# Lymphatus/caesium-clt

Measured on AMD Instinct MI355X. Metric: megapixels/sec JPEG q=80 1920x1080 batch, higher is better.
Workload: dtype int32

## Files before the change

caesium-clt_amd/binding.py:

```python
import ctypes as C
import os

_HERE = os.path.dirname(os.path.abspath(__file__))
NPHASES = 8
NKERNELS = 36
PHASE_NAMES = ["decode", "pixel", "masks_flags_runs", "stats_tables", "sizes_scan", "pack", "stuff_assemble", "reserved"]


class CCSParameters(C.Structure):
    _fields_ = [("keep_metadata", C.c_bool), ("jpeg_quality", C.c_uint32), ("jpeg_chroma_subsampling", C.c_uint32),
                ("jpeg_progressive", C.c_bool), ("jpeg_optimize", C.c_bool), ("jpeg_preserve_icc", C.c_bool),
                ("png_quality", C.c_uint32), ("png_optimization_level", C.c_uint32), ("png_force_zopfli", C.c_bool),
                ("png_optimize", C.c_bool), ("gif_quality", C.c_uint32), ("webp_quality", C.c_uint32), ("webp_lossless", C.c_bool),
                ("tiff_compression", C.c_uint32), ("tiff_deflate_level", C.c_uint32), ("width", C.c_uint32), ("height", C.c_uint32)]


class CCSResult(C.Structure):
    _fields_ = [("success", C.c_bool), ("code", C.c_uint32), ("error_message", C.c_char_p)]


class CByteArray(C.Structure):
    _fields_ = [("data", C.POINTER(C.c_uint8)), ("length", C.c_size_t)]


class Timing(C.Structure):
    _fields_ = [("total_ms", C.c_float), ("phase_ms", C.c_float * NPHASES), ("kernel_ms", C.c_float * NKERNELS), ("in_bytes", C.c_uint64), ("out_bytes", C.c_uint64),
                ("pixels", C.c_uint64), ("coef_bytes", C.c_uint64), ("n_images", C.c_uint32), ("n_failed", C.c_uint32), ("n_seq_decoded", C.c_uint32), ("n_par_fallback", C.c_uint32), ("n_par_short", C.c_uint32), ("n_prog_decoded", C.c_uint32), ("n_refine_chains", C.c_uint32), ("n_search_extra", C.c_uint32), ("n_fused_lists", C.c_uint32), ("n_list_refine", C.c_uint32), ("n_ac_in_lists", C.c_uint32)]


class PngTiming(C.Structure):
    _fields_ = [("total_ms", C.c_float), ("kernel_ms", C.c_float * 16), ("in_bytes", C.c_uint64), ("out_bytes", C.c_uint64), ("pixels", C.c_uint64),
                ("raw_bytes", C.c_uint64), ("n_images", C.c_uint32), ("n_failed", C.c_uint32), ("n_trials", C.c_uint32)]


class CaesiumError(RuntimeError):
    def __init__(self, code, message):
        super().__init__(f"[{code}] {message}")
        self.code = code


def library_path():
    return os.path.join(_HERE, "libcaesium_hip.so")


EXPORTS = ["cs_default_parameters", "cs_compress_in_memory", "cs_compress_to_size_in_memory", "cs_convert_in_memory",
           "cs_batch_compress", "cs_batch_extent", "cs_free_bytes", "cs_free_result", "csh_device_count", "csh_last_error", "csh_kernel_name", "csh_kernel_name_webp", "csh_release_cached_memory", "csh_warmup", "csh_batch_create",
           "csh_batch_run", "csh_batch_fetch", "csh_batch_destroy", "csh_batch_retain_dct", "csh_batch_set_quality", "csh_batch_rerun_encode", "cs_batch_compress_to_size", "csh_batch_geometry", "csh_batch_read_coefs",
           "csp_kernel_name", "csp_batch_create", "csp_batch_create_webp", "csp_batch_create_pixels", "csh_batch_create_pixels", "csh_batch_pixels", "csh_batch_create_from_pixels", "csp_png_to_jpeg", "csp_png_to_lossless_webp", "csp_batch_run", "csp_batch_fetch", "csp_batch_destroy", "csp_batch_geometry", "csp_batch_read_rows", "csp_batch_read_stream",
           "csp_batch_trials", "csp_batch_read_scores", "csp_batch_chunk_bits", "csh_batch_create_webp", "cs_batch_convert",
           "cswd_batch_create", "cswd_batch_run", "cswd_batch_pixels", "cswd_batch_read_pixels", "cswd_batch_alpha", "cswd_batch_read_rgba", "cswd_batch_destroy", "cswd_rgba_join", "cswd_rgba_destroy", "csh_batch_create_webp_from_pixels", "csh_batch_create_from_pixels_rgb", "csl_encode_pixels", "csl_attach_alpha"]


def _declare(L):
    P = C.POINTER
    L.cs_default_parameters.argtypes = [P(CCSParameters)]
    L.cs_default_parameters.restype = None
    L.cs_compress_in_memory.argtypes = [C.c_char_p, C.c_size_t, P(CCSParameters), P(CByteArray)]
    L.cs_compress_in_memory.restype = CCSResult
    L.cs_compress_to_size_in_memory.argtypes = [C.c_char_p, C.c_size_t, P(CCSParameters), C.c_size_t, C.c_bool, P(CByteArray)]
    L.cs_compress_to_size_in_memory.restype = CCSResult
    L.cs_convert_in_memory.argtypes = [C.c_char_p, C.c_size_t, P(CCSParameters), C.c_uint32, P(CByteArray)]
    L.cs_convert_in_memory.restype = CCSResult
    L.cs_batch_compress.argtypes = [P(CByteArray), C.c_size_t, P(CCSParameters), C.c_int, P(CByteArray), P(CCSResult)]
    L.cs_batch_extent.argtypes = [P(CByteArray), C.c_size_t]
    L.cs_batch_extent.restype = C.c_size_t
    L.cs_free_bytes.argtypes = [P(CByteArray)]
    L.cs_free_bytes.restype = None
    L.cs_free_result.argtypes = [P(CCSResult)]
    L.cs_free_result.restype = None
    L.csh_last_error.restype = C.c_char_p
    L.csh_kernel_name.argtypes = [C.c_int]
    L.csh_kernel_name.restype = C.c_char_p
    L.csh_kernel_name_webp.argtypes = [C.c_int]
    L.csh_kernel_name_webp.restype = C.c_char_p
    L.csh_batch_create.argtypes = [P(CByteArray), C.c_size_t, P(CCSParameters), C.c_int, P(C.c_void_p)]
    L.csh_batch_run.argtypes = [C.c_void_p, P(Timing)]
    L.csh_batch_fetch.argtypes = [C.c_void_p, P(CByteArray), P(CCSResult)]
    L.csh_batch_retain_dct.argtypes = [C.c_void_p, C.c_int]
    L.csh_batch_set_quality.argtypes = [C.c_void_p, P(C.c_uint32)]
    L.csh_batch_rerun_encode.argtypes = [C.c_void_p, P(Timing)]
    L.cs_batch_compress_to_size.argtypes = [P(CByteArray), C.c_size_t, P(CCSParameters), C.c_size_t, C.c_bool, C.c_int, P(CByteArray), P(CCSResult)]
    L.csh_batch_destroy.argtypes = [C.c_void_p]
    L.csh_batch_destroy.restype = None
    L.csh_batch_geometry.argtypes = [C.c_void_p, C.c_size_t, C.c_int, C.c_int, P(C.c_int), P(C.c_int), P(C.c_int), P(C.c_int)]
    L.csh_batch_read_coefs.argtypes = [C.c_void_p, C.c_size_t, C.c_int, C.c_int, C.c_void_p]
    L.csh_batch_create_webp.argtypes = [P(CByteArray), C.c_size_t, P(CCSParameters), C.c_int, P(C.c_void_p)]
    L.cs_batch_convert.argtypes = [P(CByteArray), C.c_size_t, P(CCSParameters), C.c_uint32, C.c_int, P(CByteArray), P(CCSResult)]
    L.csp_kernel_name.argtypes = [C.c_int]
    L.csp_kernel_name.restype = C.c_char_p
    L.csp_batch_create.argtypes = [P(CByteArray), C.c_size_t, P(CCSParameters), C.c_int, P(C.c_void_p)]
    L.csp_batch_run.argtypes = [C.c_void_p, P(PngTiming)]
    L.csp_batch_fetch.argtypes = [C.c_void_p, P(CByteArray), P(CCSResult)]
    L.csp_batch_destroy.argtypes = [C.c_void_p]
    L.csp_batch_destroy.restype = None
    L.csp_batch_geometry.argtypes = [C.c_void_p, C.c_size_t, P(C.c_uint32), P(C.c_uint32), P(C.c_uint32)]
    L.csp_batch_read_rows.argtypes = [C.c_void_p, C.c_size_t, C.c_void_p]
    L.csp_batch_read_stream.argtypes = [C.c_void_p, C.c_size_t, C.c_int, C.c_void_p]
    L.csp_batch_read_scores.argtypes = [C.c_void_p, C.c_size_t, C.c_void_p, P(C.c_int)]
    L.csp_batch_chunk_bits.argtypes = [C.c_void_p, C.c_size_t, C.c_int, P(C.c_uint64), C.c_size_t, P(C.c_size_t)]
    L.csp_batch_trials.argtypes = [C.c_void_p, C.c_size_t, P(C.c_int), P(C.c_uint64), P(C.c_int), P(C.c_int)]
    L.cswd_batch_create.argtypes = [P(CByteArray), C.c_size_t, C.c_int, P(C.c_void_p)]
    L.cswd_batch_run.argtypes = [C.c_void_p]
    L.cswd_batch_pixels.argtypes = [C.c_void_p, C.c_size_t, P(C.c_void_p), P(C.c_uint32), P(C.c_uint32), P(C.c_uint32), P(C.c_char_p)]
    L.cswd_batch_read_pixels.argtypes = [C.c_void_p, C.c_size_t, C.c_void_p]
    L.cswd_batch_alpha.argtypes = [C.c_void_p, C.c_size_t, P(C.c_void_p), P(C.c_void_p)]
    L.cswd_batch_read_rgba.argtypes = [C.c_void_p, C.c_size_t, C.c_void_p]
    L.cswd_batch_destroy.argtypes = [C.c_void_p]
    L.cswd_batch_destroy.restype = None
    L.cswd_rgba_join.argtypes = [C.c_void_p, C.c_void_p, C.c_uint32, C.c_uint32, C.c_int, C.POINTER(C.c_void_p), C.POINTER(C.c_void_p)]
    L.cswd_rgba_join.restype = C.c_int
# ... 344 lines not shown
```

caesium-clt_amd/csrc/batch.hpp:

```cpp
#pragma once
#include <array>
#include <chrono>
#include <map>
#include <string>
#include <vector>

#include "../../include/caesium_hip.h"
#include "devmem.hpp"
#include "jpeg_host.hpp"
#include "kernels.h"
#include "webp_kernels.h"

namespace csh {

struct Item {
    int code = 0;
    std::string msg;
    JpegInfo in;
    JpegInfo out;
    int image = -1;
    size_t file_size = 0;
    std::vector<uint8_t> meta_out;
};

struct DecodePlan {
    PinnedBytes bits_pool;
    std::vector<DecScan> dscans;
    std::vector<DevHuffSet> hsets;
    std::vector<ParHuffSet> phsets;
    std::vector<char> phset_fits;
    std::vector<ParHuffSet4> phsets4;
    std::vector<std::array<int8_t, 8>> slot4;
    bool use4 = true;
    std::vector<ParScan> pscans;
    std::vector<uint32_t> need_seq_init;
    std::vector<ProgChain> chains;
    std::vector<int> chain_scans;
    std::vector<RefineUnit> refine_units;
    uint32_t refine_hist = 0, refine_pos = 0, refine_max_blocks = 0;
    uint32_t total_sub = 0, max_sub = 0, max_par_blocks = 0, dc_total = 0;

    DevBuf<uint8_t> d_bits, d_clean;
    DevBuf<ParScan> d_pscans;
    DevBuf<uint64_t> d_pstate, d_relax_list[2], d_unstuff_off, d_blk_off, d_dc_off;
    DevBuf<uint32_t> d_unstuff_cnt, d_nblk, d_need_seq, d_need_seq_init, d_relax_cnt, d_scan_pending, d_cut_block, d_claim;
    DevBuf<uint16_t> d_hyp;
    DevBuf<int32_t> d_dcdiff;
    DevBuf<DecScan> d_dscans;
    DevBuf<ProgChain> d_chains;
    DevBuf<int> d_chain_scans;
    DevBuf<uint64_t> d_refine_hist;
    DevBuf<uint32_t> d_refine_pos, d_refine_prog;
    DevBuf<RefineUnit> d_refine_units;
    DevBuf<DevHuffSet> d_hsets;
    DevBuf<ParHuffSet> d_phsets;
    DevBuf<ParHuffSet4> d_phsets4;
};

struct PixelPlan {
    std::vector<PlaneWork> pwork;
    std::vector<ResizeWork> rwork;
    std::vector<ResizeTap> rtaps;
    std::vector<float> rweights;
    uint64_t rgb_bytes = 0, tmp_floats = 0, max_tmp = 0, max_dst = 0;
    uint32_t max_row_in = 0, max_out_w = 0, max_nh = 0;
    uint32_t max_src_px = 0;
    uint64_t plane_bytes = 0, oplane_bytes = 0;
    uint32_t max_quads = 0;
    bool any_layout = false, any_layout_rgb = false;

    DevBuf<uint8_t> d_planes, d_oplanes, d_rgb;
    DevBuf<PlaneWork> d_pwork;
    DevBuf<ResizeWork> d_rwork;
    DevBuf<ResizeTap> d_rtaps;
    DevBuf<float> d_rweights, d_rtmp;
    DevBuf<int16_t> d_dct_raw;
};

struct Stage {
    uint32_t work0 = 0, nwork = 0, slot0 = 0, nslots = 0, ech0 = 0, nech = 0, table0 = 0, ntables = 0, plan0 = 0, nplans = 0, nzc0 = 0, nnzc = 0, ls0 = 0, nls = 0, ts0 = 0, nts = 0, rs0 = 0, nrs = 0;
    bool nz_build[2] = {true, true}, nz_filter[2] = {true, true};
};
struct SearchImg {
    int cand_work[64]; int ncand;
    int Al_luma = 0, Al_chroma = 0;
    uint64_t best_luma = 0, best_chroma = 0;
    int split_luma = 0, split_chroma = 0;
    bool luma_on = false, chroma_on = false;
};

struct EncodePlan {
    std::vector<EncScan> script;
    std::vector<ScanWork> swork;
    uint32_t nslots = 0, nlist_slots = 0, ntok_slots = 0;
    uint32_t nref_slots = 0;
    uint32_t last_run_refine = 0;
    uint64_t total_corr = 0;
    uint64_t total_units = 0, total_words = 0;
    uint32_t max_units = 0;
    int ntables = 0;
    std::vector<TokPlan> plans;
    std::vector<int> plan_comp, plan_image;
    std::vector<EChunk> echunks;
    uint64_t tok_cap = 0;
    uint32_t tok_scale = 1;
    std::vector<TokRegion> regions;
    std::vector<uint32_t> region_est;
    uint32_t hist_rows = 0;
    std::vector<NzList> nzlists;
    std::vector<NzSet> nzsets;
    std::vector<int> nzset_of;
    std::vector<uint32_t> nzset_built;
    std::vector<int> nzset_comp, nzset_image;
    std::vector<NzChunk> nzchunks;
    std::vector<NzChunk> nzchunks_fused;
    uint32_t n_fused = 0;
    uint32_t last_run_fused = 0;
    uint32_t n_ac_lists = 0;
    uint32_t last_run_ac_lists = 0;
    std::vector<uint8_t> nzset_ac_lists;
    std::vector<uint32_t> nz_est, nz_worst;
    uint32_t nz_nrec = 0;
    uint64_t nz_cap = 0;
    bool search = false;
    enum { ST_1 = 0, ST_1B = 1, ST_2 = 2, ST_2B = 3, ST_2C = 4, ST_N = 5 };
    Stage stage[ST_N];
    void stage_begin(Stage &sg) {
        sg.work0 = uint32_t(swork.size()); sg.slot0 = nslots; sg.ech0 = uint32_t(echunks.size()); sg.table0 = uint32_t(ntables); sg.plan0 = uint32_t(plans.size());
        sg.nzc0 = uint32_t(nzchunks.size()); sg.ls0 = nlist_slots; sg.ts0 = ntok_slots; sg.rs0 = nref_slots;
    }
    void stage_end(Stage &sg) {
        sg.nwork = uint32_t(swork.size()) - sg.work0; sg.nslots = nslots - sg.slot0; sg.nech = uint32_t(echunks.size()) - sg.ech0;
        sg.ntables = uint32_t(ntables) - sg.table0; sg.nplans = uint32_t(plans.size()) - sg.plan0;
        sg.nnzc = uint32_t(nzchunks.size()) - sg.nzc0; sg.nls = nlist_slots - sg.ls0; sg.nts = ntok_slots - sg.ts0; sg.nrs = nref_slots - sg.rs0;
    }
    std::vector<SearchImg> simg;
    std::vector<uint8_t> work_active;
    uint32_t n_gated_runs = 0;
    std::vector<uint32_t> img_list, img_nlist, h_cost;
    std::map<std::array<int, 5>, int> cand_script;
    std::vector<uint8_t> hdr_pool;
    std::vector<uint32_t> hdr_off;

    DevBuf<uint8_t> d_hdr, d_tail, d_scan_tmp, d_work_active;
    DevBuf<EncScan> d_script;
    DevBuf<ScanWork> d_swork;
    DevBuf<uint32_t> d_slot_work;
    DevBuf<EChunk> d_echunks;
    DevBuf<SlotRec> d_slots;
    DevBuf<TokPlan> d_plans;
    DevBuf<uint64_t> d_corr, d_symbits, d_eobbits, d_tok_off, d_chunk_off, d_scan_raw_off;
    DevBuf<uint32_t> d_tok_cursor;
    DevBuf<TokRegion> d_regions;
    DevBuf<uint16_t> d_eobrun, d_slot_hist;
    DevBuf<uint32_t> d_img_list, d_img_nlist, d_scan_cost, d_slot_raw, d_slot_eobh, d_long_runs, d_long_cnt, d_tokens, d_chunk_ntok, d_chunk_bits, d_raw, d_scan_pad, d_chunk_ff, d_hdr_off;
    DevBuf<DevEncTable> d_tables;
    DevBuf<NzList> d_nzlists;
    DevBuf<NzSet> d_nzsets;
    DevBuf<NzChunk> d_nzchunks, d_nzchunks_fused;
    DevBuf<uint32_t> d_nz_pool, d_nz_cursor, d_nz_chunk_off, d_nz_chunk_cnt, d_list_slots, d_tok_slots, d_ref_slots;
};

struct TrellisPlan {
    bool trellis = false, dering = false;
    Stage tstage;
    std::vector<TrellisWork> twork;
    std::vector<TrellisRun> truns;
    uint32_t t_units = 0, t_max_rows = 0;
    std::vector<uint32_t> trows;
    bool t_sort = false;
    bool nz_once = false;

    DevBuf<TrellisWork> d_twork;
    DevBuf<TrellisRun> d_truns;
    DevBuf<uint32_t> d_tqueue, d_trows, d_tperm, d_tspill;
    DevBuf<uint8_t> d_tblk_cnt;
    DevBuf<uint16_t> d_tblk_off;
    DevBuf<uint64_t> d_tlambda, d_tdcbt;
};

struct WebpTail {
    uint32_t webp_mb_bytes = 768;
    std::vector<csw::WebpImg> wimgs;
    uint64_t wwork_bytes = 0, wlevels = 0;
    uint32_t wmax_luma = 0, wmax_mbh = 0;

    DevBuf<csw::WebpImg> d_wimgs;
    DevBuf<uint8_t> d_wwork, d_wscratch, d_wprobs, d_wupdate;
    DevBuf<uint32_t> d_wpart, d_wstats;
    DevBuf<int16_t> d_wlevels;
};

struct Outputs {
    uint64_t raw_bytes_cap = 0, out_cap = 0;
    DevBuf<uint8_t> d_out;
    DevBuf<uint64_t> d_img_off;
    DevBuf<uint32_t> d_img_size, d_img_size_pad, d_status, d_overflow;
    std::vector<uint32_t> h_img_size;
    std::vector<uint64_t> h_img_off;
    std::vector<uint32_t> h_status;
    bool ran = false;
};

}

struct csh_batch {
    int device = 0;
    hipStream_t stream = 0;
    bool have_stream = false;
    CCSParameters params;
    std::vector<csh::Item> items;
    int nimg = 0;
    bool lossless = false;
    bool rgb_out = false;
    bool webp = false;
    int test_pool_shift = -1;
    bool progressive = true;
    bool retain_dct = false;
    bool have_dct = false;
    int q_base = 0;

    std::vector<csh::ImgDesc> imgs;
    std::vector<csh::DevQuant> quants;
    uint32_t ntiles = 0, ntiles_in = 0, ntiles_out = 0, max_tiles = 0, max_dummy = 0;
    csh::DevBuf<csh::ImgDesc> d_imgs;
    csh::DevBuf<csh::DevQuant> d_quants;
    csh::DevBuf<int16_t> d_coef;

    csh::DecodePlan dec;
    csh::PixelPlan pix;
    csh::EncodePlan enc;
    csh::TrellisPlan tr;
    csh::WebpTail wp;
    csh::Outputs out;

    ~csh_batch() { if (have_stream) { (void)hipStreamSynchronize(stream); (void)hipStreamDestroy(stream); } }
};

namespace csh {

enum KernelSlot {
    KS_MEMSET_COEF, KS_UNSTUFF, KS_DEC_SPEC, KS_DEC_RELAX0, KS_DEC_RELAX, KS_DEC_WRITE, KS_DC_SCATTER, KS_REFINE_CHAINS, KS_DECODE_PROG_SEQ,
    KS_IDCT_PLANE, KS_RESIZE, KS_XFORM_DIRECT, KS_RESAMPLE_FDCT, KS_FIX_DUMMY, KS_MEMSET_ENC, KS_TRELLIS_STATS, KS_TRELLIS_AC, KS_TRELLIS_DC,
    KS_NZLIST, KS_TOKENS, KS_LIST_STATS, KS_AC_RUNS, KS_GEN_TABLES, KS_CHUNK_SIZES, KS_SCAN_CHUNK_BITS, KS_SCAN_LAYOUT, KS_PACK, KS_LIST_PACK,
    KS_FF_COUNT, KS_SCAN_SEARCH, KS_LAYOUT, KS_SCAN_IMAGES, KS_EMIT, KS_SPARE0, KS_SPARE1, KS_SPARE2, KS_COUNT,
    KS_WEBP_YUV = KS_XFORM_DIRECT, KS_WEBP_ENCODE = KS_RESAMPLE_FDCT, KS_WEBP_ASSEMBLE = KS_FIX_DUMMY
};
struct KernelSlotRow { KernelSlot slot; const char *name; int phase; };
constexpr KernelSlotRow kKernelSlots[] = {
    {KS_MEMSET_COEF, "memset_coef", 0},        {KS_UNSTUFF, "unstuff", 0},                 {KS_DEC_SPEC, "k_dec_spec", 0},
    {KS_DEC_RELAX0, "k_dec_relax0", 0},        {KS_DEC_RELAX, "k_dec_relax1_4", 0},        {KS_DEC_WRITE, "k_dec_write", 0},
    {KS_DC_SCATTER, "k_dc_scatter", 0},        {KS_REFINE_CHAINS, "k_refine_chains", 0},   {KS_DECODE_PROG_SEQ, "k_decode_prog+seq", 0},
    {KS_IDCT_PLANE, "k_idct_plane", 1},        {KS_RESIZE, "resize", 1},                   {KS_XFORM_DIRECT, "k_xform_direct", 1},
    {KS_RESAMPLE_FDCT, "k_resample+k_plane_fdct", 1}, {KS_FIX_DUMMY, "k_fix_dummy", 1},    {KS_MEMSET_ENC, "memset_enc", 2},
    {KS_TRELLIS_STATS, "trellis_stats", 1},    {KS_TRELLIS_AC, "k_trellis_ac", 1},         {KS_TRELLIS_DC, "k_trellis_dc", 1},
    {KS_NZLIST, "k_nzlist", 2},                {KS_TOKENS, "k_tokens", 2},                 {KS_LIST_STATS, "k_list_stats", 2},
    {KS_AC_RUNS, "k_ac_runs", 2},              {KS_GEN_TABLES, "k_gen_tables", 3},         {KS_CHUNK_SIZES, "k_chunk_sizes", 4},
    {KS_SCAN_CHUNK_BITS, "scan_chunk_bits", 4}, {KS_SCAN_LAYOUT, "scan_layout", 4},        {KS_PACK, "k_pack", 5},
    {KS_LIST_PACK, "k_list_pack", 5},          {KS_FF_COUNT, "k_ff_count", 6},             {KS_SCAN_SEARCH, "scan_search_stage2", 7},
    {KS_LAYOUT, "k_layout", 6},                {KS_SCAN_IMAGES, "scan_images", 6},         {KS_EMIT, "k_emit", 6},
    {KS_SPARE0, "", 7},                        {KS_SPARE1, "", 7},                         {KS_SPARE2, "", 7}};
constexpr bool kernel_slots_in_order() {
    for (int i = 0; i < int(sizeof kKernelSlots / sizeof kKernelSlots[0]); i++) if (kKernelSlots[i].slot != i) return false;
    return true;
}
static_assert(sizeof kKernelSlots / sizeof kKernelSlots[0] == CSH_NKERNELS && int(KS_COUNT) == int(CSH_NKERNELS), "one row per csh_timing.kernel_ms slot");
static_assert(kernel_slots_in_order(), "row i of kKernelSlots describes slot i");

struct PlanSwitches {
    std::string profile;
    bool nz_once = true;
    bool tr_sort = true;
    int prog_par = -1;
    bool fused_420 = true;
    bool nz_fused = true;
    bool ref_list = true;
    bool ac_tiles = false;
    static PlanSwitches read();
};

struct Laps {
    const bool trace;
    std::chrono::steady_clock::time_point at = std::chrono::steady_clock::now();
    std::string text;
    Laps();
    void lap(const char *what);
};

struct BatchPlanner {
    csh_batch *const b;
    const CByteArray *const inputs;
    const size_t count;
    const CCSParameters *const p;
    const csp_pixels *const px;
    const PlanSwitches sw;
    const bool progressive;
    uint16_t qout_nat[64];
    int script_base3 = 0, script_base1 = 0;
    std::vector<std::pair<std::vector<uint8_t>, int>> hset_keys;
    std::map<std::vector<uint16_t>, int> quant_index;
    uint64_t plane_off = 64, oplane_off = 0;

    BatchPlanner(csh_batch *b, const CByteArray *inputs, size_t count, const CCSParameters *p, const csp_pixels *px);
    void begin();
    void parse();
    int reserve_pinned();
    int plan_image(size_t n);
    int plan_search_stages();
    int plan_trellis();
    void finish_descriptors();
    int upload(Laps &laps);

private:
    void image_geometry(Item &it, ImgDesc &im);
    int decode_scans(Item &it, ImgDesc &im, const uint8_t *d);
    int huff_set(const JScan &js);
    void place_blocks(ParScan &ps, const JpegInfo &in, const JScan &js, uint32_t units, bool dc_rows, bool subseqs);
    int sequential_split(const Item &it, const ImgDesc &im, const uint8_t *d, int img_index, bool &par_ok);
    bool progressive_plan(const Item &it, const ImgDesc &im, int img_index);
    void plane_work(ImgDesc &im, const JpegInfo &in, const JpegInfo &o, int img_index, bool resized);
    void resize_work(const JpegInfo &in, const JpegInfo &o, int img_index);
    void output_scans(Item &it, ImgDesc &im, int img_index, size_t in_len);
    void frame_header(Item &it);
    template <class Fill> int enc_scan(const std::array<int, 5> &key, Fill fill);
    int cand_index(int comp, int Ss, int Se, int Ah, int Al);
    int dc_scan_index(int ncomp);
    int seq1_index(int comp);
    uint32_t nz_list(int img_index, int comp, int Al, const ImgDesc &im, size_t in_len);
    void add_works(Item &it, ImgDesc &im, int img_index, const std::vector<int> &list, size_t in_len, const JpegInfo &o, bool stats_only = false);
    template <class Make> void add_stage(int sid, Make make);
    template <class Add> void splits(const ImgDesc &im, Add &add, int i0, int i1, bool whole);
};

void layout_token_pool(csh_batch *b);

int run_once(csh_batch *b, csh_timing *t, bool requant_only);

int search_costs(csh_batch *b, AsmCtx &a, int stage);
uint32_t search_gate(csh_batch *b, int stage, int (*want)(const SearchImg &));
int search_decide(csh_batch *b, int stage);
int search_lists(csh_batch *b);

}
```

caesium-clt_amd/csrc/batch_plan.cpp:

```cpp
#include <algorithm>
#include <atomic>
#include <cmath>
#include <thread>

#include "batch.hpp"
#include "resize_host.h"

namespace csh {

static void build_dev_huff(const HuffSpec &h, DevHuff &d) {
    memset(&d, 0, sizeof d);
    for (int l = 0; l < 18; l++) d.maxcode[l] = -1;
    if (!h.present) return;
    int code = 0, p = 0;
    for (int l = 1; l <= 16; l++) {
        if (h.bits[l]) {
            d.valptr[l] = p - code;
            for (int i = 0; i < h.bits[l]; i++, p++, code++)
                if (l <= 9) {
                    int base = code << (9 - l);
                    for (int k = 0; k < (1 << (9 - l)); k++) d.look[(base + k) & 511] = uint16_t((l << 8) | h.vals[p]);
                }
            d.maxcode[l] = code - 1;
        }
// ... 115 lines not shown
    else if (hx == 2 && vx == 1 && cw > 2) u.cls = CSH_UP_H2V1;
    else if (hx == 1 && vx == 2) u.cls = CSH_UP_H1V2;
    else if (hx == 2 && vx == 2 && cw > 2) u.cls = CSH_UP_H2V2;
    else u.cls = CSH_UP_REP;
    return u;
}
static int dn_kind(int hx, int vx) { return hx == 1 ? CSH_DN_FULL : (hx == 4 ? CSH_DN_H4V1 : (vx == 2 ? CSH_DN_H2V2 : CSH_DN_H2V1)); }

static int plan_item(Item &it, const CCSParameters &p, bool lossless) {
    const JpegInfo &in = it.in;
    if (in.ncomp != 1 && in.ncomp != 3) { it.msg = "unsupported component count (CMYK/YCCK not on the device path yet)"; return CS_ERR_JPEG_FEATURE; }
    if (in.ncomp == 3) {
        bool rgb_ids = in.comp[0].id == 'R' && in.comp[1].id == 'G' && in.comp[2].id == 'B';
        if (in.adobe_transform == 0 || rgb_ids) { it.msg = "RGB-colourspace JPEG not on the device path yet"; return CS_ERR_JPEG_FEATURE; }
    }
    if (uint64_t(in.width) * uint64_t(in.height) > (1ull << 28)) { it.msg = "image dimensions too large for the device path"; return CS_ERR_JPEG_FEATURE; }
    it.out = JpegInfo();
    JpegInfo &o = it.out;
    o.width = in.width; o.height = in.height; o.ncomp = in.ncomp;
    if (p.width || p.height) {
        if (lossless) { it.msg = "resize + lossless transcode not on the device path"; return CS_ERR_UNSUPPORTED; }
        csh_compute_dimensions(in.width, in.height, int(p.width), int(p.height), o.width, o.height);
        if (o.width > 65500 || o.height > 65500 || uint64_t(o.width) * uint64_t(o.height) > (1ull << 28)) { it.msg = "resize target too large for JPEG"; return CS_ERR_JPEG_FEATURE; }
    }
    if (lossless) {
        for (int c = 0; c < in.ncomp; c++) o.comp[c] = in.comp[c];
        jpeg_geometry(o);
        return 0;
    }
    int ss = int(p.jpeg_chroma_subsampling);
    if (ss == 0) ss = 420;
    for (int c = 0; c < in.ncomp; c++) { o.comp[c].id = c + 1; o.comp[c].h = o.comp[c].v = 1; o.comp[c].tq = c ? 1 : 0; }
    if (in.ncomp == 3) {
        int blocks = 0;
        for (int c = 0; c < 3; c++) {
            const JComp &k = in.comp[c];
            blocks += k.h * k.v;
            if (in.hmax % k.h || in.vmax % k.v) { it.msg = "fractional chroma sampling ratio (component factors do not divide the largest ones)"; return CS_ERR_JPEG_FEATURE; }
            if (in.hmax / k.h > 4 || in.vmax / k.v > 4) { it.msg = "chroma sampling ratio above 4"; return CS_ERR_JPEG_FEATURE; }
        }
        if (blocks > 10) { it.msg = "more than 10 blocks per MCU"; return CS_ERR_JPEG_FEATURE; }
        if (ss == 420) { o.comp[0].h = 2; o.comp[0].v = 2; }
        else if (ss == 422) { o.comp[0].h = 2; o.comp[0].v = 1; }
        else if (ss == 411) { o.comp[0].h = 4; o.comp[0].v = 1; }
        else if (ss != 444) { it.msg = "unknown output chroma subsampling"; return CS_ERR_JPEG_FEATURE; }
    }
    jpeg_geometry(o);
    return 0;
}

void layout_token_pool(csh_batch *b) {
    b->enc.regions.resize(b->enc.region_est.size());
    if (b->test_pool_shift < 0) b->test_pool_shift = getenv("CSH_TEST_POOL_SHIFT") ? std::min(16, std::max(0, atoi(getenv("CSH_TEST_POOL_SHIFT")))) : 0;
    const int shift = b->test_pool_shift;
    uint64_t at = 0;
    for (size_t i = 0; i < b->enc.regions.size(); i++) {
        const uint64_t cap = std::min<uint64_t>(std::max<uint64_t>((uint64_t(b->enc.region_est[i]) * b->enc.tok_scale) >> shift, 64), 0xFFFFFFF0ull);
        b->enc.regions[i].base = at; b->enc.regions[i].cap = uint32_t(cap); b->enc.regions[i].pad = 0;
        at += (cap + 3) & ~uint64_t(3);
    }
    b->enc.tok_cap = at + 64;
    at = 0;
    for (size_t i = 0; i < b->enc.nzlists.size(); i++) {
        const uint64_t cap = std::min<uint64_t>(std::max<uint64_t>((uint64_t(b->enc.nz_est[i]) * b->enc.tok_scale) >> shift, 64), b->enc.nz_worst[i]);
        b->enc.nzlists[i].base = at; b->enc.nzlists[i].cap = uint32_t(cap);
        at += (cap + 3) & ~uint64_t(3);
    }
    b->enc.nz_cap = at + 64;
}

PlanSwitches PlanSwitches::read() {
    auto is = [](const char *name, const char *v) { const char *e = getenv(name); return e && !strcmp(e, v); };
    PlanSwitches s;
    const char *penv = getenv("CSH_PROFILE");
    s.profile = penv && *penv ? penv : "mozjpeg";
    s.nz_once = !is("CSH_NZ_ONCE", "0");
    s.tr_sort = !is("CSH_TR_SORT", "0");
    s.nz_fused = !is("CSH_NZ_FUSED", "0");
    s.ac_tiles = is("CSH_AC_TILES", "1");
    s.ref_list = is("CSH_REF_LIST", "1") || (s.ref_list && !is("CSH_REF_LIST", "0"));
    const char *pp = getenv("CSH_PROG_PAR");
    s.prog_par = pp && !strcmp(pp, "0") ? 0 : (pp && !strcmp(pp, "1") ? 1 : -1);
    s.fused_420 = !getenv("CSH_NO_FUSED_420");
    return s;
}

Laps::Laps() : trace(getenv("CSH_TRACE") != nullptr) {}
void Laps::lap(const char *what) {
    if (!trace) return;
    const auto now = std::chrono::steady_clock::now();
    char buf[64];
    snprintf(buf, sizeof buf, " %s %.1f", what, std::chrono::duration<double, std::milli>(now - at).count());
    text += buf; at = now;
}

BatchPlanner::BatchPlanner(csh_batch *b_, const CByteArray *inputs_, size_t count_, const CCSParameters *p_, const csp_pixels *px_)
    : b(b_), inputs(inputs_), count(count_), p(p_), px(px_), sw(PlanSwitches::read()), progressive(p_->jpeg_progressive) {}

void BatchPlanner::begin() {
    b->items.resize(count);
    quality_table(int(p->jpeg_quality), qout_nat);
    DevQuant qo; make_quant(qout_nat, qo);
    b->quants.push_back(qo);
    b->q_base = int(b->quants.size()) - 1;
    for (int q = 1; q <= 100; q++) { uint16_t tq[64]; quality_table(q, tq); DevQuant dq; make_quant(tq, dq); b->quants.push_back(dq); }
    b->progressive = progressive;

    add_script(b->enc.script, 3, true);
    add_script(b->enc.script, 1, true);
    add_script(b->enc.script, 3, false);
    add_script(b->enc.script, 1, false);
    script_base3 = progressive ? 0 : 16; script_base1 = progressive ? 10 : 17;
    const bool webp = b->webp, rgb_out = b->rgb_out;
    const std::string &profile = sw.profile;
    b->enc.search = progressive && !webp && !rgb_out && profile != "plain";
    const bool lossy_jpeg = !b->lossless && !webp && !rgb_out;
    b->tr.trellis = lossy_jpeg && (profile == "mozjpeg" || profile == "mozjpeg-trellis");
    b->tr.dering = lossy_jpeg && (profile == "mozjpeg" || profile == "mozjpeg-dering");
    b->tr.nz_once = b->tr.trellis && progressive && sw.nz_once && sw.tr_sort;
}

template <class Fill>
int BatchPlanner::enc_scan(const std::array<int, 5> &key, Fill fill) {
    auto f = b->enc.cand_script.find(key);
    if (f != b->enc.cand_script.end()) return f->second;
    EncScan e;
    memset(&e, 0, sizeof e);
    fill(e);
    b->enc.script.push_back(e);
    return b->enc.cand_script[key] = int(b->enc.script.size()) - 1;
}
int BatchPlanner::cand_index(int comp, int Ss, int Se, int Ah, int Al) {
    return enc_scan({comp, Ss, Se, Ah, Al}, [&](EncScan &e) {
        const int id = comp ? 1 : 0;
        e.ncomp = 1; e.comp[0] = comp; e.Ss = Ss; e.Se = Se; e.Ah = Ah; e.Al = Al;
        e.ntables = 1; e.dht_id[0] = 0x10 | id; e.sos_tdta[0] = id;
    });
}
int BatchPlanner::dc_scan_index(int ncomp) {
    return enc_scan({-ncomp, 0, 0, 0, 0}, [&](EncScan &e) {
        e.ncomp = ncomp;
        for (int k = 0; k < ncomp; k++) {
            e.comp[k] = k;
            const int id = k ? 1 : 0;
            int idx = -1;
            for (int t = 0; t < e.ntables; t++) if (e.dht_id[t] == id) idx = t;
            if (idx < 0) { idx = e.ntables; e.dht_id[e.ntables++] = id; }
            e.dc_tbl[k] = idx; e.sos_tdta[k] = id << 4;
        }
    });
}
int BatchPlanner::seq1_index(int comp) {
    return enc_scan({comp, 0, 63, -1, -1}, [&](EncScan &e) {
        const int id = comp ? 1 : 0;
        e.ncomp = 1; e.comp[0] = comp; e.Ss = 0; e.Se = 63; e.sequential = 1;
        e.ntables = 2; e.dht_id[0] = id; e.dht_id[1] = 0x10 | id; e.dc_tbl[0] = 0; e.ac_tbl[0] = 1; e.sos_tdta[0] = (id << 4) | id;
    });
}

static uint64_t blocks_of(const ImgDesc &im) {
    uint64_t n = 0;
    for (int k = 0; k < im.ncomp; k++) n += uint64_t(im.out[k].real_bw) * im.out[k].real_bh;
    return n;
}

uint32_t BatchPlanner::nz_list(int img_index, int comp, int Al, const ImgDesc &im, size_t in_len) {
    if (b->enc.nzset_of.size() < size_t(img_index + 1) * CSH_MAX_COMPS) b->enc.nzset_of.resize(size_t(img_index + 1) * CSH_MAX_COMPS, -1);
    int &si = b->enc.nzset_of[size_t(img_index) * CSH_MAX_COMPS + size_t(comp)];
    const uint32_t nu = uint32_t(im.out[comp].real_bw * im.out[comp].real_bh);
    if (si < 0) {
        NzSet S;
        memset(&S, 0, sizeof S);
        for (int L = 0; L < CSH_NZ_LEVELS; L++) S.list[L] = 0xFFFFFFFFu;
        S.cnt_base = 0xFFFFFFFFu;
        S.nunits = nu; S.real_bw = im.out[comp].real_bw; S.bw = im.out[comp].bw; S.tile_base = im.out[comp].tile_base;
        si = int(b->enc.nzsets.size());
        b->enc.nzsets.push_back(S); b->enc.nzset_built.push_back(0u); b->enc.nzset_comp.push_back(comp); b->enc.nzset_image.push_back(img_index);
    }
    const uint64_t blocks_all = blocks_of(im);
    static const uint32_t kShare[CSH_NZ_LEVELS] = {20, 16, 12, 9};
    for (int L : {0, Al}) {
        if (b->enc.nzsets[size_t(si)].list[L] != 0xFFFFFFFFu) continue;
        const uint32_t nch = (nu + 255) / 256;
        NzList R;
        memset(&R, 0, sizeof R);
        R.chunk0 = b->enc.nz_nrec; b->enc.nz_nrec += nch;
        b->enc.nzsets[size_t(si)].list[L] = uint32_t(b->enc.nzlists.size());
        b->enc.nzlists.push_back(R);
        const uint64_t est = uint64_t(in_len) * kShare[L] / 8 * nu / std::max<uint64_t>(1, blocks_all) + nu + 4ull * nch + 256;
        const uint64_t worst = uint64_t(nu) * 64 + 4ull * nch;
        b->enc.nz_est.push_back(uint32_t(std::min<uint64_t>(est, worst)));
        b->enc.nz_worst.push_back(uint32_t(std::min<uint64_t>(worst, 0xFFFFFFF0ull)));
    }
    return b->enc.nzsets[size_t(si)].list[Al];
}

void BatchPlanner::add_works(Item &it, ImgDesc &im, int img_index, const std::vector<int> &list, size_t in_len, const JpegInfo &o, bool stats_only) {
    const int w_first = int(b->enc.swork.size());
    uint32_t nz_need[CSH_MAX_COMPS] = {0, 0, 0}, nz_gate[CSH_MAX_COMPS] = {0, 0, 0};
    for (int sidx : list) {
        const EncScan &e = b->enc.script[sidx];
        ScanWork w;
        memset(&w, 0, sizeof w);
        w.image = img_index; w.scan = sidx;
        w.out_off = 0xFFFFFFFFu;
        const bool from_list = e.Ss > 0 && !e.sequential && e.Ah == 0;
        const bool ref_list = sw.ref_list && e.Ss > 0 && !e.sequential && e.Ah != 0;
        w.list = 0xFFFFFFFFu; w.rs_base = 0xFFFFFFFFu;
        if (from_list || ref_list) {
            if (e.Al >= CSH_NZ_LEVELS) { it.code = CS_ERR_JPEG_FEATURE; it.msg = "internal: output scan script outside what the list coder carries"; }
            else {
                w.list = nz_list(img_index, e.comp[0], e.Al, im, in_len);
                if (!nz_need[e.comp[0]]) nz_gate[e.comp[0]] = uint32_t(b->enc.swork.size());
                nz_need[e.comp[0]] |= 1u << e.Al;
            }
        }
        if (e.Ss == 0 && e.ncomp > 1) w.nunits = uint32_t(im.omcus_x * im.omcus_y);
        else w.nunits = uint32_t(im.out[e.comp[0]].real_bw * im.out[e.comp[0]].real_bh);
        w.unit_base = uint32_t(b->enc.total_units);
        b->enc.total_units += w.nunits;
        w.corr_base = 0xFFFFFFFFu;
        if (e.Ss > 0 && !e.sequential && e.Ah) { w.corr_base = uint32_t(b->enc.total_corr); b->enc.total_corr += w.nunits; }
        w.word_base = uint32_t(b->enc.total_words);
        if (e.Ss) b->enc.total_words += (w.nunits + 63) / 64;
        w.table_base = uint32_t(b->enc.ntables);
        b->enc.ntables += e.ntables;
        b->enc.max_units = std::max(b->enc.max_units, w.nunits);
        {
            const uint32_t nch = (w.nunits + 255) / 256;
            w.first_chunk = b->enc.nslots; b->enc.nslots += nch;
            w.hist_row0 = b->enc.hist_rows; b->enc.hist_rows += nch * uint32_t(e.ntables);
            uint32_t &cursor = (from_list && w.list != 0xFFFFFFFFu) ? b->enc.nlist_slots : b->enc.ntok_slots;
            w.ls_base = cursor; cursor += nch;
            if (ref_list && w.list != 0xFFFFFFFFu) { w.rs_base = b->enc.nref_slots; b->enc.nref_slots += nch; }
        }
        if (e.Ss == 0 || e.sequential) {
            uint32_t blocks = 0;
            for (int k = 0; k < e.ncomp; k++) blocks += e.ncomp > 1 ? uint32_t(o.comp[e.comp[k]].h * o.comp[e.comp[k]].v) : 1u;
            const uint32_t per_unit = e.sequential ? blocks * 20u : (e.Ah ? (blocks + 14u) / 15u : blocks);
            for (uint32_t j = 0; j < (w.nunits + 255) / 256; j++) b->enc.echunks.push_back(EChunk{uint32_t(b->enc.swork.size()), 0, 1, j, 0, uint32_t(b->enc.region_est.size())});
            b->enc.region_est.push_back(stats_only ? 64u : w.nunits * per_unit + 64);
        }
        b->enc.swork.push_back(w);
    }
    for (int c = 0; c < im.ncomp; c++) {
        if (!nz_need[c]) continue;
        const int si = b->enc.nzset_of[size_t(img_index) * CSH_MAX_COMPS + size_t(c)];
        uint32_t levels = stats_only ? (nz_need[c] | 1u) : ((nz_need[c] | 1u) & ~b->enc.nzset_built[size_t(si)]);
        b->enc.nzset_built[size_t(si)] |= levels;
        if (!stats_only && b->tr.nz_once && (levels & 1u)) levels = (levels & ~1u) | CSH_NZ_COMPACT0;
        const uint32_t nu = b->enc.nzsets[size_t(si)].nunits;
        for (uint32_t j = 0; levels && j < (nu + 255) / 256; j++) b->enc.nzchunks.push_back(NzChunk{uint32_t(si), j, levels, nz_gate[c]});
    }
    for (int c = 0; c < im.ncomp; c++) {
        int nac = 0;
        for (int sidx : list) { const EncScan &e = b->enc.script[sidx]; if (e.Ss > 0 && !e.sequential && e.Ah && e.comp[0] == c) { nac++; if (e.Al > 3 && !sw.ref_list) nac = 99; } }
        const bool too_many = !sw.ref_list && nac > CSH_TK_MAXSLOT;
        if (too_many) { it.code = CS_ERR_JPEG_FEATURE; it.msg = "internal: output scan script outside what the token kernel carries"; }
        const uint32_t nu = uint32_t(im.out[c].real_bw * im.out[c].real_bh);
        if (!nac || too_many) continue;
        const uint64_t blocks_all = blocks_of(im);
        const uint64_t scripts = b->enc.search ? uint64_t(nac + 1) / 2 : 1;
        const uint64_t est = uint64_t(in_len) * 3 * scripts * nu / std::max<uint64_t>(1, blocks_all) + uint64_t(nu) * nac + 1024;
        if (sw.ref_list) {
            for (size_t k = 0; k < list.size(); k++) {
                const EncScan &e = b->enc.script[list[k]];
                if (e.Ss > 0 && !e.sequential && e.Ah && e.comp[0] == c && b->enc.swork[size_t(w_first) + k].rs_base != 0xFFFFFFFFu) b->enc.swork[size_t(w_first) + k].region = uint32_t(b->enc.region_est.size());
            }
            b->enc.region_est.push_back(stats_only ? 64u : uint32_t(std::min<uint64_t>(est, 0x3FFFFFFFu)));
            continue;
        }
        TokPlan P;
        memset(&P, 0, sizeof P);
        P.nunits = nu; P.real_bw = im.out[c].real_bw; P.bw = im.out[c].bw; P.tile_base = im.out[c].tile_base;
        P.work0 = 0xFFFFFFFFu;
        for (size_t k = 0; k < list.size(); k++) {
            const EncScan &e = b->enc.script[list[k]];
            if (!(e.Ss > 0 && !e.sequential && e.Ah && e.comp[0] == c)) continue;
            const ScanWork &w = b->enc.swork[size_t(w_first) + k];
            if (P.work0 == 0xFFFFFFFFu) P.work0 = uint32_t(w_first) + uint32_t(k);
            AcSlot &a = P.s[P.nslot++];
            a.unit_base = w.unit_base; a.word_base = w.word_base; a.first_chunk = w.first_chunk; a.table_base = w.table_base; a.nunits_work = w.nunits; a.corr_base = w.corr_base;
            a.Ss = uint8_t(e.Ss); a.Se = uint8_t(e.Se); a.Ah = uint8_t(e.Ah); a.Al = uint8_t(e.Al);
        }
        for (uint32_t j = 0; j < (nu + 255) / 256; j++) b->enc.echunks.push_back(EChunk{uint32_t(img_index), uint16_t(c), 0, j, uint32_t(b->enc.plans.size()), uint32_t(b->enc.region_est.size())});
        b->enc.region_est.push_back(stats_only ? 64u : uint32_t(std::min<uint64_t>(est, 0x3FFFFFFFu)));
        b->enc.plan_comp.push_back(c); b->enc.plan_image.push_back(img_index);
        b->enc.plans.push_back(P);
    }
}

void BatchPlanner::parse() {
    std::atomic<size_t> next{0};
    auto worker = [&]() {
        for (size_t n; (n = next++) < count;) {
            Item &it = b->items[n];
            it.file_size = inputs[n].length;
            int type = sniff_type(inputs[n].data, inputs[n].length);
            if (type == CS_TYPE_UNKN) { it.code = CS_ERR_UNKNOWN_TYPE; it.msg = "unknown file type"; }
            else if (type != CS_TYPE_JPEG) { it.code = CS_ERR_UNSUPPORTED; it.msg = "this input format has no device path in this build (built: JPEG, PNG)"; }
            else it.code = parse_jpeg(inputs[n].data, inputs[n].length, it.in, it.msg);
        }
    };
    size_t nthreads = std::min<size_t>(std::min<size_t>(16, std::max(1u, std::thread::hardware_concurrency())), (count + 15) / 16);
    std::vector<std::thread> pool;
    for (size_t t = 1; t < nthreads; t++) pool.emplace_back(worker);
    worker();
    for (auto &t : pool) t.join();
}

int BatchPlanner::reserve_pinned() {
    size_t total = 0;
    for (size_t n = 0; n < count; n++) total += inputs[n].length;
    if (total + total / 16 + (64u << 10) >= 0xF0000000ull) { csh_set_error("csh_batch_create: more than 3.75 GiB of input in one device batch (cs_batch_extent sizes groups)"); return CS_ERR_POOL_OVERFLOW; }
    if (!b->dec.bits_pool.reserve(total + total / 16 + (64u << 10))) { csh_set_error("out of pinned host memory"); return CS_ERR_NO_DEVICE; }
    return 0;
}
// ... 533 lines not shown
        std::vector<uint8_t> fused(b->enc.nzsets.size(), 0);
        const bool lists_only = progressive && !sw.ac_tiles && sw.ref_list && sw.nz_once && sw.tr_sort && (!b->tr.trellis || (b->tr.t_sort && b->tr.nz_once));
        std::vector<uint8_t> planned(b->enc.nzsets.size(), 0);
        for (size_t i = 0; i < b->enc.plans.size(); i++) {
            const size_t at = size_t(b->enc.plan_image[i]) * CSH_MAX_COMPS + size_t(b->enc.plan_comp[i]);
            if (at < b->enc.nzset_of.size() && b->enc.nzset_of[at] >= 0) planned[size_t(b->enc.nzset_of[at])] = 1;
        }
        b->enc.nzset_ac_lists.assign(b->enc.nzsets.size(), 0);
        for (PlaneWork &w : b->pix.pwork) {
            w.ac_lists = 0u;
            const size_t at = size_t(w.image) * CSH_MAX_COMPS + size_t(w.comp);
            const int si = allowed && at < b->enc.nzset_of.size() ? b->enc.nzset_of[at] : -1;
            if (si < 0) continue;
            const NzSet &S = b->enc.nzsets[size_t(si)];
            if (S.real_bw != S.bw || S.list[0] == 0xFFFFFFFFu) continue;
            w.nzset = uint32_t(si); fused[size_t(si)] = 1; b->enc.n_fused++;
            if (lists_only && !planned[size_t(si)]) { w.ac_lists = 1u; b->enc.nzset_ac_lists[size_t(si)] = 1; b->enc.n_ac_lists++; }
        }
        for (TrellisWork &tw : b->tr.twork) tw.ac_lists = (tw.nzset != 0xFFFFFFFFu && b->enc.nzset_ac_lists[tw.nzset]) ? 1u : 0u;
        for (NzChunk &ch : b->enc.nzchunks_fused) if (fused[ch.set]) ch.levels &= ~1u;
        auto flags = [&](Stage &sg) {
            for (int f = 0; f < 2; f++) {
                const std::vector<NzChunk> &v = f ? b->enc.nzchunks_fused : b->enc.nzchunks;
                sg.nz_build[f] = sg.nz_filter[f] = false;
                for (uint32_t i = sg.nzc0; i < sg.nzc0 + sg.nnzc; i++) { sg.nz_build[f] |= (v[i].levels & 1u) != 0u; sg.nz_filter[f] |= (v[i].levels & ~1u) != 0u; }
            }
        };
        for (Stage &sg : b->enc.stage) flags(sg);
        flags(b->tr.tstage);
    }
    for (ParScan &ps : b->dec.pscans)
        for (int m = 0; m < ps.nb_mcu && m < 10; m++) {
            int dcs = ps.dct[m] & 3, acs = 4 + (ps.act[m] & 3);
            if (b->dec.use4) { dcs = std::max<int>(0, b->dec.slot4[ps.huff_set][dcs]); acs = std::max<int>(0, b->dec.slot4[ps.huff_set][acs]); }
            ps.sel |= uint64_t(dcs | (acs << 3)) << (6 * m);
        }
    {
        std::vector<int> last(b->dec.chains.size(), -1);
        for (int s = 0;; s++) {
            bool any = false;
            for (size_t c = 0; c < b->dec.chains.size(); c++)
                if (b->dec.chains[c].refine && b->dec.chains[c].count > s) {
                    RefineUnit u; u.chain = int(c); u.s = s; u.prev = last[c];
                    last[c] = int(b->dec.refine_units.size());
                    b->dec.refine_units.push_back(u);
                    any = true;
                }
            if (!any) break;
        }
    }
    b->ntiles = b->ntiles_in + b->ntiles_out;
    b->pix.plane_bytes = plane_off;
    b->pix.oplane_bytes = oplane_off;
    b->out.out_cap = b->out.raw_bytes_cap;
    layout_token_pool(b);
}

int BatchPlanner::upload(Laps &laps) {
    hipStream_t st = b->stream;
    if (!b->nimg) return 0;
    b->dec.bits_pool.flush_copies();
    laps.lap("copy_in");
    if (b->dec.d_bits.alloc(b->dec.bits_pool.size()) || (b->dec.bits_pool.size() && hipMemcpyAsync(b->dec.d_bits.p, b->dec.bits_pool.p, b->dec.bits_pool.size(), hipMemcpyHostToDevice, st) != hipSuccess) ||
        b->d_imgs.upload(b->imgs, st) || b->dec.d_dscans.upload(b->dec.dscans, st) || b->dec.d_chains.upload(b->dec.chains, st) || b->dec.d_chain_scans.upload(b->dec.chain_scans, st) ||
        b->dec.d_hsets.upload(b->dec.hsets, st) || b->dec.d_phsets.upload(b->dec.phsets, st) || (b->dec.use4 && b->dec.d_phsets4.upload(b->dec.phsets4, st)) || b->d_quants.upload(b->quants, st) || b->pix.d_pwork.upload(b->pix.pwork, st) ||
        b->enc.d_script.upload(b->enc.script, st) || b->enc.d_swork.upload(b->enc.swork, st) || b->enc.d_slot_work.alloc(size_t(b->enc.nslots) + 1) || b->enc.d_slots.alloc(size_t(b->enc.nslots) + 1) || b->enc.d_plans.upload(b->enc.plans, st) || b->enc.d_echunks.upload(b->enc.echunks, st) || b->enc.d_hdr.upload(b->enc.hdr_pool, st) ||
        b->enc.d_hdr_off.upload(b->enc.hdr_off, st) || b->dec.d_pscans.upload(b->dec.pscans, st) || b->pix.d_rwork.upload(b->pix.rwork, st) || b->pix.d_rtaps.upload(b->pix.rtaps, st) ||
        b->pix.d_rweights.upload(b->pix.rweights, st) || b->pix.d_rgb.alloc(b->pix.rgb_bytes + 64) || b->pix.d_rtmp.alloc((resize_is_fused(b->pix.max_row_in) ? 0 : b->pix.tmp_floats) + 16) || b->dec.d_need_seq_init.upload(b->dec.need_seq_init, st))
        return CS_ERR_NO_DEVICE;
    size_t nchunks = b->dec.bits_pool.size() / 64 + 1, nst = size_t(b->dec.total_sub) + b->dec.pscans.size() + 1;
    if (b->dec.d_clean.alloc(b->dec.bits_pool.size() + 64) || b->dec.d_unstuff_cnt.alloc(nchunks + 1) || b->dec.d_unstuff_off.alloc(nchunks + 2) ||
        b->dec.d_pstate.alloc(nst) || b->dec.d_relax_list[0].alloc(nst) || b->dec.d_relax_list[1].alloc(nst) || b->dec.d_relax_cnt.alloc(512) || b->dec.d_scan_pending.alloc(b->dec.pscans.size() + 1) || b->dec.d_cut_block.alloc(b->dec.pscans.size() + 1) || b->dec.d_claim.alloc(size_t(b->dec.total_sub) + 1) || b->dec.d_hyp.alloc((size_t(b->dec.total_sub) + 1) * 10) ||
        b->dec.d_nblk.alloc(size_t(b->dec.total_sub) + 1) || b->dec.d_blk_off.alloc(size_t(b->dec.total_sub) + 2) || b->dec.d_need_seq.alloc(b->nimg + 1) ||
        b->dec.d_dcdiff.alloc(size_t(b->dec.dc_total) + 1) || b->dec.d_dc_off.alloc(size_t(b->dec.dc_total) + 2) ||
        b->dec.d_refine_hist.alloc(size_t(b->dec.refine_hist) + 1) || b->dec.d_refine_pos.alloc(size_t(b->dec.refine_pos) + 1) || b->dec.d_refine_units.upload(b->dec.refine_units, st) ||
        b->dec.d_refine_prog.alloc(b->dec.refine_units.size() + 1))
        return CS_ERR_NO_DEVICE;
    if (b->d_coef.alloc(size_t(b->ntiles) * CSH_TILE_I16) || b->pix.d_planes.alloc(b->pix.plane_bytes + 64) || b->pix.d_oplanes.alloc(b->pix.oplane_bytes + 64) ||
        b->enc.d_symbits.alloc(b->enc.total_words + 1) || b->enc.d_eobbits.alloc(b->enc.total_words + 1) ||
        b->enc.d_long_runs.alloc(2 * (b->enc.total_units / 512 + b->enc.swork.size() + 16)) || b->enc.d_long_cnt.alloc(4) || b->enc.d_tail.alloc(b->enc.total_units + 1) || b->enc.d_eobrun.alloc(b->enc.total_units + 1) || b->enc.d_corr.alloc(b->enc.total_corr + 1) ||
        b->enc.d_tok_off.alloc(4 * size_t(b->enc.nslots) + 4) || b->enc.d_chunk_ntok.alloc(4 * size_t(b->enc.nslots) + 4) || b->enc.d_slot_hist.alloc(size_t(b->enc.hist_rows) * 256 + 256) ||
        b->enc.d_slot_raw.alloc(size_t(b->enc.nslots) + 1) || b->enc.d_img_list.upload(b->enc.img_list, st) || b->enc.d_img_nlist.upload(b->enc.img_nlist, st) || b->enc.d_scan_cost.alloc(b->enc.swork.size() + 1) || b->enc.d_slot_eobh.alloc(16 * size_t(b->enc.nslots) + 16) || b->enc.d_chunk_bits.alloc(size_t(b->enc.nslots) + 1) || b->enc.d_chunk_off.alloc(size_t(b->enc.nslots) + 2) || b->enc.d_tok_cursor.alloc(b->enc.region_est.size() + 1) || b->enc.d_regions.upload(b->enc.regions, st) ||
        b->enc.d_tables.alloc(b->enc.ntables) || b->enc.d_scan_pad.alloc(b->enc.swork.size() + 1) ||
        b->enc.d_nzlists.upload(b->enc.nzlists, st) || b->enc.d_nzsets.upload(b->enc.nzsets, st) || b->enc.d_nzchunks.upload(b->enc.nzchunks, st) || (b->enc.n_fused && b->enc.d_nzchunks_fused.upload(b->enc.nzchunks_fused, st)) || b->enc.d_list_slots.alloc(size_t(b->enc.nlist_slots) + 1) || b->enc.d_tok_slots.alloc(size_t(b->enc.ntok_slots) + 1) || b->enc.d_ref_slots.alloc(size_t(b->enc.nref_slots) + 1) ||
        b->enc.d_nz_cursor.alloc(b->enc.nzlists.size() + 1) || b->enc.d_nz_chunk_off.alloc(size_t(b->enc.nz_nrec) + 1) || b->enc.d_nz_chunk_cnt.alloc(size_t(b->enc.nz_nrec) + 1) ||
        b->enc.d_scan_raw_off.alloc(b->enc.swork.size() + 2) || b->out.d_img_size.alloc(b->nimg + 1) || b->out.d_img_size_pad.alloc(b->nimg + 1) ||
        b->out.d_img_off.alloc(b->nimg + 2) || b->out.d_status.alloc(b->nimg) || b->out.d_overflow.alloc(4))
        return CS_ERR_NO_DEVICE;
    if (hipMemsetAsync(b->enc.d_slots.p, 0, (size_t(b->enc.nslots) + 1) * sizeof(SlotRec), st) != hipSuccess ||
        hipMemsetAsync(b->enc.d_slot_work.p, 0, (size_t(b->enc.nslots) + 1) * sizeof(uint32_t), st) != hipSuccess) { csh_set_error("hipMemsetAsync failed"); return CS_ERR_NO_DEVICE; }
    launch_make_slots(st, b->enc.d_swork.p, uint32_t(b->enc.swork.size()), b->enc.d_script.p, b->enc.d_nzlists.p, b->enc.d_slots.p, b->enc.d_slot_work.p, b->enc.d_list_slots.p, b->enc.d_tok_slots.p, b->enc.d_ref_slots.p);
    if (b->tr.trellis && (b->tr.d_trows.upload(b->tr.trows, st) || (b->tr.t_sort && (b->tr.d_tperm.alloc(size_t(b->tr.t_units) + 1) || b->tr.d_tblk_cnt.alloc(size_t(b->tr.t_units) + 1) || (b->tr.nz_once && b->tr.d_tblk_off.alloc(size_t(b->tr.t_units) + 1)))))) return CS_ERR_NO_DEVICE;
    if (b->tr.trellis && (b->tr.d_twork.upload(b->tr.twork, st) || b->tr.d_truns.upload(b->tr.truns, st) || b->tr.d_tqueue.alloc(1) || b->tr.d_tlambda.alloc(size_t(b->tr.t_units) + 1) || b->tr.d_tdcbt.alloc(size_t(b->tr.t_units) + 1) ||
                       b->tr.d_tspill.alloc(trellis_spill_words(trellis_ac_slots())) || b->pix.d_dct_raw.alloc(size_t(b->ntiles_out) * CSH_TILE_I16)))
        return CS_ERR_NO_DEVICE;
    for (size_t n = 0; px && n < count; n++) {
        const Item &it = b->items[n];
        if (it.image < 0) continue;
        const ResizeWork &rw = b->pix.rwork[size_t(it.image)];
        if (rw.image != it.image) { csh_set_error("internal: resize work out of order"); return CS_ERR_NO_DEVICE; }
        if (hipMemcpyAsync(b->pix.d_rgb.p + rw.rgb_src_off, px[n].device_pixels, size_t(px[n].width) * px[n].height * px[n].channels, hipMemcpyDeviceToDevice, st) != hipSuccess) { csh_set_error("pixel copy failed"); return CS_ERR_NO_DEVICE; }
    }
    laps.lap("alloc+enqueue");
    if (hipStreamSynchronize(st) != hipSuccess) { csh_set_error("upload failed"); return CS_ERR_NO_DEVICE; }
    laps.lap("upload_wait");
    return 0;
}

}
```

caesium-clt_amd/csrc/batch_run.cpp:

```cpp
#include <algorithm>

#include "batch.hpp"

namespace csh {
namespace {

class KernelMarks {
    hipEvent_t ev[CSH_NKERNELS + 1];
    int created = 0, next = 0;
    const hipStream_t st;

public:
    explicit KernelMarks(hipStream_t s) : st(s) {}
    KernelMarks(const KernelMarks &) = delete;
    KernelMarks &operator=(const KernelMarks &) = delete;
    ~KernelMarks() { for (int i = 0; i < created; i++) (void)hipEventDestroy(ev[i]); }
    int start() {
        for (; created <= CSH_NKERNELS; created++) CSH_CHECK(hipEventCreate(&ev[created]));
        CSH_CHECK(hipEventRecord(ev[0], st));
        return 0;
    }
    int claim(KernelSlot slot, hipEvent_t *e) {
        if (int(slot) != next || next >= CSH_NKERNELS) {
            csh_set_error("internal: timing mark '%s' out of order (slot %d is next)", slot < KS_COUNT ? kKernelSlots[slot].name : "?", next);
// ... 149 lines not shown
                      b->pix.max_src_px, b->pix.max_tmp, b->pix.max_dst, b->pix.max_row_in, b->pix.max_out_w, b->pix.max_nh, !(b->webp || b->rgb_out), b->pix.any_layout_rgb);
        MARK(KS_RESIZE);
        return 0;
    }
    int pixels() {
        const int nw = b->lossless ? 0 : int(b->pix.pwork.size());
        int16_t *rawp = ((b->retain_dct || b->tr.trellis) && !b->lossless) ? b->pix.d_dct_raw.p : nullptr;
        NzFuse nzf;
        memset(&nzf, 0, sizeof nzf);
        fused = nw && b->enc.n_fused;
        if (fused) {
            if (b->enc.d_nz_cursor.zero(st) || b->enc.d_nz_chunk_cnt.zero(st)) return -1;
            nzf.nzsets = b->enc.d_nzsets.p; nzf.nzlists = b->enc.d_nzlists.p; nzf.nz_pool = b->enc.d_nz_pool.p; nzf.nz_cursor = b->enc.d_nz_cursor.p;
            nzf.nz_chunk_off = b->enc.d_nz_chunk_off.p; nzf.nz_chunk_cnt = b->enc.d_nz_chunk_cnt.p; nzf.overflow = b->out.d_overflow.p;
            nzf.blk_cnt = (b->tr.trellis && b->tr.t_sort) ? b->tr.d_tblk_cnt.p : nullptr;
            nzf.blk_off = (nzf.blk_cnt && b->tr.nz_once) ? b->tr.d_tblk_off.p : nullptr;
        }
        if (nw && getenv("CSH_DEBUG") && (uint32_t(atoi(getenv("CSH_DEBUG"))) & 32768u))
            CSH_CHECK(hipMemsetAsync(b->d_coef.p + size_t(b->ntiles_in) * CSH_TILE_I16, 0x5A, size_t(b->ntiles - b->ntiles_in) * CSH_TILE_I16 * sizeof(int16_t), st));
        launch_xform_direct(st, b->d_imgs.p, b->pix.d_pwork.p, nw, b->max_tiles, b->d_quants.p, b->d_coef.p, b->d_coef.p, rawp, b->ntiles_in, b->tr.dering, nzf);
        MARK(KS_XFORM_DIRECT);
        launch_resample_plane(st, b->d_imgs.p, b->pix.d_pwork.p, nw, b->pix.max_quads, b->pix.d_planes.p, b->pix.d_oplanes.p);
        if (b->pix.any_layout) launch_resample_any(st, b->d_imgs.p, b->pix.d_pwork.p, nw, b->pix.max_quads, b->pix.d_planes.p, b->pix.d_oplanes.p);
        launch_plane_fdct(st, b->d_imgs.p, b->pix.d_pwork.p, nw, b->max_tiles, b->d_quants.p, b->pix.d_oplanes.p, b->d_coef.p, rawp, b->ntiles_in, b->tr.dering, nzf);
        launch_resample_fdct_420(st, b->d_imgs.p, b->pix.d_pwork.p, nw, b->max_tiles, b->d_quants.p, b->pix.d_planes.p, b->d_coef.p, rawp, b->ntiles_in, b->tr.dering, nzf);
        MARK(KS_RESAMPLE_FDCT);
        if (!b->lossless) launch_fix_dummy(st, b->d_imgs.p, nimg, b->max_dummy, b->d_coef.p);
        MARK(KS_FIX_DUMMY);
        return 0;
    }

    void fill_enc_ctx() {
        memset(&c, 0, sizeof c);
        c.imgs = b->d_imgs.p; c.script = b->enc.d_script.p; c.work = b->enc.d_swork.p; c.nwork = int(b->enc.swork.size());
        c.echunks = b->enc.d_echunks.p; c.plans = b->enc.d_plans.p; c.nechunks = uint32_t(b->enc.echunks.size()); c.slot_work = b->enc.d_slot_work.p; c.slots = b->enc.d_slots.p; c.nslots = b->enc.nslots;
        c.coef = b->d_coef.p; c.sym_bits = b->enc.d_symbits.p; c.eob_bits = b->enc.d_eobbits.p; c.tail = b->enc.d_tail.p;
        c.eobrun = b->enc.d_eobrun.p; c.long_runs = b->enc.d_long_runs.p; c.long_cnt = b->enc.d_long_cnt.p; c.corr = b->enc.d_corr.p;
        c.tokens = b->enc.d_tokens.p; c.regions = b->enc.d_regions.p; c.tok_cursor = b->enc.d_tok_cursor.p; c.tok_off = b->enc.d_tok_off.p; c.chunk_ntok = b->enc.d_chunk_ntok.p; c.slot_hist = b->enc.d_slot_hist.p; c.slot_raw = b->enc.d_slot_raw.p; c.slot_eobh = b->enc.d_slot_eobh.p;
        c.chunk_bits = b->enc.d_chunk_bits.p; c.chunk_off = b->enc.d_chunk_off.p; c.tables = b->enc.d_tables.p;
        c.raw = b->enc.d_raw.p; c.raw_words = raw_chunks * 16; c.status = b->out.d_status.p; c.overflow = b->out.d_overflow.p;
        c.nzlists = b->enc.d_nzlists.p; c.nzsets = b->enc.d_nzsets.p; c.nz_pool = b->enc.d_nz_pool.p; c.nz_cursor = b->enc.d_nz_cursor.p; c.nz_chunk_off = b->enc.d_nz_chunk_off.p; c.nz_chunk_cnt = b->enc.d_nz_chunk_cnt.p;
        c.debug = getenv("CSH_DEBUG") ? uint32_t(atoi(getenv("CSH_DEBUG"))) : 0u;
    }
    void fill_asm_ctx() {
        memset(&a, 0, sizeof a);
        a.imgs = b->d_imgs.p; a.script = b->enc.d_script.p; a.work = b->enc.d_swork.p; a.nimg = nimg;
        a.nwork = b->tr.trellis ? int(b->tr.tstage.work0) : c.nwork;
        a.tables = b->enc.d_tables.p; a.chunk_off = b->enc.d_chunk_off.p; a.scan_pad_bytes = b->enc.d_scan_pad.p; a.scan_raw_off = b->enc.d_scan_raw_off.p;
        a.raw = b->enc.d_raw.p; a.raw_chunks = raw_chunks; a.chunk_ff = b->enc.d_chunk_ff.p;
        a.hdr_pool = b->enc.d_hdr.p; a.hdr_off = b->enc.d_hdr_off.p; a.img_size = b->out.d_img_size.p; a.img_size_pad = b->out.d_img_size_pad.p;
        a.img_off = b->out.d_img_off.p; a.out = b->out.d_out.p; a.out_cap = b->out.out_cap; a.status = b->out.d_status.p; a.overflow = b->out.d_overflow.p;
        a.img_list = b->enc.d_img_list.p; a.img_nlist = b->enc.d_img_nlist.p; a.scan_cost = b->enc.d_scan_cost.p;
    }
    void fill_trellis_ctx(TrellisCtx &tc) {
        memset(&tc, 0, sizeof tc);
        tc.imgs = b->d_imgs.p; tc.quant = b->d_quants.p; tc.work = b->tr.d_twork.p; tc.nwork = int(b->tr.twork.size()); tc.runs = b->tr.d_truns.p; tc.nruns = uint32_t(b->tr.truns.size());
        tc.tables = b->enc.d_tables.p; tc.raw = b->pix.d_dct_raw.p; tc.raw_tile0 = b->ntiles_in; tc.coef = b->d_coef.p; tc.dcrec = b->tr.d_tlambda.p; tc.dcbt = b->tr.d_tdcbt.p;
        tc.spill = b->tr.d_tspill.p; tc.nslots = uint32_t(b->tr.d_tspill.n / trellis_spill_words(1)); tc.max_rows = b->tr.t_max_rows;
        tc.queue = b->tr.d_tqueue.p;
        tc.rows = b->tr.d_trows.p; tc.nrows = uint32_t(b->tr.trows.size());
        if (b->tr.t_sort) { tc.blk_cnt = b->tr.d_tblk_cnt.p; tc.perm = b->tr.d_tperm.p; }
        if (b->tr.t_sort && b->tr.nz_once) {
            tc.nz_pool = b->enc.d_nz_pool.p; tc.nzlists = b->enc.d_nzlists.p; tc.nzsets = b->enc.d_nzsets.p; tc.nz_chunk_off = b->enc.d_nz_chunk_off.p; tc.nz_chunk_cnt = b->enc.d_nz_chunk_cnt.p;
            tc.blk_off = b->tr.d_tblk_off.p;
        }
        tc.ac_lists = fused ? 1u : 0u;
        tc.debug = getenv("CSH_TR_DEBUG") ? uint32_t(atoi(getenv("CSH_TR_DEBUG"))) : 0u;
    }

    int encode_begin() {
        fill_enc_ctx();
        launch_reset_works(st, b->enc.d_swork.p, c.nwork);
        if (!fused && (b->enc.d_nz_cursor.zero(st) || b->enc.d_nz_chunk_cnt.zero(st))) return -1;
        if (b->enc.d_symbits.zero(st) || b->enc.d_eobbits.zero(st) || (!eobrun_cleared && b->enc.d_eobrun.zero(st)) || b->enc.d_tables.zero(st) || b->enc.d_tok_cursor.zero(st) || b->enc.d_slot_eobh.zero(st) || b->enc.d_scan_pad.zero(st)) return -1;
#ifdef CSH_EMUL
        if (b->enc.d_raw.zero(st)) return -1;
#else
        if ((c.debug & 8192u) && b->enc.d_raw.zero(st)) return -1;
#endif
        MARK(KS_MEMSET_ENC);
        return 0;
    }

    void set_stage(const Stage &sg) {
        c.echunks = b->enc.d_echunks.p + sg.ech0; c.nechunks = sg.nech; c.slot0 = sg.slot0; c.nslots = sg.nslots;
        c.nzchunks = (fused ? b->enc.d_nzchunks_fused.p : b->enc.d_nzchunks.p) + sg.nzc0; c.nnzchunks = sg.nnzc;
        c.nz_build = sg.nz_build[fused ? 1 : 0]; c.nz_filter = sg.nz_filter[fused ? 1 : 0];
        c.list_slots = b->enc.d_list_slots.p + sg.ls0; c.nlist_slots = sg.nls; c.tok_slots = b->enc.d_tok_slots.p + sg.ts0; c.ntok_slots = sg.nts;
        c.ref_slots = b->enc.d_ref_slots.p + sg.rs0; c.nref_slots = sg.nrs;
    }

    int trellis() {
        const Stage &tg = b->tr.tstage;
        set_stage(tg);
        c.stats_only = 1;
        if (b->enc.d_long_cnt.zero(st)) return -1;
        c.nz_blk_cnt = b->tr.t_sort ? b->tr.d_tblk_cnt.p : nullptr;
        c.nz_blk_off = (b->tr.t_sort && b->tr.nz_once) ? b->tr.d_tblk_off.p : nullptr;
        launch_nzlist(st, c);
        c.nz_blk_cnt = nullptr; c.nz_blk_off = nullptr;
        if (b->tr.t_sort) {
            TrellisCtx ts;
            memset(&ts, 0, sizeof ts);
            ts.work = b->tr.d_twork.p; ts.nwork = int(b->tr.twork.size()); ts.blk_cnt = b->tr.d_tblk_cnt.p; ts.perm = b->tr.d_tperm.p;
            launch_trellis_sort(st, ts);
        }
        launch_tokens(st, c);
        launch_list_stats(st, c);
        launch_ac_runs(st, c);
        launch_gen_tables(st, b->enc.d_tables.p + tg.table0, int(tg.ntables));
        c.stats_only = 0;
        if (b->enc.d_nz_cursor.zero(st)) return -1;
        MARK(KS_TRELLIS_STATS);
        TrellisCtx tc;
        fill_trellis_ctx(tc);
        if (b->tr.d_tqueue.zero(st)) return -1;
        launch_trellis_ac(st, tc);
        MARK(KS_TRELLIS_AC);
        launch_trellis_dc(st, tc);
        launch_fix_dummy(st, b->d_imgs.p, nimg, b->max_dummy, b->d_coef.p);
        MARK(KS_TRELLIS_DC);
        return 0;
    }

    int stage(const Stage &sg, bool mark, bool gate) {
#define SMARK(slot) do { if (mark) MARK(slot); } while (0)
        set_stage(sg);
        c.work_active = gate ? b->enc.d_work_active.p : nullptr;
        a.work0 = int(sg.work0); a.nwork_run = int(sg.nwork);
        if (b->enc.d_long_cnt.zero(st)) return -1;
        launch_nzlist(st, c);
        SMARK(KS_NZLIST);
        launch_list_refine(st, c);
        for (uint32_t wi = sg.work0; sg.nrs && wi < sg.work0 + sg.nwork; wi++)
            if (b->enc.swork[wi].rs_base != 0xFFFFFFFFu && (!gate || b->enc.work_active[wi])) b->enc.last_run_refine++;
        launch_tokens(st, c);
        SMARK(KS_TOKENS);
        launch_list_stats(st, c);
        SMARK(KS_LIST_STATS);
        launch_ac_runs(st, c);
        SMARK(KS_AC_RUNS);
        launch_gen_tables(st, b->enc.d_tables.p + sg.table0, int(sg.ntables));
        SMARK(KS_GEN_TABLES);
        launch_chunk_sizes(st, c);
        SMARK(KS_CHUNK_SIZES);
        launch_exclusive_scan(st, b->enc.d_chunk_bits.p + sg.slot0, b->enc.d_chunk_off.p + sg.slot0, sg.nslots, b->enc.d_scan_tmp.p, b->enc.d_scan_tmp.n);
        SMARK(KS_SCAN_CHUNK_BITS);
        launch_scan_sizes(st, a);
        launch_exclusive_scan(st, b->enc.d_scan_pad.p, b->enc.d_scan_raw_off.p, uint64_t(a.nwork), b->enc.d_scan_tmp.p, b->enc.d_scan_tmp.n);
        launch_scan_place(st, a);
        launch_zero_edges(st, c);
        SMARK(KS_SCAN_LAYOUT);
        launch_pack(st, c);
        SMARK(KS_PACK);
        launch_list_pack(st, c);
        SMARK(KS_LIST_PACK);
        launch_ff_count(st, a);
        SMARK(KS_FF_COUNT);
#undef SMARK
        return 0;
    }

    int gated_stage(int sid, int (*want)(const SearchImg &)) {
        if (!search_gate(b, sid, want)) return 0;
        b->enc.n_gated_runs++;
        if (b->enc.d_work_active.upload(b->enc.work_active, st)) return -1;
        if (stage(b->enc.stage[sid], false, true) || search_costs(b, a, sid)) return -1;
        return search_decide(b, sid);
    }
    int search() {
        b->enc.n_gated_runs = 0;
        if (search_costs(b, a, EncodePlan::ST_1) || search_decide(b, EncodePlan::ST_1)) return -1;
        if (gated_stage(EncodePlan::ST_1B, [](const SearchImg &si) { return si.luma_on ? 1 : 0; })) return -1;
        if (stage(b->enc.stage[EncodePlan::ST_2], false, false)) return -1;
        if (search_costs(b, a, EncodePlan::ST_2) || search_decide(b, EncodePlan::ST_2)) return -1;
        for (int sid : {int(EncodePlan::ST_2B), int(EncodePlan::ST_2C)})
            if (gated_stage(sid, [](const SearchImg &si) { return (si.luma_on ? 1 : 0) | (si.chroma_on ? 2 : 0); })) return -1;
        if (search_lists(b)) return -1;
        return 0;
    }

    int emit() {
        MARK(KS_SCAN_SEARCH);
        launch_layout(st, a);
        MARK(KS_LAYOUT);
        launch_exclusive_scan(st, b->out.d_img_size_pad.p, b->out.d_img_off.p, uint64_t(nimg), b->enc.d_scan_tmp.p, b->enc.d_scan_tmp.n);
        MARK(KS_SCAN_IMAGES);
        launch_emit(st, a);
        MARK(KS_EMIT);
        return 0;
    }

    int finish(bool phases) {
        CSH_CHECK(hipStreamSynchronize(st));
        CSH_CHECK(hipGetLastError());
        if (t && marks.read(t, phases)) return -1;
        if (t && !phases) t->n_images = uint32_t(nimg);
        return 0;
    }

    int webp() {
        const int nwimg = int(b->wp.wimgs.size());
        uint64_t out_bytes = 0;
        std::vector<uint64_t> off(size_t(b->nimg) + 1, 0);
        for (auto &wi : b->wp.wimgs) {
            const uint64_t cap = 4096 + uint64_t(wi.mbw) * wi.mbh * (b->wp.webp_mb_bytes + 2);
            wi.out_cap = uint32_t(std::min<uint64_t>(cap, 0xFFFFFF00u)); wi.out_off = out_bytes;
            off[wi.image] = out_bytes;
            out_bytes += (wi.out_cap + 63) & ~uint64_t(63);
            const int q = int(b->params.webp_quality);
            wi.quality = q < 0 ? 0 : q > 100 ? 100 : q;
        }
        off[b->nimg] = out_bytes;
        if (b->out.d_out.n < out_bytes + 64 && b->out.d_out.alloc(out_bytes + 64)) return -1;
        if ((b->wp.d_wscratch.n < out_bytes + 64 && b->wp.d_wscratch.alloc(out_bytes + 64)) || (b->wp.d_wpart.n < size_t(b->nimg) * 9 + 9 && b->wp.d_wpart.alloc(size_t(b->nimg) * 9 + 9)) ||
            (b->wp.d_wstats.n < size_t(b->nimg) * 2112 + 8 && (b->wp.d_wstats.alloc(size_t(b->nimg) * 2112 + 8) || b->wp.d_wprobs.alloc(size_t(b->nimg) * 1056 + 8) || b->wp.d_wupdate.alloc(size_t(b->nimg) * 1056 + 8))))
            return -1;
        if (b->wp.d_wstats.zero(st)) return -1;
        if (b->wp.d_wimgs.upload(b->wp.wimgs, st) || (b->wp.d_wwork.n < b->wp.wwork_bytes + 64 && b->wp.d_wwork.alloc(b->wp.wwork_bytes + 64)) ||
            (b->wp.d_wlevels.n < b->wp.wlevels + 64 && b->wp.d_wlevels.alloc(b->wp.wlevels + 64)))
            return -1;
        CSH_CHECK(hipMemcpyAsync(b->out.d_img_off.p, off.data(), off.size() * sizeof(uint64_t), hipMemcpyHostToDevice, st));
        if (b->out.d_img_size.zero(st)) return -1;
        csw::launch_webp_yuv(st, b->wp.d_wimgs.p, nwimg, b->wp.wmax_luma, b->pix.d_rgb.p, b->wp.d_wwork.p);
        MARK(KS_WEBP_YUV);
        hipEvent_t mid;
        if (marks.claim(KS_WEBP_ENCODE, &mid)) return -1;
        if (csw::launch_webp_encode(st, b->wp.wimgs.data(), nwimg, b->wp.d_wimgs.p, b->wp.d_wwork.p, b->wp.d_wlevels.p, b->wp.d_wscratch.p, b->wp.d_wpart.p, b->out.d_out.p, b->out.d_img_size.p, b->out.d_status.p, mid)) return -1;
        MARK(KS_WEBP_ASSEMBLE);
        return finish(false);
    }
};

}

int run_once(csh_batch *b, csh_timing *t, bool requant_only) {
    Run r(b, t);
    b->enc.last_run_fused = 0; b->enc.last_run_refine = 0; b->enc.last_run_ac_lists = 0;
    if (r.pools() || r.marks.start()) return -1;
    const bool from_pixels = requant_only && b->tr.dering;
    if (requant_only && !from_pixels) {
        if (r.requant()) return -1;
    } else {
        if (from_pixels ? r.skip_decode() : r.decode()) return -1;
        if (r.planes()) return -1;
        if (b->webp) return r.webp();
        if (b->rgb_out) return (r.marks.mark(KS_XFORM_DIRECT) || r.finish(false)) ? -1 : 0;
        if (r.pixels()) return -1;
    }
    if (r.encode_begin()) return -1;
    b->enc.last_run_fused = r.fused ? b->enc.n_fused : 0u;
    b->enc.last_run_ac_lists = r.fused ? b->enc.n_ac_lists : 0u;
    if (b->tr.trellis ? r.trellis() : r.marks.skip_to(KS_NZLIST)) return -1;
    r.fill_asm_ctx();
    if (r.stage(b->enc.stage[0], true, false)) return -1;
    if (b->enc.search && r.search()) return -1;
    return (r.emit() || r.finish(true)) ? -1 : 0;
}

}
```

caesium-clt_amd/csrc/k_aclist.hip:

```cpp
#include "kernels.h"
#include "wave.h"

namespace csh {

#define CSH_LP_WORDS 1024

__device__ __forceinline__ static uint32_t lbitlen(uint32_t v) { return 32u - uint32_t(__clz(v)); }
__device__ __forceinline__ static int lwave() { return int(threadIdx.x) / CSP_WAVE_THREADS; }

#define CSH_NZ_HALF 16
__device__ __forceinline__ static uint4 nz_load(const EncCtx &c, const NzSet &S, uint32_t u, int bx, int by, uint32_t oct) {
    uint4 q; q.x = q.y = q.z = q.w = 0u;
    if (u < S.nunits) {
        const int b = by * S.bw + bx;
        q = *reinterpret_cast<const uint4 *>(c.coef + (size_t(S.tile_base) + size_t(b >> 6)) * CSH_TILE_I16 + size_t((b & 63) * CSH_BLK_STRIDE) + size_t(oct) * CSH_OCT_STRIDE);
    }
    return q;
}
__device__ __forceinline__ static uint32_t nz_mask8(const uint4 &q, uint32_t oct) {
    uint32_t m = 0;
    m |= (q.x & 0xFFFFu) ? 1u : 0u;   m |= (q.x >> 16) ? 2u : 0u;
    m |= (q.y & 0xFFFFu) ? 4u : 0u;   m |= (q.y >> 16) ? 8u : 0u;
    m |= (q.z & 0xFFFFu) ? 16u : 0u;  m |= (q.z >> 16) ? 32u : 0u;
    m |= (q.w & 0xFFFFu) ? 64u : 0u;  m |= (q.w >> 16) ? 128u : 0u;
// ... 156 lines not shown
    for (uint32_t g0 = 0; g0 < n0; g0 += 256) {
        LV<uint32_t> e0, e1, e2, e3;
        LFOR(l) {
            const uint32_t g = g0 + 4u * uint32_t(l);
            uint4 e; e.x = e.y = e.z = e.w = 0u;
            if (g < n0) e = *reinterpret_cast<const uint4 *>(src + g);
            e0[l] = e.x; e1[l] = e.y; e2[l] = e.z; e3[l] = e.w;
        }
        for (int L = Lfirst; L < CSH_NZ_LEVELS; L++) {
            if (!okL[L]) continue;
            LV<uint32_t> k4;
            LFOR(l) k4[l] = kept(e0[l], L) + kept(e1[l], L) + kept(e2[l], L) + kept(e3[l], L);
            uint32_t tot;
            const LV<uint32_t> ex = lscan(k4, tot);
            LFOR(l) {
                const uint32_t e[4] = {e0[l], e1[l], e2[l], e3[l]};
                uint32_t o = runL[L] + ex[l];
                CSH_UNROLL
                for (int q = 0; q < 4; q++)
                    if (kept(e[q], L)) dstL[L][o++] = (e[q] & 0xFF8000FFu) | ((((e[q] >> 8) & 0x7FFFu) >> L) << 8);
            }
            runL[L] += tot;
        }
    }
    if (okL[0]) {
        const uint32_t na = (n0new + 3u) & ~3u;
        LFOR(l) {
            if (n0new + uint32_t(l) < na) dstL[0][n0new + uint32_t(l)] = 0u;
            if (l == 0) c.nz_chunk_cnt[L0.chunk0 + ch.j] = n0new;
        }
    }
}

__global__ void __launch_bounds__(256) k_nz_to_tiles(const NzSet *nzsets, const NzList *nzlists, const uint32_t *nz_pool, const uint32_t *nz_chunk_off, const uint32_t *nz_chunk_cnt, uint32_t set,
                                                      int16_t *coef) {
    const NzSet S = nzsets[set];
    const NzList L0 = nzlists[S.list[0]];
    const uint32_t j = blockIdx.x, u0 = j * 256u;
    CSH_PHASE_LOOP(2) {
        if (phase == 0) {
            const uint32_t u = u0 + threadIdx.x;
            if (u >= S.nunits) continue;
            const int by = int(u) / S.real_bw, bx = int(u) - by * S.real_bw;
            int16_t *blk = coef + coef_index(S.tile_base, by * S.bw + bx, 0);
            uint4 z; z.x = z.y = z.z = z.w = 0u;
            z.x = uint32_t(uint16_t(blk[0]));
            CSH_UNROLL
            for (int o = 0; o < 8; o++) { *reinterpret_cast<uint4 *>(blk + CSH_OCT_STRIDE * o) = z; z.x = 0u; }
            continue;
        }
        const uint32_t n = nz_chunk_cnt[L0.chunk0 + j];
        const uint32_t *src = nz_pool + L0.base + nz_chunk_off[L0.chunk0 + j];
        for (uint32_t i = threadIdx.x; i < n; i += 256u) {
            const uint32_t e = src[i], k = e & 127u, u = u0 + ((e >> 23) & 255u);
            if (k == 0u || k >= CSH_NZ_END || u >= S.nunits) continue;
            const int by = int(u) / S.real_bw, bx = int(u) - by * S.real_bw, m = int((e >> 8) & 0x7FFFu);
            coef[coef_index(S.tile_base, by * S.bw + bx, int(k))] = int16_t((e & 128u) ? -m : m);
        }
    }
}
void launch_nz_to_tiles(hipStream_t st, const NzSet *nzsets, const NzList *nzlists, const uint32_t *nz_pool, const uint32_t *nz_chunk_off, const uint32_t *nz_chunk_cnt, uint32_t set,
                        uint32_t nchunks, int16_t *coef) {
    if (nchunks) CSH_LAUNCH_PHASED(k_nz_to_tiles, 2, dim3(nchunks), dim3(256), st, nzsets, nzlists, nz_pool, nz_chunk_off, nz_chunk_cnt, set, coef);
}

struct NzEvent { uint32_t coded, term, run, size, bits, has, eob, blk; };
__device__ __forceinline__ static NzEvent nz_event(uint32_t e, uint32_t p, uint32_t Ss, uint32_t Se) {
    NzEvent v;
    const uint32_t k = e & 127u, pk = p & 127u;
    const bool same = !(p & CSH_NZ_END);
    const bool pin = same && pk >= Ss;
    v.coded = (k >= Ss && k <= Se) ? 1u : 0u;
    v.term = (k > Se && !(same && pk > Se)) ? 1u : 0u;
    v.run = k - (pin ? pk + 1u : Ss);
    const uint32_t m = (e >> 8) & 0x7FFFu;
    v.size = lbitlen(m);
    v.bits = ((e & 128u) ? ~m : m) & ((1u << v.size) - 1u);
    v.has = pin ? 1u : 0u;
    v.eob = (pin && pk == Se) ? 0u : 1u;
    v.blk = (e >> 23) & 255u;
    return v;
}
struct ListSlot { const uint32_t *lst; uint32_t n; };
__device__ __forceinline__ static ListSlot list_of_slot(const EncCtx &c, const SlotRec &r) {
    ListSlot s;
    s.n = c.nz_chunk_cnt[r.nzrec];
    s.lst = c.nz_pool + c.nzlists[r.nzlist].base + c.nz_chunk_off[r.nzrec];
    return s;
}
__device__ __forceinline__ static void list_load4(const ListSlot &s, uint32_t g, uint32_t &e0, uint32_t &e1, uint32_t &e2, uint32_t &e3) {
    uint4 q; q.x = q.y = q.z = q.w = 0u;
    if (g < s.n) q = *reinterpret_cast<const uint4 *>(s.lst + g);
    e0 = q.x; e1 = q.y; e2 = q.z; e3 = q.w;
}

__global__ void __launch_bounds__(256) k_list_stats(EncCtx c) {
    CSH_SHARED uint32_t s_hist[4][4][256];
    CSH_SHARED uint32_t s_flag[4][16];
    const int wv = lwave();
    const uint32_t idx = blockIdx.x * 4u + uint32_t(wv);
    if (idx >= c.nlist_slots) return;
    const uint32_t cs = c.list_slots[idx];
    const SlotRec r = c.slots[cs];
    if (c.work_active && !c.work_active[r.work]) return;
    const ListSlot ls = list_of_slot(c, r);
    uint32_t *hist = &s_hist[wv][0][0], *flag = s_flag[wv];
    LFOR(l) { for (int i = l; i < 1024; i += 64) hist[i] = 0u; if (l < 16) flag[l] = 0u; }
    CSP_WAVE_SYNC();
    const uint32_t Ss = r.Ss, Se = r.Se;
    uint32_t carry = CSH_NZ_END;
    LV<uint32_t> raw;
    LFOR(l) raw[l] = 0u;
    LV<uint32_t> x0, x1, x2, x3;
    LFOR(l) list_load4(ls, 4u * uint32_t(l), x0[l], x1[l], x2[l], x3[l]);
    for (uint32_t g0 = 0; g0 < ls.n; g0 += 256) {
        const LV<uint32_t> e0 = x0, e1 = x1, e2 = x2, e3 = x3;
        if (g0 + 256u < ls.n) LFOR(l) list_load4(ls, g0 + 256u + 4u * uint32_t(l), x0[l], x1[l], x2[l], x3[l]);
        const LV<uint32_t> p0 = lprev(e3, carry);
        carry = llast(e3);
        LFOR(l) {
            uint32_t *h = hist + 256 * (l & 3);
            const uint32_t e[4] = {e0[l], e1[l], e2[l], e3[l]}, p[4] = {p0[l], e0[l], e1[l], e2[l]};
            CSH_UNROLL
            for (int q = 0; q < 4; q++) {
                const NzEvent v = nz_event(e[q], p[q], Ss, Se);
                if (v.coded) {
                    atomicAdd(&h[((v.run & 15u) << 4) | v.size], 1u);
                    if (v.run >> 4) atomicAdd(&h[0xF0], v.run >> 4);
                    raw[l] += v.size;
                } else if (v.term) {
                    if (v.has) atomicOr(&flag[v.blk >> 5], 1u << (v.blk & 31u));
                    if (v.eob) atomicOr(&flag[8u + (v.blk >> 5)], 1u << (v.blk & 31u));
                }
            }
        }
    }
    CSP_WAVE_SYNC();
    const uint32_t rawbits = lsum32(raw);
    LFOR(l) {
        for (int i = l; i < 256; i += 64) {
            const uint32_t v = hist[i] + hist[256 + i] + hist[512 + i] + hist[768 + i];
            c.slot_hist[size_t(r.hist_row) * 256u + uint32_t(i)] = uint16_t(v);
            if (v) atomicAdd(&c.tables[r.table_base].freq[i], v);
        }
        if (l == 0) c.slot_raw[cs] = rawbits;
        if (l < 4 && r.j * 4u + uint32_t(l) < ((r.nunits_work + 63u) >> 6)) {
            c.sym_bits[r.word_base + r.j * 4u + uint32_t(l)] = uint64_t(flag[2 * l]) | (uint64_t(flag[2 * l + 1]) << 32);
            c.eob_bits[r.word_base + r.j * 4u + uint32_t(l)] = uint64_t(flag[8 + 2 * l]) | (uint64_t(flag[9 + 2 * l]) << 32);
        }
    }
}

__device__ __forceinline__ static void lor_bits(uint32_t *words, uint64_t pos, uint32_t v, uint32_t n) {
    v &= n >= 32 ? 0xFFFFFFFFu : ((1u << n) - 1u);
    const uint64_t t = uint64_t(v) << (64u - n - uint32_t(pos & 31u));
    const uint32_t hi = uint32_t(t >> 32), lo = uint32_t(t);
    if (hi) atomicOr(words + (pos >> 5), hi);
    if (lo) atomicOr(words + (pos >> 5) + 1, lo);
}
__global__ void __launch_bounds__(256) k_list_pack(EncCtx c) {
    CSH_SHARED uint32_t s_win[4][CSH_LP_WORDS];
    CSH_SHARED uint32_t s_lut[4][256];
    CSH_SHARED uint16_t s_eob[4][256];
    const int wv = lwave();
    const uint32_t idx = blockIdx.x * 4u + uint32_t(wv);
    if (idx >= c.nlist_slots) return;
    const uint32_t cs = c.list_slots[idx];
    const SlotRec r = c.slots[cs];
    if (c.work_active && !c.work_active[r.work]) return;
    const ScanWork &w = c.work[r.work];
    if (w.no_room) { LFOR(l) if (l == 0) c.status[w.image] = 20200; return; }
    const ListSlot ls = list_of_slot(c, r);
    const uint64_t scan0 = c.chunk_off[r.first_chunk];
    const uint64_t raw_bit0 = w.raw_off * 8 + (c.chunk_off[cs] - scan0);
    uint32_t pad = 0;
    if (r.j == r.nch - 1) { const uint64_t total = c.chunk_off[r.first_chunk + r.nch] - scan0; pad = uint32_t((8 - (total & 7)) & 7); }
    uint32_t *buf = s_win[wv], *lut = s_lut[wv];
    uint16_t *eobrun = s_eob[wv];
    LFOR(l) {
        for (int i = l; i < 256; i += 64) {
            lut[i] = c.tables[r.table_base].lut[i];
            eobrun[i] = uint32_t(i) < r.nun ? c.eobrun[r.unit0 + uint32_t(i)] : uint16_t(0);
        }
        for (int i = l; i < CSH_LP_WORDS; i += 64) buf[i] = 0u;
    }
    CSP_WAVE_SYNC();
    uint32_t *out = c.raw + (raw_bit0 >> 5);
    uint64_t pos = raw_bit0 & 31u;
    uint32_t ww = 0;
    bool first_flush = true;
    const uint32_t Ss = r.Ss, Se = r.Se;
    const uint32_t zrl = lut[0xF0], zc = zrl & 0xFFFFu, zl = zrl >> 16;
    uint32_t carry = CSH_NZ_END;
    const uint32_t n_ext = ls.n + (pad ? 1u : 0u);
    LV<uint32_t> x0, x1, x2, x3;
    LFOR(l) list_load4(ls, 4u * uint32_t(l), x0[l], x1[l], x2[l], x3[l]);
    for (uint32_t g0 = 0; g0 < n_ext; g0 += 256) {
        const LV<uint32_t> e0 = x0, e1 = x1, e2 = x2, e3 = x3;
        if (g0 + 256u < n_ext) LFOR(l) list_load4(ls, g0 + 256u + 4u * uint32_t(l), x0[l], x1[l], x2[l], x3[l]);
        const LV<uint32_t> p0 = lprev(e3, carry);
        carry = llast(e3);
        LV<uint32_t> v0, v1, v2, v3, n0, n1, n2, n3, z, len;
        LFOR(l) {
            const uint32_t e[4] = {e0[l], e1[l], e2[l], e3[l]}, p[4] = {p0[l], e0[l], e1[l], e2[l]};
            uint32_t v[4], n[4], zz = 0, ln = 0;
            CSH_UNROLL
            for (int q = 0; q < 4; q++) {
                v[q] = 0; n[q] = 0;
                const uint32_t g = g0 + 4u * uint32_t(l) + uint32_t(q);
                const NzEvent ev = nz_event(e[q], p[q], Ss, Se);
                if (g >= ls.n) { if (pad && g == ls.n) { v[q] = (1u << pad) - 1u; n[q] = pad; } }
                else if (ev.coded) {
                    const uint32_t t = lut[((ev.run & 15u) << 4) | ev.size];
                    v[q] = ((t & 0xFFFFu) << ev.size) | ev.bits; n[q] = (t >> 16) + ev.size;
                    zz |= (ev.run >> 4) << (2 * q);
                    ln += (ev.run >> 4) * zl;
                } else if (ev.term) {
                    const uint32_t run = eobrun[ev.blk];
                    if (run) {
                        const uint32_t nb = lbitlen(run) - 1u, t = lut[nb << 4];
                        v[q] = ((t & 0xFFFFu) << nb) | (run & ((1u << nb) - 1u)); n[q] = (t >> 16) + nb;
                    }
                }
                ln += n[q];
            }
            v0[l] = v[0]; v1[l] = v[1]; v2[l] = v[2]; v3[l] = v[3]; n0[l] = n[0]; n1[l] = n[1]; n2[l] = n[2]; n3[l] = n[3]; z[l] = zz; len[l] = ln;
        }
        uint32_t tot;
        const LV<uint32_t> ex = lscan(len, tot);
        LFOR(l) {
            uint64_t at = pos + ex[l] - uint64_t(ww) * 32u;
            const uint32_t v[4] = {v0[l], v1[l], v2[l], v3[l]}, n[4] = {n0[l], n1[l], n2[l], n3[l]};
            CSH_UNROLL
            for (int q = 0; q < 4; q++) {
                for (uint32_t t = (z[l] >> (2 * q)) & 3u; t; t--) { lor_bits(buf, at, zc, zl); at += zl; }
                if (n[q]) { lor_bits(buf, at, v[q], n[q]); at += n[q]; }
            }
        }
        pos += tot;
        const uint32_t done = uint32_t(pos >> 5) - ww;
        if (done > CSH_LP_WORDS - 640) {
            CSP_WAVE_SYNC();
            LFOR(l) for (uint32_t q = uint32_t(l); q < done; q += 64) {
                const uint32_t v = buf[q];
                if (first_flush && q == 0) { if (v) atomicOr(out + ww, v); } else out[ww + q] = v;
            }
            const uint32_t partial = buf[done];
            CSP_WAVE_SYNC();
            LFOR(l) for (int q = l; q < CSH_LP_WORDS; q += 64) buf[q] = (q == 0) ? partial : 0u;
            CSP_WAVE_SYNC();
            ww += done; first_flush = false;
        }
    }
    CSP_WAVE_SYNC();
    const uint32_t last = uint32_t((pos + 31) >> 5) - ww;
    LFOR(l) for (uint32_t q = uint32_t(l); q < last; q += 64) {
        const uint32_t v = buf[q];
        if ((first_flush && q == 0) || q == last - 1) { if (v) atomicOr(out + ww + q, v); } else out[ww + q] = v;
    }
}

struct RefCarry { uint32_t runH, runN, base, prevN, prevNZ; };
__device__ __forceinline__ static uint32_t ref_isN(uint32_t e, uint32_t Ss, uint32_t Se) { const uint32_t k = e & 127u; return (k >= Ss && k <= Se && ((e >> 8) & 0x7FFFu) == 1u) ? 1u : 0u; }
__device__ __forceinline__ static uint32_t ref_isH(uint32_t e, uint32_t Ss, uint32_t Se) { const uint32_t k = e & 127u; return (k >= Ss && k <= Se && ((e >> 8) & 0x7FFFu) >= 2u) ? 1u : 0u; }
__device__ __forceinline__ static uint32_t ref_same(uint32_t key, uint32_t blk) { return (key >> 6) == blk + 1u ? (key & 63u) : 0u; }
template <bool WITH_ZQ>
__device__ __forceinline__ static void ref_step(const LV<uint32_t> (&e)[4], uint32_t Ss, uint32_t Se, RefCarry &C, LV<uint32_t> (&hex)[4], LV<uint32_t> (&z)[4], LV<uint32_t> (&zp)[4],
                                                LV<uint32_t> (&zq)[4]) {
    LV<uint32_t> cnt;
    LFOR(l) {
        uint32_t s = 0;
        CSH_UNROLL
        for (int q = 0; q < 4; q++) s += ref_isH(e[q][l], Ss, Se) | (ref_isN(e[q][l], Ss, Se) << 16);
        cnt[l] = s;
    }
    uint32_t tot;
    const LV<uint32_t> ex = lscan(cnt, tot);
    LV<uint32_t> kb[4];
    LFOR(l) {
        uint32_t ph = C.runH + (ex[l] & 0xFFFFu), pn = C.runN + (ex[l] >> 16);
        CSH_UNROLL
        for (int q = 0; q < 4; q++) {
            kb[q][l] = (e[q][l] & CSH_NZ_END) ? ((ph << 14) | pn) + 1u : 0u;
            hex[q][l] = ph; z[q][l] = pn;
            ph += ref_isH(e[q][l], Ss, Se); pn += ref_isN(e[q][l], Ss, Se);
        }
    }
    C.runH += tot & 0xFFFFu; C.runN += tot >> 16;
    lscan_last4(kb, C.base);
    LFOR(l) {
        CSH_UNROLL
        for (int q = 0; q < 4; q++) {
            const uint32_t b = kb[q][l] ? kb[q][l] - 1u : 0u, blk = (e[q][l] >> 23) & 255u, nz = ref_isH(e[q][l], Ss, Se) | ref_isN(e[q][l], Ss, Se);
            const uint32_t h = hex[q][l] - (b >> 14), n = z[q][l] - (b & 0x3FFFu);
            hex[q][l] = h;
            z[q][l] = nz ? (e[q][l] & 127u) - Ss - h - n : 0u;
            const uint32_t key = ((blk + 1u) << 6) | z[q][l];
            zp[q][l] = ref_isN(e[q][l], Ss, Se) ? key : 0u;
            if (WITH_ZQ) zq[q][l] = nz ? key : 0u;
        }
    }
    lscan_last4(zp, C.prevN);
    if (WITH_ZQ) lscan_last4(zq, C.prevNZ);
    LFOR(l) {
        CSH_UNROLL
        for (int q = 0; q < 4; q++) {
            const uint32_t blk = (e[q][l] >> 23) & 255u;
            zp[q][l] = ref_same(zp[q][l], blk);
            if (WITH_ZQ) zq[q][l] = ref_same(zq[q][l], blk);
        }
    }
}
__global__ void __launch_bounds__(256) k_list_refine(EncCtx c) {
    CSH_SHARED uint32_t s_hist[4][4][256];
    CSH_SHARED uint32_t s_lastn[4][256];
    CSH_SHARED uint32_t s_nh[4][256];
    CSH_SHARED uint32_t s_corr[4][256][2];
    const int wv = lwave();
    const uint32_t idx = blockIdx.x * 4u + uint32_t(wv);
    if (idx >= c.nref_slots) return;
    const uint32_t cs = c.ref_slots[idx];
    const SlotRec r = c.slots[cs];
    if (c.work_active && !c.work_active[r.work]) return;
    const ListSlot ls = list_of_slot(c, r);
    uint32_t *hist = &s_hist[wv][0][0], *lastn = s_lastn[wv], *nh = s_nh[wv], *corr = &s_corr[wv][0][0];
    LFOR(l) {
        for (int i = l; i < 1024; i += 64) hist[i] = 0u;
        for (int i = l; i < 256; i += 64) { lastn[i] = 0u; nh[i] = 0u; corr[2 * i] = 0u; corr[2 * i + 1] = 0u; }
    }
    CSP_WAVE_SYNC();
    const uint32_t Ss = r.Ss, Se = r.Se;
    RefCarry C;
    C.runH = C.runN = C.base = C.prevN = C.prevNZ = 0u;
    LV<uint32_t> ntok;
    LFOR(l) ntok[l] = 0u;
    {
        LV<uint32_t> x[4];
        LFOR(l) list_load4(ls, 4u * uint32_t(l), x[0][l], x[1][l], x[2][l], x[3][l]);
        for (uint32_t g0 = 0; g0 < ls.n; g0 += 256) {
            LV<uint32_t> e[4], hex[4], z[4], zp[4], zq[4];
            LFOR(l) { e[0][l] = x[0][l]; e[1][l] = x[1][l]; e[2][l] = x[2][l]; e[3][l] = x[3][l]; }
            if (g0 + 256u < ls.n) LFOR(l) list_load4(ls, g0 + 256u + 4u * uint32_t(l), x[0][l], x[1][l], x[2][l], x[3][l]);
            ref_step<false>(e, Ss, Se, C, hex, z, zp, zq);
            LFOR(l) {
                uint32_t *h = hist + 256 * (l & 3);
                CSH_UNROLL
                for (int q = 0; q < 4; q++) {
                    const uint32_t v = e[q][l], blk = (v >> 23) & 255u;
                    if (ref_isH(v, Ss, Se)) {
                        atomicMax(&nh[blk], hex[q][l] + 1u);
                        if (v & 0x100u) atomicOr(&corr[2u * blk + (hex[q][l] >> 5)], 0x80000000u >> (hex[q][l] & 31u));
                    } else if (ref_isN(v, Ss, Se)) {
                        const uint32_t zr = z[q][l] - zp[q][l];
                        atomicMax(&lastn[blk], ((v & 127u) << 6) | hex[q][l]);
                        atomicAdd(&h[((zr & 15u) << 4) | 1u], 1u);
                        if (zr >> 4) atomicAdd(&h[0xF0], zr >> 4);
                        ntok[l] += 1u + (zr >> 4);
                    }
                }
            }
        }
    }
    CSP_WAVE_SYNC();
    for (uint32_t w4 = 0; w4 < 4; w4++) {
        LFOR(l) {
            const uint32_t i = 64u * w4 + uint32_t(l);
            if (i < r.nun) {
                const uint32_t ln = lastn[i];
                if (ls.n && (ln >> 6) != Se) ntok[l] += 1u;
                c.tail[r.unit0 + i] = uint8_t(nh[i] - (ln & 63u));
                c.corr[r.corr0 + i] = (uint64_t(corr[2u * i]) << 32) | corr[2u * i + 1u];
            }
        }
        const uint64_t ms = lballot([&](int j) { const uint32_t i = 64u * w4 + uint32_t(j); return i < r.nun && lastn[i] != 0u; });
        const uint64_t me = lballot([&](int j) { const uint32_t i = 64u * w4 + uint32_t(j); return i < r.nun && (lastn[i] >> 6) != Se; });
        LFOR(l) if (l == 0 && r.j * 4u + w4 < ((r.nunits_work + 63u) >> 6)) { c.sym_bits[r.word_base + r.j * 4u + w4] = ms; c.eob_bits[r.word_base + r.j * 4u + w4] = me; }
    }
    const uint32_t total = lsum32(ntok);
    LFOR(l) {
        for (int i = l; i < 256; i += 64) {
            const uint32_t v = hist[i] + hist[256 + i] + hist[512 + i] + hist[768 + i];
            c.slot_hist[size_t(r.hist_row) * 256u + uint32_t(i)] = uint16_t(v);
            if (v) atomicAdd(&c.tables[r.table_base].freq[i], v);
        }
        if (l == 0) c.slot_raw[cs] = C.runN + C.runH;
    }
    if (c.stats_only) return;
    const TokRegion rg = c.regions[r.region];
    uint32_t rel = 0;
    LFOR(l) if (l == 0) rel = atomicAdd(&c.tok_cursor[r.region], total);
    rel = uni(rel);
    const bool ok = uint64_t(rel) + total <= rg.cap;
    LFOR(l) {
        if (l < 4) { c.tok_off[cs * 4u + uint32_t(l)] = rg.base + rel; c.chunk_ntok[cs * 4u + uint32_t(l)] = (ok && l == 0) ? total : 0u; }
        if (l == 0 && !ok) c.overflow[1] = 1;
    }
    if (!ok) return;
    uint32_t *tk = c.tokens + rg.base + rel;
    C.runH = C.runN = C.base = C.prevN = C.prevNZ = 0u;
    uint32_t curc = 0, at = 0;
    for (uint32_t g0 = 0; g0 < ls.n; g0 += 256) {
        LV<uint32_t> e[4], hex[4], z[4], zp[4], zq[4], cur[4], nt;
        LFOR(l) list_load4(ls, g0 + 4u * uint32_t(l), e[0][l], e[1][l], e[2][l], e[3][l]);
        ref_step<true>(e, Ss, Se, C, hex, z, zp, zq);
        LFOR(l) {
            uint32_t s = 0;
            CSH_UNROLL
            for (int q = 0; q < 4; q++) {
                const uint32_t v = e[q][l], blk = (v >> 23) & 255u, lastk = lastn[blk] >> 6, isN = ref_isN(v, Ss, Se);
                uint32_t nz = 0, n = 0;
                if ((isN | ref_isH(v, Ss, Se)) && (v & 127u) <= lastk) { nz = ((z[q][l] - zp[q][l]) >> 4) - ((zq[q][l] - zp[q][l]) >> 4); n = nz + isN; }
                cur[q][l] = n ? ((blk + 1u) << 6) | hex[q][l] : 0u;
                if ((v & CSH_NZ_END) && lastk != Se) n = 1u;
                zq[q][l] = nz | (n << 8);
                s += n;
            }
            nt[l] = s;
        }
        lscan_last4(cur, curc);
        uint32_t tot;
        const LV<uint32_t> ex = lscan(nt, tot);
        LFOR(l) {
            uint32_t o = at + ex[l];
            CSH_UNROLL
            for (int q = 0; q < 4; q++) {
                const uint32_t v = e[q][l], blk = (v >> 23) & 255u, nz = zq[q][l] & 255u, n = zq[q][l] >> 8;
                if (!n) continue;
                const uint32_t cu = ref_same(cur[q][l], blk);
                if (v & CSH_NZ_END) {
                    if (o < total) tk[o] = TK_EOB | (blk << 3) | ((nh[blk] - cu) << 16) | (cu << 22);
                    o++;
                    continue;
                }
                uint32_t cnt = hex[q][l] - cu, from = cu;
                for (uint32_t t = 0; t < nz; t++) {
                    if (o < total) tk[o] = TK_REF | (blk << 3) | (cnt << 16) | (from << 22) | (1u << 28);
                    o++; cnt = 0u; from = hex[q][l];
                }
                if (n > nz) {
                    if (o < total) tk[o] = TK_REF | (blk << 3) | (((z[q][l] - zp[q][l]) & 15u) << 11) | ((v & 128u) ? 0u : (1u << 15)) | (cnt << 16) | (from << 22);
                    o++;
                }
            }
        }
        at += tot;
    }
#ifdef CSH_EMUL
    if (at != total) { fprintf(stderr, "k_list_refine: pass 2 made %u tokens, pass 1 counted %u\n", at, total); abort(); }
#endif
}

__global__ void k_reset_works(ScanWork *work, int nwork) {
    const int j = int(blockIdx.x * blockDim.x + threadIdx.x);
    if (j >= nwork) return;
    work[j].out_off = 0xFFFFFFFFu; work[j].raw_bytes = 0; work[j].hdr_bytes = 0; work[j].ff_bytes = 0; work[j].no_room = 0;
}

void launch_nzlist(hipStream_t st, const EncCtx &c) {
    if (!c.nnzchunks) return;
    if (c.nz_build) CSH_LAUNCH_PHASED(k_nzlist, 3, dim3(c.nnzchunks), dim3(2 * CSP_WAVE_THREADS), st, c);
    if (c.nz_filter) CSH_LAUNCH(k_nzfilter, dim3(c.nnzchunks), dim3(CSP_WAVE_THREADS), st, c);
}
void launch_list_stats(hipStream_t st, const EncCtx &c) { if (c.nlist_slots) CSH_LAUNCH(k_list_stats, dim3((c.nlist_slots + 3) / 4), dim3(4 * CSP_WAVE_THREADS), st, c); }
void launch_list_refine(hipStream_t st, const EncCtx &c) { if (c.nref_slots) CSH_LAUNCH(k_list_refine, dim3((c.nref_slots + 3) / 4), dim3(4 * CSP_WAVE_THREADS), st, c); }
void launch_list_pack(hipStream_t st, const EncCtx &c) { if (c.nlist_slots) CSH_LAUNCH(k_list_pack, dim3((c.nlist_slots + 3) / 4), dim3(4 * CSP_WAVE_THREADS), st, c); }
__global__ void __launch_bounds__(64) k_make_slots(const ScanWork *works, uint32_t nworks, const EncScan *script, const NzList *nzlists, SlotRec *slots, uint32_t *slot_work, uint32_t *list_slots,
                                                   uint32_t *tok_slots, uint32_t *ref_slots) {
    const uint32_t wi = blockIdx.x;
    if (wi >= nworks) return;
    const ScanWork &w = works[wi];
    const EncScan &e = script[w.scan];
    const uint32_t nch = (w.nunits + 255u) / 256u;
    const bool prog_ac = e.Ss > 0 && !e.sequential, has_list = w.list != 0xFFFFFFFFu;
    const bool ref_list = has_list && prog_ac && e.Ah;
    const bool listed = has_list && !ref_list;
    for (uint32_t j = threadIdx.x; j < nch; j += blockDim.x) {
        SlotRec r;
        r.work = wi; r.j = j; r.nch = nch; r.first_chunk = w.first_chunk; r.unit0 = w.unit_base + 256u * j;
        r.nun = w.nunits - 256u * j < 256u ? w.nunits - 256u * j : 256u; r.table_base = w.table_base; r.ntables = uint16_t(e.ntables);
        r.flags = uint16_t((prog_ac ? 1 : 0) | (prog_ac && e.Ah ? 2 : 0) | (listed ? 4 : 0) | (ref_list ? 8 : 0));
        r.hist_row = w.hist_row0 + j * uint32_t(e.ntables);
        r.word_base = w.word_base; r.unit_base = w.unit_base; r.nunits_work = w.nunits;
        r.Ss = uint8_t(e.Ss); r.Se = uint8_t(e.Se); r.Ah = uint8_t(e.Ah); r.Al = uint8_t(e.Al); r.corr0 = w.corr_base == 0xFFFFFFFFu ? 0u : w.corr_base + 256u * j;
        r.nzlist = has_list ? w.list : 0u; r.nzrec = has_list ? nzlists[w.list].chunk0 + j : 0u; r.region = ref_list ? w.region : 0u;
        slots[w.first_chunk + j] = r;
        slot_work[w.first_chunk + j] = wi;
        (listed ? list_slots : tok_slots)[w.ls_base + j] = w.first_chunk + j;
        if (ref_list) ref_slots[w.rs_base + j] = w.first_chunk + j;
    }
}
__global__ void __launch_bounds__(64) k_rebind_slots(const ScanWork *works, uint32_t nworks, const NzList *nzlists, SlotRec *slots) {
    const uint32_t wi = blockIdx.x;
    if (wi >= nworks) return;
    const ScanWork &w = works[wi];
    if (w.list == 0xFFFFFFFFu) return;
    const uint32_t nch = (w.nunits + 255u) / 256u, chunk0 = nzlists[w.list].chunk0;
    for (uint32_t j = threadIdx.x; j < nch; j += blockDim.x) { slots[w.first_chunk + j].nzlist = w.list; slots[w.first_chunk + j].nzrec = chunk0 + j; }
}
void launch_rebind_slots(hipStream_t st, const ScanWork *works, uint32_t nworks, const NzList *nzlists, SlotRec *slots) {
    if (nworks) CSH_LAUNCH(k_rebind_slots, dim3(nworks), dim3(64), st, works, nworks, nzlists, slots);
}
void launch_make_slots(hipStream_t st, const ScanWork *works, uint32_t nworks, const EncScan *script, const NzList *nzlists, SlotRec *slots, uint32_t *slot_work, uint32_t *list_slots,
                       uint32_t *tok_slots, uint32_t *ref_slots) {
    if (!nworks) return;
    CSH_LAUNCH(k_make_slots, dim3(nworks), dim3(64), st, works, nworks, script, nzlists, slots, slot_work, list_slots, tok_slots, ref_slots);
}

void launch_reset_works(hipStream_t st, ScanWork *work, int nwork) { if (nwork) CSH_LAUNCH(k_reset_works, dim3((nwork + 255) / 256), dim3(256), st, work, nwork); }

}
```

caesium-clt_amd/csrc/kernels.h:

```cpp
#pragma once
#include "gpu_rt.h"
#include "types.h"

namespace csh {

__host__ __device__ static inline int coef_off(int k) { return (k >> 3) * CSH_OCT_STRIDE + (k & 7); }
__host__ __device__ static inline size_t coef_index(uint32_t tile_base, int b, int k) {
    return (size_t(tile_base) + size_t(b >> 6)) * CSH_TILE_I16 + size_t((b & 63) * CSH_BLK_STRIDE) + size_t(coef_off(k));
}

#define CSH_RAW_OCT 8
__host__ __device__ static inline size_t raw_index(uint32_t tile_base, int b) { return size_t(tile_base) * CSH_TILE_I16 + size_t(b) * 64; }

__device__ __forceinline__ static int csh_plane_at(const uint8_t *p, int pitch, int cw, int ch, int y, int x) {
    y = y < 0 ? 0 : (y > ch - 1 ? ch - 1 : y);
    x = x < 0 ? 0 : (x > cw - 1 ? cw - 1 : x);
    return p[size_t(y) * pitch + x];
}
__device__ __forceinline__ static int csh_upsample_at(const uint8_t *p, int pitch, int cw, int ch, UpDesc u, int r, int xx) {
    switch (u.cls) {
    case CSH_UP_COPY: return csh_plane_at(p, pitch, cw, ch, r, xx);
    case CSH_UP_H2V1: {
        const int cx = xx >> 1, nb = (xx & 1) ? cx + 1 : cx - 1;
        return (3 * csh_plane_at(p, pitch, cw, ch, r, cx) + csh_plane_at(p, pitch, cw, ch, r, nb) + ((xx & 1) ? 2 : 1)) >> 2;
    }
    case CSH_UP_H1V2: {
        const int cy = r >> 1, fy = (r & 1) ? cy + 1 : cy - 1;
        return (3 * csh_plane_at(p, pitch, cw, ch, cy, xx) + csh_plane_at(p, pitch, cw, ch, fy, xx) + ((r & 1) ? 2 : 1)) >> 2;
    }
    case CSH_UP_H2V2: {
        const int cy = r >> 1, cx = xx >> 1, fy = (r & 1) ? cy + 1 : cy - 1, nb = (xx & 1) ? cx + 1 : cx - 1;
        const int cs = 3 * csh_plane_at(p, pitch, cw, ch, cy, cx) + csh_plane_at(p, pitch, cw, ch, fy, cx);
        const int cn = 3 * csh_plane_at(p, pitch, cw, ch, cy, nb) + csh_plane_at(p, pitch, cw, ch, fy, nb);
        return (3 * cs + cn + ((xx & 1) ? 7 : 8)) >> 4;
    }
    default: return csh_plane_at(p, pitch, cw, ch, r / int(u.vx), xx / int(u.hx));
    }
}

void launch_decode_seq(hipStream_t st, const uint8_t *bits, ImgDesc *imgs, const DecScan *scans, const DevHuffSet *huffs,
                       int16_t *coef, int nimg, const uint32_t *need_seq);

void launch_unstuff_count(hipStream_t st, const uint8_t *raw, const ParScan *ps, int nps, uint32_t nchunks, uint32_t *cnt);
void launch_unstuff_copy(hipStream_t st, const uint8_t *raw, uint8_t *clean, ParScan *ps, int nps, uint32_t nchunks, const uint64_t *off);
struct DenseArgs {
    const uint8_t *clean; const ParScan *pss; const void *huffs; int compact;
    uint64_t *state; uint32_t *nblk; uint64_t *list_out; uint32_t *cnt_out;
    uint16_t *hyp; const uint32_t *scan_pending;
    const uint64_t *blk_off; const ImgDesc *imgs; int16_t *coef; int32_t *dcdiff; uint32_t *need_seq;
    uint32_t *cut_block;
    uint8_t *zero_ptr; uint64_t zero_bytes;
    uint8_t *zero2_ptr; uint64_t zero2_bytes;
};
void launch_dec_dense(hipStream_t st, int mode , int nps, uint32_t max_sub, const DenseArgs &a);
void launch_dec_relax_list(hipStream_t st, const uint8_t *clean, const ParScan *ps, uint32_t total_sub, const void *huffs, int compact, uint64_t *state, uint32_t *nblk,
                           const uint64_t *list_in, const uint32_t *cnt_in, uint64_t *list_out, uint32_t *cnt_out, size_t nstate, uint32_t *claim, uint32_t epoch);
void launch_refine_chains(hipStream_t st, const uint8_t *clean, const ParScan *pss, const ParHuffSet *huffs, const DecScan *scans, const ProgChain *chains,
                          const int *chain_scans, int nchains, const RefineUnit *units, int nunits, uint32_t max_blocks, const ImgDesc *imgs, int16_t *coef,
                          uint32_t *need_seq, uint64_t *hist, uint32_t *posv, uint32_t *prog);
void launch_rebind_slots(hipStream_t st, const ScanWork *works, uint32_t nworks, const NzList *nzlists, SlotRec *slots);
void launch_make_slots(hipStream_t st, const ScanWork *works, uint32_t nworks, const EncScan *script, const NzList *nzlists, SlotRec *slots, uint32_t *slot_work, uint32_t *list_slots,
                       uint32_t *tok_slots, uint32_t *ref_slots);
void launch_decode_prog(hipStream_t st, const uint8_t *clean, const ParScan *pss, const ParHuffSet *huffs, const DecScan *scans, const ProgChain *chains,
                        const int *chain_scans, int nchains, const ImgDesc *imgs, int16_t *coef, uint32_t *need_seq);
void launch_dec_mark_pending(hipStream_t st, const ParScan *ps, uint32_t total_sub, const uint64_t *list_in, const uint32_t *cnt_in, uint32_t *scan_pending);
void launch_dec_chain(hipStream_t st, const ParScan *ps, int nps, uint64_t *state, uint32_t *nblk, const uint16_t *hyp, const uint32_t *scan_pending, uint32_t *need_seq);
void launch_dc_refine(hipStream_t st, const uint8_t *clean, const ParScan *ps, int nps, uint32_t max_blocks, const ImgDesc *imgs, int16_t *coef, const uint32_t *need_seq);
void launch_dc_scatter(hipStream_t st, const ParScan *ps, int nps, uint32_t max_blocks, const ImgDesc *imgs, const uint64_t *dc_off, int16_t *coef,
                       const uint32_t *need_seq, const uint32_t *cut_block);

struct NzFuse {
    const NzSet *nzsets; const NzList *nzlists;
    uint32_t *nz_pool, *nz_cursor, *nz_chunk_off, *nz_chunk_cnt;
    uint8_t *blk_cnt; uint16_t *blk_off;
    uint32_t *overflow;
};
void launch_xform_direct(hipStream_t st, const ImgDesc *imgs, const PlaneWork *work, int nwork, int max_tiles, const DevQuant *quant,
                         const int16_t *coef_in, int16_t *coef_out, int16_t *dct_raw, uint32_t raw_tile0, bool dering, const NzFuse &nzf);
void launch_requant(hipStream_t st, const ImgDesc *imgs, const PlaneWork *work, int nwork, int max_tiles, const DevQuant *quant, const int16_t *dct_raw,
                    uint32_t raw_tile0, int16_t *coef_out);
void launch_idct_plane(hipStream_t st, const ImgDesc *imgs, const PlaneWork *work, int nwork, int max_tiles, const DevQuant *quant,
                       const int16_t *coef_in, uint8_t *planes);
void launch_resample_plane(hipStream_t st, const ImgDesc *imgs, const PlaneWork *work, int nwork, uint32_t max_quads, const uint8_t *planes, uint8_t *oplanes);
void launch_plane_fdct(hipStream_t st, const ImgDesc *imgs, const PlaneWork *work, int nwork, int max_tiles, const DevQuant *quant,
                       const uint8_t *oplanes, int16_t *coef_out, int16_t *dct_raw, uint32_t raw_tile0, bool dering, const NzFuse &nzf);
void launch_resample_fdct_420(hipStream_t st, const ImgDesc *imgs, const PlaneWork *work, int nwork, int max_tiles, const DevQuant *quant,
                              const uint8_t *planes, int16_t *coef_out, int16_t *dct_raw, uint32_t raw_tile0, bool dering, const NzFuse &nzf);
void launch_resample_any(hipStream_t st, const ImgDesc *imgs, const PlaneWork *work, int nwork, uint32_t max_quads, const uint8_t *planes, uint8_t *oplanes);
void launch_fix_dummy(hipStream_t st, const ImgDesc *imgs, int nimg, int max_blocks, int16_t *coef_out);

bool resize_is_fused(uint32_t max_row_in);
void launch_resize(hipStream_t st, const ImgDesc *imgs, const ResizeWork *work, int nwork, const ResizeTap *taps, const float *weights,
                   uint8_t *planes, uint8_t *rgb, float *tmp, uint32_t max_src_px, uint64_t max_tmp, uint64_t max_dst, uint32_t max_row_in, uint32_t max_out_w, uint32_t max_nh, bool to_planes,
                   bool any_layout = false);

struct EncCtx {
    const ImgDesc *imgs;
    const EncScan *script;
    const ScanWork *work;
    int nwork;
    const EChunk *echunks;
    uint32_t nechunks;
    const TokPlan *plans;
    const uint32_t *slot_work;
    const SlotRec *slots;
    uint32_t slot0, nslots;
    const int16_t *coef;
    uint64_t *sym_bits;
    uint64_t *eob_bits;
    uint8_t *tail;
    uint16_t *eobrun;
    uint32_t *long_runs, *long_cnt;
    uint64_t *corr;
    uint32_t *tokens;
    const TokRegion *regions;
    uint32_t *tok_cursor;
    uint64_t *tok_off;
    uint32_t *chunk_ntok;
    uint16_t *slot_hist;
    uint32_t *slot_raw;
    uint32_t *slot_eobh;
    uint32_t *chunk_bits;
    const uint64_t *chunk_off;
    DevEncTable *tables;
    uint32_t *raw;
    uint64_t raw_words;
    uint32_t *status;
    uint32_t *overflow;
    uint32_t debug;
    uint32_t stats_only;
    const uint8_t *work_active;
    const NzList *nzlists;
    const NzSet *nzsets;
    const NzChunk *nzchunks;
    uint32_t nnzchunks;
    uint32_t *nz_pool;
    uint32_t *nz_cursor;
    uint32_t *nz_chunk_off;
    uint32_t *nz_chunk_cnt;
    uint8_t *nz_blk_cnt;
    uint16_t *nz_blk_off;
    const uint32_t *list_slots;
    uint32_t nlist_slots;
    const uint32_t *tok_slots;
    uint32_t ntok_slots;
    const uint32_t *ref_slots;
    uint32_t nref_slots;
    uint32_t nz_build, nz_filter;
};
enum : uint32_t { TK_SYM = 0u, TK_RAW = 1u, TK_ACF = 2u, TK_REF = 3u, TK_EOB = 4u };
void launch_tokens(hipStream_t st, const EncCtx &c);
void launch_ac_runs(hipStream_t st, const EncCtx &c);
void launch_gen_tables(hipStream_t st, DevEncTable *tables, int ntables);
void launch_chunk_sizes(hipStream_t st, const EncCtx &c);
void launch_zero_edges(hipStream_t st, const EncCtx &c);
void launch_pack(hipStream_t st, const EncCtx &c);
void launch_nzlist(hipStream_t st, const EncCtx &c);
void launch_list_stats(hipStream_t st, const EncCtx &c);
void launch_list_refine(hipStream_t st, const EncCtx &c);
void launch_list_pack(hipStream_t st, const EncCtx &c);
void launch_nz_to_tiles(hipStream_t st, const NzSet *nzsets, const NzList *nzlists, const uint32_t *nz_pool, const uint32_t *nz_chunk_off, const uint32_t *nz_chunk_cnt,
                        uint32_t set, uint32_t nchunks, int16_t *coef);
void launch_reset_works(hipStream_t st, ScanWork *work, int nwork);

#ifndef CSH_TR_WG
#define CSH_TR_WG 256
#endif
#ifndef CSH_TR_RUN
#define CSH_TR_RUN 8
#endif
struct TrellisCtx {
    const ImgDesc *imgs;
    const DevQuant *quant;
    const TrellisWork *work;
    int nwork;
    const TrellisRun *runs;
    uint32_t nruns;
    uint32_t *queue;
    uint32_t nslots;
    const DevEncTable *tables;
    const int16_t *raw;
    uint32_t raw_tile0;
    int16_t *coef;
    uint64_t *dcrec;
    uint64_t *dcbt;
    uint32_t *spill;
    uint32_t max_rows;
    const uint8_t *blk_cnt;
    uint32_t *perm;
    const uint32_t *rows;
    uint32_t nrows;
    uint32_t debug;
    uint32_t *nz_pool;
    const NzList *nzlists;
    const NzSet *nzsets;
    const uint32_t *nz_chunk_off, *nz_chunk_cnt;
    const uint16_t *blk_off;
    uint32_t ac_lists;
};
void launch_trellis_sort(hipStream_t st, const TrellisCtx &c);
void launch_trellis_ac(hipStream_t st, const TrellisCtx &c);
void launch_trellis_dc(hipStream_t st, const TrellisCtx &c);
uint32_t trellis_ac_slots();
size_t trellis_spill_words(uint32_t nslots);

void launch_exclusive_scan(hipStream_t st, const uint32_t *in, uint64_t *out, uint64_t n, void *tmp, size_t tmp_bytes);
size_t exclusive_scan_tmp_bytes(uint64_t n);

struct AsmCtx {
    const ImgDesc *imgs;
    const EncScan *script;
    ScanWork *work;
    int nwork, nimg, scans_per_image;
    int work0, nwork_run;
    const uint32_t *img_list;
    const uint32_t *img_nlist;
    uint32_t *scan_cost;
    const DevEncTable *tables;
    const uint64_t *chunk_off;
    uint32_t *scan_pad_bytes;
    uint64_t *scan_raw_off;
    const uint32_t *raw;
    uint64_t raw_chunks;
    uint32_t *chunk_ff;
    const uint8_t *hdr_pool;
    const uint32_t *hdr_off;
    uint32_t *img_size_pad;
    uint32_t *img_size;
    uint64_t *img_off;
    uint8_t *out;
    uint64_t out_cap;
    uint32_t *status;
    uint32_t *overflow;
};
void launch_scan_cost(hipStream_t st, const AsmCtx &a);
void launch_scan_sizes(hipStream_t st, const AsmCtx &a);
void launch_scan_place(hipStream_t st, const AsmCtx &a);
void launch_ff_count(hipStream_t st, const AsmCtx &a);
void launch_layout(hipStream_t st, const AsmCtx &a);
void launch_emit(hipStream_t st, const AsmCtx &a);

}
```

caesium-clt_amd/csrc/pipeline.cpp:

```cpp
#include <algorithm>
#include <atomic>
#include <cmath>
#include <cstdarg>
#include <memory>
#include <thread>

#include "batch.hpp"
#include "../../include/vp8_tables.h"
#include "resize_host.h"

static thread_local char g_err[512];
void csh_set_error(const char *fmt, ...) {
    va_list ap;
    va_start(ap, fmt);
    vsnprintf(g_err, sizeof g_err, fmt, ap);
    va_end(ap);
}
extern "C" const char *csh_last_error(void) { return g_err; }

#ifdef CSH_EMUL
thread_local dim3 threadIdx, blockIdx, blockDim, gridDim;
int csh_emul_reverse = 0;
thread_local int csh_emul_phase = 0;
extern "C" void csh_emul_set_reverse(int r) { csh_emul_reverse = r; }
// ... 142 lines not shown
    if (b->lossless) { csh_set_error("retain_dct: a coefficient transcode has no quality to re-target"); return -1; }
    b->retain_dct = on != 0;
    if (b->retain_dct && b->nimg && b->pix.d_dct_raw.n == 0 && b->pix.d_dct_raw.alloc(size_t(b->ntiles_out) * CSH_TILE_I16)) return -1;
    return 0;
}
extern "C" int csh_batch_set_quality(csh_batch *b, const uint32_t *quality) {
    if (b->lossless) { csh_set_error("set_quality on a lossless batch"); return -1; }
    b->enc.hdr_pool.clear(); b->enc.hdr_off.clear();
    for (size_t n = 0; n < b->items.size(); n++) {
        Item &it = b->items[n];
        if (it.image < 0) continue;
        ImgDesc &im = b->imgs[it.image];
        if (quality[n]) {
            int q = int(quality[n]) < 1 ? 1 : (quality[n] > 100 ? 100 : int(quality[n]));
            for (int c = 0; c < im.ncomp; c++) im.qt_out[c] = b->q_base + q;
        }
        JpegInfo hdr = it.out;
        int qidx = im.qt_out[0];
        uint16_t nat[64];
        for (int k = 0; k < 64; k++) nat[kZigZag[k]] = b->quants[qidx].q[k];
        memcpy(hdr.qt[0], nat, 128); memcpy(hdr.qt[1], nat, 128);
        std::vector<uint8_t> fh = build_frame_header(hdr, b->progressive, it.meta_out.empty() ? nullptr : &it.meta_out);
        b->enc.hdr_off.push_back(uint32_t(b->enc.hdr_pool.size()));
        b->enc.hdr_pool.insert(b->enc.hdr_pool.end(), fh.begin(), fh.end());
    }
    b->enc.hdr_off.push_back(uint32_t(b->enc.hdr_pool.size()));
    if (!b->nimg) return 0;
    if (hipSetDevice(b->device) != hipSuccess) return -1;
    if (b->d_imgs.upload(b->imgs, b->stream) || b->enc.d_hdr.upload(b->enc.hdr_pool, b->stream) || b->enc.d_hdr_off.upload(b->enc.hdr_off, b->stream)) return -1;
    CSH_CHECK(hipStreamSynchronize(b->stream));
    return 0;
}
extern "C" int csh_batch_rerun_encode(csh_batch *b, csh_timing *t) {
    if (!b->have_dct) { csh_set_error("rerun_encode needs a completed csh_batch_run after csh_batch_retain_dct(1)"); return -1; }
    return batch_run(b, t, true);
}

static int batch_run(csh_batch *b, csh_timing *t, bool requant_only) {
    if (t) memset(t, 0, sizeof *t);
    if (!b->nimg) { b->out.ran = true; return 0; }
    if (hipSetDevice(b->device) != hipSuccess) { csh_set_error("hipSetDevice failed"); return CS_ERR_NO_DEVICE; }
    for (int attempt = 0; attempt < 4; attempt++) {
        if (run_once(b, t, requant_only)) return CS_ERR_NO_DEVICE;
        uint32_t ovf[4] = {0, 0, 0, 0};
        if (csh_copy_wait(ovf, b->out.d_overflow.p, sizeof ovf, hipMemcpyDeviceToHost, b->stream) != hipSuccess) { csh_set_error("D2H failed"); return CS_ERR_NO_DEVICE; }
        b->out.h_status.resize(b->nimg);
        if (csh_copy_wait(b->out.h_status.data(), b->out.d_status.p, b->nimg * sizeof(uint32_t), hipMemcpyDeviceToHost, b->stream) != hipSuccess) return CS_ERR_NO_DEVICE;
        bool pool = ovf[0] != 0;
        if (ovf[1]) {
            pool = true; b->enc.tok_scale *= 4;
            layout_token_pool(b);
            if (b->enc.d_regions.upload(b->enc.regions, b->stream) || b->enc.d_nzlists.upload(b->enc.nzlists, b->stream) || hipStreamSynchronize(b->stream) != hipSuccess) return CS_ERR_NO_DEVICE;
        }
        for (uint32_t s : b->out.h_status) if (s == CS_ERR_POOL_OVERFLOW) pool = true;
        if (!pool) break;
        if (attempt == 3) { csh_set_error("device pools overflowed after 3 retries"); return CS_ERR_POOL_OVERFLOW; }
        b->out.raw_bytes_cap *= 4; b->out.out_cap = b->out.raw_bytes_cap;
        b->wp.webp_mb_bytes *= 4;
    }
    b->out.h_img_size.resize(b->nimg);
    b->out.h_img_off.resize(b->nimg + 1);
    if (csh_copy_wait(b->out.h_img_size.data(), b->out.d_img_size.p, b->nimg * sizeof(uint32_t), hipMemcpyDeviceToHost, b->stream) != hipSuccess ||
        csh_copy_wait(b->out.h_img_off.data(), b->out.d_img_off.p, (b->nimg + 1) * sizeof(uint64_t), hipMemcpyDeviceToHost, b->stream) != hipSuccess) {
        csh_set_error("D2H of sizes failed"); return CS_ERR_NO_DEVICE;
    }
    if (t) {
        std::vector<uint32_t> ns(b->nimg);
        if (csh_copy_wait(ns.data(), b->dec.d_need_seq.p, b->nimg * sizeof(uint32_t), hipMemcpyDeviceToHost, b->stream) != hipSuccess) return CS_ERR_NO_DEVICE;
        if (getenv("CSH_TRACE") && b->dec.d_relax_cnt.n) {
            std::vector<uint32_t> rc(b->dec.d_relax_cnt.n);
            if (csh_copy_wait(rc.data(), b->dec.d_relax_cnt.p, rc.size() * sizeof(uint32_t), hipMemcpyDeviceToHost, b->stream) == hipSuccess) {
                fprintf(stderr, "[csh] relax list sizes (of %u sub-sequences):", b->dec.total_sub);
                for (size_t i = 0; i < rc.size() && (i < 16 || rc[i]); i++) fprintf(stderr, " %u", rc[i]);
                fprintf(stderr, "\n");
            }
        }
        for (const ProgChain &pc : b->dec.chains) if (pc.refine && ns[size_t(pc.image)] == 4) t->n_refine_chains++;
        for (uint32_t v : ns) { if (v == 4) { t->n_prog_decoded++; continue; } if (v) t->n_seq_decoded++; if (v == 2 || v == 3) t->n_par_fallback++; if (v == 3) t->n_par_short++; }
        t->n_images = uint32_t(b->nimg);
        t->n_search_extra = b->enc.search ? b->enc.n_gated_runs : 0u;
        t->n_fused_lists = b->enc.last_run_fused;
        t->n_list_refine = b->enc.last_run_refine;
        t->n_ac_in_lists = b->enc.last_run_ac_lists;
        for (const Item &it : b->items) if (it.image < 0) t->n_failed++;
        for (int i = 0; i < b->nimg; i++) { t->out_bytes += b->out.h_img_size[i]; t->pixels += uint64_t(b->imgs[i].width) * b->imgs[i].height; }
        t->in_bytes = b->dec.bits_pool.size();
        uint64_t in_tiles = 0;
        for (const ImgDesc &im : b->imgs) for (int c = 0; c < im.ncomp; c++) in_tiles += im.in[c].ntiles;
        t->coef_bytes = in_tiles * CSH_TILE_I16 * 2;
    }
    b->out.ran = true;
    if (!requant_only) b->have_dct = (b->retain_dct || b->tr.trellis) && !b->lossless;
    return 0;
}

static void set_result(CCSResult *r, int code, const std::string &msg) {
    r->success = code == 0;
    r->code = uint32_t(code);
    r->error_message = nullptr;
    if (code) { char *m = (char *)malloc(msg.size() + 1); memcpy(m, msg.c_str(), msg.size() + 1); r->error_message = m; }
}

extern "C" int csh_batch_pixels(csh_batch *b, size_t image, const uint8_t **device_pixels, uint32_t *width, uint32_t *height, uint32_t *channels, const char **message) {
    *device_pixels = nullptr; *width = *height = *channels = 0;
    if (message) *message = "";
    if (!b || !b->out.ran || !b->rgb_out || image >= b->items.size()) { csh_set_error("csh_batch_pixels: not a pixel batch that has run"); if (message) *message = "not a pixel batch that has run"; return CS_ERR_NO_DEVICE; }
    const Item &it = b->items[image];
    if (it.code) { if (message) *message = it.msg.c_str(); return it.code; }
    if (b->out.h_status[it.image]) { if (message) *message = "device reported a malformed stream"; return int(b->out.h_status[it.image]); }
    if (size_t(it.image) < b->pix.rwork.size() && b->pix.rwork[size_t(it.image)].image == it.image) {
        const ResizeWork &rw = b->pix.rwork[size_t(it.image)];
        *device_pixels = b->pix.d_rgb.p + rw.rgb_dst_off; *width = uint32_t(rw.nw); *height = uint32_t(rw.nh); *channels = uint32_t(b->imgs[it.image].ncomp);
        return 0;
    }
    if (message) *message = "image has no pixel output";
    return CS_ERR_NO_DEVICE;
}

extern "C" int csh_batch_fetch(csh_batch *b, CByteArray *outputs, CCSResult *results) {
    if (!b->out.ran) { csh_set_error("csh_batch_fetch before csh_batch_run"); return -1; }
    if (b->rgb_out) { csh_set_error("csh_batch_fetch: a pixel batch has no files (csh_batch_pixels)"); return -1; }
    struct PinnedOut { uint8_t *p = nullptr; size_t cap = 0; ~PinnedOut() { if (p) pinned_cache().put(p, cap); } uint8_t *data() const { return p; } } host;
    if (b->nimg && b->out.h_img_off[b->nimg]) {
        host.p = static_cast<uint8_t *>(pinned_cache().get(b->out.h_img_off[b->nimg], host.cap));
        if (!host.p) { csh_set_error("out of pinned host memory"); return -1; }
        if (csh_copy_wait(host.p, b->out.d_out.p, b->out.h_img_off[b->nimg], hipMemcpyDeviceToHost, b->stream) != hipSuccess) { csh_set_error("D2H of output failed"); return -1; }
    }
    std::atomic<int> failed{0};
    std::atomic<size_t> next{0};
    auto worker = [&]() {
        for (size_t n; (n = next++) < b->items.size();) {
            Item &it = b->items[n];
            outputs[n].data = nullptr; outputs[n].length = 0;
            int code = it.code;
            std::string msg = it.msg;
            if (!code && it.image >= 0 && b->out.h_status[it.image]) { code = int(b->out.h_status[it.image]); msg = "device reported a malformed stream"; }
            if (!code) {
                size_t len = b->out.h_img_size[it.image];
                outputs[n].data = (uint8_t *)malloc(len ? len : 1);
                memcpy(outputs[n].data, host.data() + b->out.h_img_off[it.image], len);
                outputs[n].length = len;
            } else failed++;
            if (results) set_result(&results[n], code, msg);
        }
    };
    size_t nthreads = std::min<size_t>(std::min<size_t>(8, std::max(1u, std::thread::hardware_concurrency())), b->items.size() / 64 + 1);
    std::vector<std::thread> pool;
    for (size_t t = 1; t < nthreads; t++) pool.emplace_back(worker);
    worker();
    for (auto &t : pool) t.join();
    return failed.load();
}

extern "C" int csh_batch_geometry(csh_batch *b, size_t image, int comp, int which, int *bw, int *bh, int *real_bw, int *real_bh) {
    if (image >= b->items.size() || b->items[image].image < 0) { csh_set_error("image not on the device"); return -1; }
    const ImgDesc &im = b->imgs[b->items[image].image];
    if (comp < 0 || comp >= im.ncomp) { csh_set_error("bad component"); return -1; }
    const CompGeom &g = which ? im.out[comp] : im.in[comp];
    *bw = g.bw; *bh = g.bh; *real_bw = g.real_bw; *real_bh = g.real_bh;
    return 0;
}

extern "C" int csh_batch_read_coefs(csh_batch *b, size_t image, int comp, int which, int16_t *dst) {
    int bw, bh, rbw, rbh;
    if (csh_batch_geometry(b, image, comp, which, &bw, &bh, &rbw, &rbh)) return -1;
    const ImgDesc &im = b->imgs[b->items[image].image];
// ... 17 lines not shown
```

caesium-clt_amd/csrc/types.h:

```cpp
#pragma once
#include <cstdint>

#define CSH_TILE_BLOCKS 64
#define CSH_TILE_I16 4096
#ifndef CSH_BLOCK_MAJOR
#define CSH_BLOCK_MAJOR 0
#endif
#if CSH_BLOCK_MAJOR
#define CSH_OCT_STRIDE 8
#define CSH_BLK_STRIDE 64
#else
#define CSH_OCT_STRIDE 512
#define CSH_BLK_STRIDE 8
#endif
#define CSH_MAX_COMPS 3
#define CSH_MASK_PLANES 6
#define CSH_MASK_TILE (CSH_MASK_PLANES * 64)
#define CSH_MAX_SCANS 20
#define CSH_LIST_MAX 16

namespace csh {

struct CompGeom {
    int h, v;
// ... 59 lines not shown

#define CSH_SUBSEQ_BYTES 128
struct ParScan {
    uint32_t bits_off, bits_len;
    uint32_t clean_len;
    int huff_set, image, ncomp;
    int nb_mcu;
    int comp_of[10], by_of[10], bx_of[10], dct[10], act[10];
    uint32_t total_blocks;
    uint32_t sub_base;
    uint32_t par_index;
    uint32_t dc_base[10], dc_per_mcu[10], dc_idx[10];
    uint64_t sel;
    uint32_t first_mcu;
    int kind;
    int Ss, Se, Al;
};
enum { CSH_PS_SEQ = 0, CSH_PS_UNSTUFF = 1, CSH_PS_DC_FIRST = 2, CSH_PS_AC_FIRST = 3, CSH_PS_DC_REFINE = 4 };

struct DevQuant {
    uint16_t q[64];
    int32_t div[64];
    float rcp[64];
    float lt[64];
    uint32_t mul[64];
    uint32_t sh[64];
};

enum { CSH_UP_COPY = 0, CSH_UP_H2V2 = 1, CSH_UP_H2V1 = 2, CSH_UP_H1V2 = 3, CSH_UP_REP = 4 };
enum { CSH_DN_FULL = 0, CSH_DN_H2V2 = 1, CSH_DN_H2V1 = 2, CSH_DN_H4V1 = 3 };
struct UpDesc { uint8_t cls, hx, vx, pad; };

#define CSH_MODE_ANY 11
struct PlaneWork {
    int image, comp;
    int mode;
    UpDesc up;
    int dn;
    uint32_t nzset;
    uint32_t ac_lists;
};

#define CSH_RZ_ANY (-2)
struct ResizeWork {
    int image, in_kind;
    UpDesc up[CSH_MAX_COMPS];
    int nw, nh;
    uint64_t rgb_src_off, rgb_dst_off;
    uint64_t tmp_off;
    uint32_t vtap_base, htap_base;
};
struct ResizeTap { int left, n; uint32_t woff; };

struct EncScan {
    int ncomp, comp[CSH_MAX_COMPS];
    int Ss, Se, Ah, Al;
    int dc_tbl[CSH_MAX_COMPS];
    int ac_tbl[CSH_MAX_COMPS];
    int sequential;
    int ntables;
    int dht_id[4];
    int sos_tdta[CSH_MAX_COMPS];
};

struct ScanWork {
    int image, scan;
    uint32_t nunits;
    uint32_t unit_base;
    uint32_t first_chunk;
    uint32_t word_base;
    uint32_t table_base;
    uint32_t ff_bytes;
    uint64_t raw_off;
    uint32_t raw_bytes;
    uint32_t out_off;
    uint32_t hdr_bytes;
    uint32_t no_room;
    uint32_t list;
    uint32_t corr_base;
    uint32_t hist_row0;
    uint32_t ls_base;
    uint32_t rs_base;
    uint32_t region;
};

struct EChunk { uint32_t a; uint16_t comp, kind; uint32_t j; uint32_t plan; uint32_t region; };
struct TokRegion { uint64_t base; uint32_t cap, pad; };
#define CSH_TK_MAXSLOT 12
struct AcSlot { uint32_t unit_base, word_base, first_chunk, table_base, nunits_work; uint8_t Ss, Se, Ah, Al; uint32_t corr_base, pad; };
struct TokPlan {
    uint32_t nslot, nunits;
    int32_t real_bw, bw;
    uint32_t tile_base;
    uint32_t work0;
    uint32_t pad[2];
    AcSlot s[CSH_TK_MAXSLOT];
};
#define CSH_NZ_END 64u
#define CSH_NZ_LEVELS 4
struct NzList {
    uint64_t base;
    uint32_t cap;
    uint32_t chunk0;
};
struct NzSet {
    uint32_t list[CSH_NZ_LEVELS];
    uint32_t nunits;
    int32_t real_bw, bw;
    uint32_t tile_base;
    uint32_t cnt_base;
    uint32_t pad[3];
};
#define CSH_NZ_COMPACT0 0x80000000u
struct NzChunk { uint32_t set, j, levels, work0; };

struct SlotRec {
    uint32_t work, j, nch;
    uint32_t first_chunk;
    uint32_t unit0, nun;
    uint32_t table_base;
    uint16_t ntables, flags;
    uint32_t hist_row;
    uint32_t word_base, unit_base, nunits_work;
    uint8_t Ss, Se, Ah, Al; uint32_t corr0;
    uint32_t nzlist, nzrec;
    uint32_t region;
};

struct TrellisWork {
    int image, comp;
    uint32_t table_ac;
    int32_t table_dc;
    uint32_t nunits;
    uint32_t unit_base;
    uint32_t nzset;
    uint32_t ac_lists;
};
struct TrellisRun { uint32_t work, j, n; };

struct DevEncTable {
    uint32_t freq[257];
    uint8_t bits[17];
    uint8_t vals[256];
    uint16_t code[256];
    uint8_t size[256];
    int nsym;
    uint32_t lut[256];
};

}
```

include/caesium_hip.h:

```cpp
#ifndef CAESIUM_HIP_H
#define CAESIUM_HIP_H
#include <stdbool.h>
#include <stddef.h>
#include <stdint.h>
#ifdef __cplusplus
extern "C" {
#endif

enum { CS_TYPE_JPEG = 0, CS_TYPE_PNG = 1, CS_TYPE_GIF = 2, CS_TYPE_WEBP = 3, CS_TYPE_TIFF = 4, CS_TYPE_UNKN = 5 };

enum {
    CS_OK = 0,
    CS_ERR_NO_DEVICE = 10001,
    CS_ERR_UNKNOWN_TYPE = 10200,
    CS_ERR_UNSUPPORTED = 10201,
    CS_ERR_BAD_JPEG = 20100,
    CS_ERR_JPEG_FEATURE = 20101,
    CS_ERR_POOL_OVERFLOW = 20200,
    CS_ERR_BAD_PNG = 30100,
    CS_ERR_BAD_WEBP = 40100,
    CS_ERR_SAME_FORMAT = 10407,
    CS_ERR_TOO_BIG = 10500
};

typedef struct {
    bool keep_metadata;
    uint32_t jpeg_quality;
    uint32_t jpeg_chroma_subsampling;
    bool jpeg_progressive;
    bool jpeg_optimize;
    bool jpeg_preserve_icc;
    uint32_t png_quality;
    uint32_t png_optimization_level;
    bool png_force_zopfli;
    bool png_optimize;
    uint32_t gif_quality;
    uint32_t webp_quality;
    bool webp_lossless;
    uint32_t tiff_compression;
    uint32_t tiff_deflate_level;
    uint32_t width;
    uint32_t height;
} CCSParameters;

typedef struct {
    bool success;
    uint32_t code;
    const char *error_message;
} CCSResult;

typedef struct {
    uint8_t *data;
    size_t length;
} CByteArray;

void cs_default_parameters(CCSParameters *p);

CCSResult cs_compress_in_memory(const uint8_t *in, size_t n, const CCSParameters *p, CByteArray *out);
CCSResult cs_compress_to_size_in_memory(const uint8_t *in, size_t n, CCSParameters *p, size_t max_output_size,
                                        bool return_smallest, CByteArray *out);
CCSResult cs_convert_in_memory(const uint8_t *in, size_t n, const CCSParameters *p, uint32_t format, CByteArray *out);
int cs_batch_convert(const CByteArray *inputs, size_t count, const CCSParameters *p, uint32_t format, int device, CByteArray *outputs, CCSResult *results);

int cs_batch_compress(const CByteArray *inputs, size_t count, const CCSParameters *p, int device,
                      CByteArray *outputs, CCSResult *results);
int cs_batch_compress_to_size(const CByteArray *inputs, size_t count, CCSParameters *p, size_t max_output_size, bool return_smallest,
                              int device, CByteArray *outputs, CCSResult *results);

size_t cs_batch_extent(const CByteArray *inputs, size_t count);

void cs_free_bytes(CByteArray *b);
void cs_free_result(CCSResult *r);

typedef struct csh_batch csh_batch;

enum { CSH_NPHASES = 8, CSH_NKERNELS = 36 };
typedef struct {
    float total_ms;
    float phase_ms[CSH_NPHASES];
    float kernel_ms[CSH_NKERNELS];
    uint64_t in_bytes, out_bytes;
    uint64_t pixels;
    uint64_t coef_bytes;
    uint32_t n_images, n_failed;
    uint32_t n_seq_decoded;
    uint32_t n_par_fallback;
    uint32_t n_par_short;
    uint32_t n_prog_decoded;
    uint32_t n_refine_chains;
    uint32_t n_search_extra;
    uint32_t n_fused_lists;
    uint32_t n_list_refine;
    uint32_t n_ac_in_lists;
} csh_timing;

int csh_device_count(void);
const char *csh_last_error(void);
void csh_warmup(int device);
void csh_release_cached_memory(void);
const char *csh_kernel_name(int slot);
const char *csh_kernel_name_webp(int slot);
int csh_batch_create(const CByteArray *inputs, size_t count, const CCSParameters *p, int device, csh_batch **out);
int csh_batch_create_webp(const CByteArray *inputs, size_t count, const CCSParameters *p, int device, csh_batch **out);
int csh_batch_create_pixels(const CByteArray *inputs, size_t count, const CCSParameters *p, int device, csh_batch **out);
int csh_batch_pixels(csh_batch *b, size_t image, const uint8_t **device_pixels, uint32_t *width, uint32_t *height, uint32_t *channels, const char **message);
struct csp_pixels_s;
int csh_batch_create_from_pixels(const struct csp_pixels_s *sources, size_t count, const CCSParameters *p, int device, csh_batch **out);
int csh_batch_run(csh_batch *b, csh_timing *t);
int csh_batch_fetch(csh_batch *b, CByteArray *outputs, CCSResult *results);
void csh_batch_destroy(csh_batch *b);

int csh_batch_retain_dct(csh_batch *b, int on);
int csh_batch_set_quality(csh_batch *b, const uint32_t *quality);
int csh_batch_rerun_encode(csh_batch *b, csh_timing *t);

int csh_batch_geometry(csh_batch *b, size_t image, int comp, int which, int *bw, int *bh, int *real_bw, int *real_bh);
int csh_batch_read_coefs(csh_batch *b, size_t image, int comp, int which, int16_t *dst);

typedef struct csp_batch csp_batch;
enum { CSP_NKERNELS = 16 };
typedef struct {
    float total_ms;
    float kernel_ms[CSP_NKERNELS];
    uint64_t in_bytes, out_bytes;
    uint64_t pixels, raw_bytes;
    uint32_t n_images, n_failed, n_trials;
} csp_timing;
const char *csp_kernel_name(int slot);
int csp_batch_create(const CByteArray *inputs, size_t count, const CCSParameters *p, int device, csp_batch **out);
int csp_batch_create_webp(const CByteArray *inputs, size_t count, const CCSParameters *p, int device, csp_batch **out);
typedef struct csp_pixels_s { const uint8_t *device_pixels; uint32_t width, height, channels; } csp_pixels;
int csp_batch_create_pixels(const csp_pixels *sources, size_t count, const CCSParameters *p, int device, csp_batch **out);
int csp_png_to_jpeg(const CByteArray *inputs, size_t count, const CCSParameters *p, int device, CByteArray *outputs, CCSResult *results);
int csp_png_to_lossless_webp(const CByteArray *inputs, size_t count, const CCSParameters *p, int device, CByteArray *outputs, CCSResult *results);
int csp_batch_run(csp_batch *b, csp_timing *t);
int csp_batch_fetch(csp_batch *b, CByteArray *outputs, CCSResult *results);
void csp_batch_destroy(csp_batch *b);
int csp_batch_geometry(csp_batch *b, size_t image, uint32_t *width, uint32_t *height, uint32_t *rowbytes);
int csp_batch_read_rows(csp_batch *b, size_t image, uint8_t *dst);
int csp_batch_read_stream(csp_batch *b, size_t image, int strategy, uint8_t *dst);
int csp_batch_read_scores(csp_batch *b, size_t image, uint64_t *dst, int *have);
int csp_batch_trials(csp_batch *b, size_t image, int *strategies, uint64_t *zlib_bytes, int *ntrials, int *winner);
int csp_batch_chunk_bits(csp_batch *b, size_t image, int trial, uint64_t *dst, size_t cap, size_t *nchunks);

int csl_encode_pixels(const struct csp_pixels_s *sources, size_t count, int device, CByteArray *outputs, CCSResult *results);
int csl_attach_alpha(CByteArray *lossy, const CByteArray *alpha_vp8l, uint32_t width, uint32_t height);

typedef struct cswd_batch cswd_batch;
int cswd_batch_create(const CByteArray *inputs, size_t count, int device, cswd_batch **out);
int cswd_batch_run(cswd_batch *b);
int cswd_batch_pixels(cswd_batch *b, size_t image, const uint8_t **device_pixels, uint32_t *width, uint32_t *height, uint32_t *channels, const char **message);
int cswd_batch_read_pixels(cswd_batch *b, size_t image, uint8_t *dst );
int cswd_batch_alpha(cswd_batch *b, size_t image, const uint8_t **device_rgba, const uint8_t **device_alpha);
int cswd_batch_read_rgba(cswd_batch *b, size_t image, uint8_t *dst );
void cswd_batch_destroy(cswd_batch *b);
typedef struct cswd_rgba cswd_rgba;
int cswd_rgba_join(const uint8_t *device_rgb, const uint8_t *device_alpha, uint32_t width, uint32_t height, int device, cswd_rgba **out, const uint8_t **device_rgba);
void cswd_rgba_destroy(cswd_rgba *r);
int csh_batch_create_webp_from_pixels(const struct csp_pixels_s *sources, size_t count, const CCSParameters *p, int device, csh_batch **out);
int csh_batch_create_from_pixels_rgb(const struct csp_pixels_s *sources, size_t count, const CCSParameters *p, int device, csh_batch **out);

#ifdef __cplusplus
}
#endif
#endif
```

Baseline: 43990.

## Process runs of consecutive list chunks per wave in list stats, refine and pack

The list-based AC kernels (stats, refine, pack) now have each wave handle a run of up to CSH_LIST_RUN (default 8) consecutive chunks instead of one chunk. Histograms and frequency counts are kept in registers and flushed once per run, which cuts global atomics and per-wave setup. The next chunk's data is prefetched across chunk boundaries. The trade-off is fewer waves in flight, so the GPU may be less fully occupied on small batches.

```diff
diff --git a/caesium-clt_amd/binding.py b/caesium-clt_amd/binding.py
--- a/caesium-clt_amd/binding.py
+++ b/caesium-clt_amd/binding.py
@@ -25,7 +25,7 @@
 
 class Timing(C.Structure):
     _fields_ = [("total_ms", C.c_float), ("phase_ms", C.c_float * NPHASES), ("kernel_ms", C.c_float * NKERNELS), ("in_bytes", C.c_uint64), ("out_bytes", C.c_uint64),
-                ("pixels", C.c_uint64), ("coef_bytes", C.c_uint64), ("n_images", C.c_uint32), ("n_failed", C.c_uint32), ("n_seq_decoded", C.c_uint32), ("n_par_fallback", C.c_uint32), ("n_par_short", C.c_uint32), ("n_prog_decoded", C.c_uint32), ("n_refine_chains", C.c_uint32), ("n_search_extra", C.c_uint32), ("n_fused_lists", C.c_uint32), ("n_list_refine", C.c_uint32), ("n_ac_in_lists", C.c_uint32)]
+                ("pixels", C.c_uint64), ("coef_bytes", C.c_uint64), ("n_images", C.c_uint32), ("n_failed", C.c_uint32), ("n_seq_decoded", C.c_uint32), ("n_par_fallback", C.c_uint32), ("n_par_short", C.c_uint32), ("n_prog_decoded", C.c_uint32), ("n_refine_chains", C.c_uint32), ("n_search_extra", C.c_uint32), ("n_fused_lists", C.c_uint32), ("n_list_refine", C.c_uint32), ("n_ac_in_lists", C.c_uint32), ("n_list_runs", C.c_uint32)]
 
 
 class PngTiming(C.Structure):
diff --git a/caesium-clt_amd/csrc/batch.hpp b/caesium-clt_amd/csrc/batch.hpp
--- a/caesium-clt_amd/csrc/batch.hpp
+++ b/caesium-clt_amd/csrc/batch.hpp
@@ -78,7 +78,7 @@
 };
 
 struct Stage {
-    uint32_t work0 = 0, nwork = 0, slot0 = 0, nslots = 0, ech0 = 0, nech = 0, table0 = 0, ntables = 0, plan0 = 0, nplans = 0, nzc0 = 0, nnzc = 0, ls0 = 0, nls = 0, ts0 = 0, nts = 0, rs0 = 0, nrs = 0;
+    uint32_t work0 = 0, nwork = 0, slot0 = 0, nslots = 0, ech0 = 0, nech = 0, table0 = 0, ntables = 0, plan0 = 0, nplans = 0, nzc0 = 0, nnzc = 0, ls0 = 0, nls = 0, ts0 = 0, nts = 0, rs0 = 0, nrs = 0, lr0 = 0, nlr = 0, rr0 = 0, nrr = 0;
     bool nz_build[2] = {true, true}, nz_filter[2] = {true, true};
 };
 struct SearchImg {
@@ -95,6 +95,9 @@
     uint32_t nslots = 0, nlist_slots = 0, ntok_slots = 0;
     uint32_t nref_slots = 0;
     uint32_t last_run_refine = 0;
+    uint32_t list_run = CSH_LIST_RUN;
+    uint32_t nlist_runs = 0, nref_runs = 0;
+    uint32_t last_run_list_runs = 0;
     uint64_t total_corr = 0;
     uint64_t total_units = 0, total_words = 0;
     uint32_t max_units = 0;
@@ -127,12 +130,12 @@
     Stage stage[ST_N];
     void stage_begin(Stage &sg) {
         sg.work0 = uint32_t(swork.size()); sg.slot0 = nslots; sg.ech0 = uint32_t(echunks.size()); sg.table0 = uint32_t(ntables); sg.plan0 = uint32_t(plans.size());
-        sg.nzc0 = uint32_t(nzchunks.size()); sg.ls0 = nlist_slots; sg.ts0 = ntok_slots; sg.rs0 = nref_slots;
+        sg.nzc0 = uint32_t(nzchunks.size()); sg.ls0 = nlist_slots; sg.ts0 = ntok_slots; sg.rs0 = nref_slots; sg.lr0 = nlist_runs; sg.rr0 = nref_runs;
     }
     void stage_end(Stage &sg) {
         sg.nwork = uint32_t(swork.size()) - sg.work0; sg.nslots = nslots - sg.slot0; sg.nech = uint32_t(echunks.size()) - sg.ech0;
         sg.ntables = uint32_t(ntables) - sg.table0; sg.nplans = uint32_t(plans.size()) - sg.plan0;
-        sg.nnzc = uint32_t(nzchunks.size()) - sg.nzc0; sg.nls = nlist_slots - sg.ls0; sg.nts = ntok_slots - sg.ts0; sg.nrs = nref_slots - sg.rs0;
+        sg.nnzc = uint32_t(nzchunks.size()) - sg.nzc0; sg.nls = nlist_slots - sg.ls0; sg.nts = ntok_slots - sg.ts0; sg.nrs = nref_slots - sg.rs0; sg.nlr = nlist_runs - sg.lr0; sg.nrr = nref_runs - sg.rr0;
     }
     std::vector<SearchImg> simg;
     std::vector<uint8_t> work_active;
@@ -158,7 +161,7 @@
     DevBuf<NzList> d_nzlists;
     DevBuf<NzSet> d_nzsets;
     DevBuf<NzChunk> d_nzchunks, d_nzchunks_fused;
-    DevBuf<uint32_t> d_nz_pool, d_nz_cursor, d_nz_chunk_off, d_nz_chunk_cnt, d_list_slots, d_tok_slots, d_ref_slots;
+    DevBuf<uint32_t> d_nz_pool, d_nz_cursor, d_nz_chunk_off, d_nz_chunk_cnt, d_list_slots, d_tok_slots, d_ref_slots, d_list_runs, d_ref_runs;
 };
 
 struct TrellisPlan {
@@ -275,6 +278,7 @@
     bool fused_420 = true;
     bool nz_fused = true;
     bool ref_list = true;
+    uint32_t list_run = CSH_LIST_RUN;
     bool ac_tiles = false;
     static PlanSwitches read();
 };
diff --git a/caesium-clt_amd/csrc/batch_plan.cpp b/caesium-clt_amd/csrc/batch_plan.cpp
--- a/caesium-clt_amd/csrc/batch_plan.cpp
+++ b/caesium-clt_amd/csrc/batch_plan.cpp
@@ -221,6 +221,7 @@
     const char *pp = getenv("CSH_PROG_PAR");
     s.prog_par = pp && !strcmp(pp, "0") ? 0 : (pp && !strcmp(pp, "1") ? 1 : -1);
     s.fused_420 = !getenv("CSH_NO_FUSED_420");
+    if (const char *lr = getenv("CSH_LIST_RUN")) { if (*lr) s.list_run = uint32_t(std::min(32, std::max(1, atoi(lr)))); }
     return s;
 }
 
@@ -244,6 +245,7 @@
     b->q_base = int(b->quants.size()) - 1;
     for (int q = 1; q <= 100; q++) { uint16_t tq[64]; quality_table(q, tq); DevQuant dq; make_quant(tq, dq); b->quants.push_back(dq); }
     b->progressive = progressive;
+    b->enc.list_run = sw.list_run;
 
     add_script(b->enc.script, 3, true);
     add_script(b->enc.script, 1, true);
@@ -345,7 +347,7 @@
         w.out_off = 0xFFFFFFFFu;
         const bool from_list = e.Ss > 0 && !e.sequential && e.Ah == 0;
         const bool ref_list = sw.ref_list && e.Ss > 0 && !e.sequential && e.Ah != 0;
-        w.list = 0xFFFFFFFFu; w.rs_base = 0xFFFFFFFFu;
+        w.list = 0xFFFFFFFFu; w.rs_base = 0xFFFFFFFFu; w.lr_base = 0xFFFFFFFFu; w.rr_base = 0xFFFFFFFFu;
         if (from_list || ref_list) {
             if (e.Al >= CSH_NZ_LEVELS) { it.code = CS_ERR_JPEG_FEATURE; it.msg = "internal: output scan script outside what the list coder carries"; }
             else {
@@ -372,6 +374,9 @@
             uint32_t &cursor = (from_list && w.list != 0xFFFFFFFFu) ? b->enc.nlist_slots : b->enc.ntok_slots;
             w.ls_base = cursor; cursor += nch;
             if (ref_list && w.list != 0xFFFFFFFFu) { w.rs_base = b->enc.nref_slots; b->enc.nref_slots += nch; }
+            const uint32_t nruns = (nch + b->enc.list_run - 1) / b->enc.list_run;
+            if (from_list && w.list != 0xFFFFFFFFu) { w.lr_base = b->enc.nlist_runs; b->enc.nlist_runs += nruns; }
+            if (ref_list && w.list != 0xFFFFFFFFu) { w.rr_base = b->enc.nref_runs; b->enc.nref_runs += nruns; }
         }
         if (e.Ss == 0 || e.sequential) {
             uint32_t blocks = 0;
@@ -1071,14 +1076,14 @@
         b->enc.d_tok_off.alloc(4 * size_t(b->enc.nslots) + 4) || b->enc.d_chunk_ntok.alloc(4 * size_t(b->enc.nslots) + 4) || b->enc.d_slot_hist.alloc(size_t(b->enc.hist_rows) * 256 + 256) ||
         b->enc.d_slot_raw.alloc(size_t(b->enc.nslots) + 1) || b->enc.d_img_list.upload(b->enc.img_list, st) || b->enc.d_img_nlist.upload(b->enc.img_nlist, st) || b->enc.d_scan_cost.alloc(b->enc.swork.size() + 1) || b->enc.d_slot_eobh.alloc(16 * size_t(b->enc.nslots) + 16) || b->enc.d_chunk_bits.alloc(size_t(b->enc.nslots) + 1) || b->enc.d_chunk_off.alloc(size_t(b->enc.nslots) + 2) || b->enc.d_tok_cursor.alloc(b->enc.region_est.size() + 1) || b->enc.d_regions.upload(b->enc.regions, st) ||
         b->enc.d_tables.alloc(b->enc.ntables) || b->enc.d_scan_pad.alloc(b->enc.swork.size() + 1) ||
-        b->enc.d_nzlists.upload(b->enc.nzlists, st) || b->enc.d_nzsets.upload(b->enc.nzsets, st) || b->enc.d_nzchunks.upload(b->enc.nzchunks, st) || (b->enc.n_fused && b->enc.d_nzchunks_fused.upload(b->enc.nzchunks_fused, st)) || b->enc.d_list_slots.alloc(size_t(b->enc.nlist_slots) + 1) || b->enc.d_tok_slots.alloc(size_t(b->enc.ntok_slots) + 1) || b->enc.d_ref_slots.alloc(size_t(b->enc.nref_slots) + 1) ||
+        b->enc.d_nzlists.upload(b->enc.nzlists, st) || b->enc.d_nzsets.upload(b->enc.nzsets, st) || b->enc.d_nzchunks.upload(b->enc.nzchunks, st) || (b->enc.n_fused && b->enc.d_nzchunks_fused.upload(b->enc.nzchunks_fused, st)) || b->enc.d_list_slots.alloc(size_t(b->enc.nlist_slots) + 1) || b->enc.d_tok_slots.alloc(size_t(b->enc.ntok_slots) + 1) || b->enc.d_ref_slots.alloc(size_t(b->enc.nref_slots) + 1) || b->enc.d_list_runs.alloc(size_t(b->enc.nlist_runs) + 1) || b->enc.d_ref_runs.alloc(size_t(b->enc.nref_runs) + 1) ||
         b->enc.d_nz_cursor.alloc(b->enc.nzlists.size() + 1) || b->enc.d_nz_chunk_off.alloc(size_t(b->enc.nz_nrec) + 1) || b->enc.d_nz_chunk_cnt.alloc(size_t(b->enc.nz_nrec) + 1) ||
         b->enc.d_scan_raw_off.alloc(b->enc.swork.size() + 2) || b->out.d_img_size.alloc(b->nimg + 1) || b->out.d_img_size_pad.alloc(b->nimg + 1) ||
         b->out.d_img_off.alloc(b->nimg + 2) || b->out.d_status.alloc(b->nimg) || b->out.d_overflow.alloc(4))
         return CS_ERR_NO_DEVICE;
     if (hipMemsetAsync(b->enc.d_slots.p, 0, (size_t(b->enc.nslots) + 1) * sizeof(SlotRec), st) != hipSuccess ||
         hipMemsetAsync(b->enc.d_slot_work.p, 0, (size_t(b->enc.nslots) + 1) * sizeof(uint32_t), st) != hipSuccess) { csh_set_error("hipMemsetAsync failed"); return CS_ERR_NO_DEVICE; }
-    launch_make_slots(st, b->enc.d_swork.p, uint32_t(b->enc.swork.size()), b->enc.d_script.p, b->enc.d_nzlists.p, b->enc.d_slots.p, b->enc.d_slot_work.p, b->enc.d_list_slots.p, b->enc.d_tok_slots.p, b->enc.d_ref_slots.p);
+    launch_make_slots(st, b->enc.d_swork.p, uint32_t(b->enc.swork.size()), b->enc.d_script.p, b->enc.d_nzlists.p, b->enc.d_slots.p, b->enc.d_slot_work.p, b->enc.d_list_slots.p, b->enc.d_tok_slots.p, b->enc.d_ref_slots.p, b->enc.d_list_runs.p, b->enc.d_ref_runs.p, b->enc.list_run);
     if (b->tr.trellis && (b->tr.d_trows.upload(b->tr.trows, st) || (b->tr.t_sort && (b->tr.d_tperm.alloc(size_t(b->tr.t_units) + 1) || b->tr.d_tblk_cnt.alloc(size_t(b->tr.t_units) + 1) || (b->tr.nz_once && b->tr.d_tblk_off.alloc(size_t(b->tr.t_units) + 1)))))) return CS_ERR_NO_DEVICE;
     if (b->tr.trellis && (b->tr.d_twork.upload(b->tr.twork, st) || b->tr.d_truns.upload(b->tr.truns, st) || b->tr.d_tqueue.alloc(1) || b->tr.d_tlambda.alloc(size_t(b->tr.t_units) + 1) || b->tr.d_tdcbt.alloc(size_t(b->tr.t_units) + 1) ||
                        b->tr.d_tspill.alloc(trellis_spill_words(trellis_ac_slots())) || b->pix.d_dct_raw.alloc(size_t(b->ntiles_out) * CSH_TILE_I16)))
diff --git a/caesium-clt_amd/csrc/batch_run.cpp b/caesium-clt_amd/csrc/batch_run.cpp
--- a/caesium-clt_amd/csrc/batch_run.cpp
+++ b/caesium-clt_amd/csrc/batch_run.cpp
@@ -255,12 +255,20 @@
         return 0;
     }
 
+    void count_list_runs(const Stage &sg, bool gate) {
+        for (uint32_t wi = sg.work0; (sg.nlr || sg.nrr) && wi < sg.work0 + sg.nwork; wi++) {
+            const ScanWork &w = b->enc.swork[wi];
+            if ((w.lr_base != 0xFFFFFFFFu || w.rr_base != 0xFFFFFFFFu) && (!gate || b->enc.work_active[wi])) b->enc.last_run_list_runs += ((w.nunits + 255u) / 256u + b->enc.list_run - 1u) / b->enc.list_run;
+        }
+    }
+
     void set_stage(const Stage &sg) {
         c.echunks = b->enc.d_echunks.p + sg.ech0; c.nechunks = sg.nech; c.slot0 = sg.slot0; c.nslots = sg.nslots;
         c.nzchunks = (fused ? b->enc.d_nzchunks_fused.p : b->enc.d_nzchunks.p) + sg.nzc0; c.nnzchunks = sg.nnzc;
         c.nz_build = sg.nz_build[fused ? 1 : 0]; c.nz_filter = sg.nz_filter[fused ? 1 : 0];
         c.list_slots = b->enc.d_list_slots.p + sg.ls0; c.nlist_slots = sg.nls; c.tok_slots = b->enc.d_tok_slots.p + sg.ts0; c.ntok_slots = sg.nts;
         c.ref_slots = b->enc.d_ref_slots.p + sg.rs0; c.nref_slots = sg.nrs;
+        c.list_runs = b->enc.d_list_runs.p + sg.lr0; c.nlist_runs = sg.nlr; c.ref_runs = b->enc.d_ref_runs.p + sg.rr0; c.nref_runs = sg.nrr; c.list_run = b->enc.list_run;
     }
 
     int trellis() {
@@ -280,6 +288,7 @@
         }
         launch_tokens(st, c);
         launch_list_stats(st, c);
+        count_list_runs(tg, false);
         launch_ac_runs(st, c);
         launch_gen_tables(st, b->enc.d_tables.p + tg.table0, int(tg.ntables));
         c.stats_only = 0;
@@ -307,6 +316,7 @@
         launch_list_refine(st, c);
         for (uint32_t wi = sg.work0; sg.nrs && wi < sg.work0 + sg.nwork; wi++)
             if (b->enc.swork[wi].rs_base != 0xFFFFFFFFu && (!gate || b->enc.work_active[wi])) b->enc.last_run_refine++;
+        count_list_runs(sg, gate);
         launch_tokens(st, c);
         SMARK(KS_TOKENS);
         launch_list_stats(st, c);
@@ -409,6 +419,7 @@
 
 int run_once(csh_batch *b, csh_timing *t, bool requant_only) {
     Run r(b, t);
+    b->enc.last_run_list_runs = 0;
     b->enc.last_run_fused = 0; b->enc.last_run_refine = 0; b->enc.last_run_ac_lists = 0;
     if (r.pools() || r.marks.start()) return -1;
     const bool from_pixels = requant_only && b->tr.dering;
diff --git a/caesium-clt_amd/csrc/k_aclist.hip b/caesium-clt_amd/csrc/k_aclist.hip
--- a/caesium-clt_amd/csrc/k_aclist.hip
+++ b/caesium-clt_amd/csrc/k_aclist.hip
@@ -262,73 +262,113 @@
     return v;
 }
 struct ListSlot { const uint32_t *lst; uint32_t n; };
-__device__ __forceinline__ static ListSlot list_of_slot(const EncCtx &c, const SlotRec &r) {
+__device__ __forceinline__ static ListSlot list_chunk(const EncCtx &c, uint64_t base, uint32_t rec) {
     ListSlot s;
-    s.n = c.nz_chunk_cnt[r.nzrec];
-    s.lst = c.nz_pool + c.nzlists[r.nzlist].base + c.nz_chunk_off[r.nzrec];
+    s.n = c.nz_chunk_cnt[rec];
+    s.lst = c.nz_pool + base + c.nz_chunk_off[rec];
     return s;
 }
+__device__ __forceinline__ static uint32_t run_chunks(const EncCtx &c, const SlotRec &r) { const uint32_t left = r.nch - r.j; return left < c.list_run ? left : c.list_run; }
 __device__ __forceinline__ static void list_load4(const ListSlot &s, uint32_t g, uint32_t &e0, uint32_t &e1, uint32_t &e2, uint32_t &e3) {
     uint4 q; q.x = q.y = q.z = q.w = 0u;
     if (g < s.n) q = *reinterpret_cast<const uint4 *>(s.lst + g);
     e0 = q.x; e1 = q.y; e2 = q.z; e3 = q.w;
 }
 
+__device__ __forceinline__ static void hist_flush(uint32_t *hist, uint16_t *row, LV<uint32_t> (&freq)[4]) {
+    LFOR(l) {
+        uint4 s; s.x = s.y = s.z = s.w = 0u;
+        CSH_UNROLL
+        for (int cpy = 0; cpy < 4; cpy++) {
+            uint4 *h = reinterpret_cast<uint4 *>(hist + 256 * cpy + 4 * l);
+            const uint4 v = *h;
+            s.x += v.x; s.y += v.y; s.z += v.z; s.w += v.w;
+            uint4 zero; zero.x = zero.y = zero.z = zero.w = 0u;
+            *h = zero;
+        }
+        uint2 o; o.x = (s.x & 0xFFFFu) | (s.y << 16); o.y = (s.z & 0xFFFFu) | (s.w << 16);
+        *reinterpret_cast<uint2 *>(row + 4 * l) = o;
+        freq[0][l] += s.x; freq[1][l] += s.y; freq[2][l] += s.z; freq[3][l] += s.w;
+    }
+}
+__device__ __forceinline__ static void freq_flush(uint32_t *dst, const LV<uint32_t> (&freq)[4]) {
+    LFOR(l) {
+        CSH_UNROLL
+        for (int q = 0; q < 4; q++) if (freq[q][l]) atomicAdd(&dst[4 * l + q], freq[q][l]);
+    }
+}
 __global__ void __launch_bounds__(256) k_list_stats(EncCtx c) {
-    CSH_SHARED uint32_t s_hist[4][4][256];
+    CSH_SHARED alignas(16) uint32_t s_hist[4][4][256];
     CSH_SHARED uint32_t s_flag[4][16];
-    const int wv = lwave();
+    const int wv = int(uni(uint32_t(lwave())));
     const uint32_t idx = blockIdx.x * 4u + uint32_t(wv);
-    if (idx >= c.nlist_slots) return;
-    const uint32_t cs = c.list_slots[idx];
-    const SlotRec r = c.slots[cs];
+    if (idx >= c.nlist_runs) return;
+    const uint32_t cs0 = c.list_runs[idx];
+    const SlotRec r = c.slots[cs0];
     if (c.work_active && !c.work_active[r.work]) return;
-    const ListSlot ls = list_of_slot(c, r);
+    const uint32_t nrun = run_chunks(c, r);
+    const uint64_t lbase = c.nzlists[r.nzlist].base;
+    ListSlot nx = list_chunk(c, lbase, r.nzrec);
     uint32_t *hist = &s_hist[wv][0][0], *flag = s_flag[wv];
-    LFOR(l) { for (int i = l; i < 1024; i += 64) hist[i] = 0u; if (l < 16) flag[l] = 0u; }
+    LFOR(l) {
+        uint4 zero; zero.x = zero.y = zero.z = zero.w = 0u;
+        for (int i = 4 * l; i < 1024; i += 256) *reinterpret_cast<uint4 *>(hist + i) = zero;
+        if (l < 16) flag[l] = 0u;
+    }
     CSP_WAVE_SYNC();
     const uint32_t Ss = r.Ss, Se = r.Se;
-    uint32_t carry = CSH_NZ_END;
-    LV<uint32_t> raw;
-    LFOR(l) raw[l] = 0u;
+    LV<uint32_t> freq[4];
+    LFOR(l) { freq[0][l] = 0u; freq[1][l] = 0u; freq[2][l] = 0u; freq[3][l] = 0u; }
     LV<uint32_t> x0, x1, x2, x3;
-    LFOR(l) list_load4(ls, 4u * uint32_t(l), x0[l], x1[l], x2[l], x3[l]);
-    for (uint32_t g0 = 0; g0 < ls.n; g0 += 256) {
-        const LV<uint32_t> e0 = x0, e1 = x1, e2 = x2, e3 = x3;
-        if (g0 + 256u < ls.n) LFOR(l) list_load4(ls, g0 + 256u + 4u * uint32_t(l), x0[l], x1[l], x2[l], x3[l]);
-        const LV<uint32_t> p0 = lprev(e3, carry);
-        carry = llast(e3);
+    bool ahead = false;
+    for (uint32_t ci = 0; ci < nrun; ci++) {
+        const ListSlot ls = nx;
+        const bool more = ci + 1u < nrun;
+        if (more) nx = list_chunk(c, lbase, r.nzrec + ci + 1u);
+        if (!ahead) LFOR(l) list_load4(ls, 4u * uint32_t(l), x0[l], x1[l], x2[l], x3[l]);
+        ahead = false;
+        uint32_t carry = CSH_NZ_END;
+        LV<uint32_t> raw;
+        LFOR(l) raw[l] = 0u;
+        for (uint32_t g0 = 0; g0 < ls.n; g0 += 256) {
+            const LV<uint32_t> e0 = x0, e1 = x1, e2 = x2, e3 = x3;
+            if (g0 + 256u < ls.n) LFOR(l) list_load4(ls, g0 + 256u + 4u * uint32_t(l), x0[l], x1[l], x2[l], x3[l]);
+            else if (more) { LFOR(l) list_load4(nx, 4u * uint32_t(l), x0[l], x1[l], x2[l], x3[l]); ahead = true; }
+            const LV<uint32_t> p0 = lprev(e3, carry);
+            carry = llast(e3);
+            LFOR(l) {
+                uint32_t *h = hist + 256 * (l & 3);
+                const uint32_t e[4] = {e0[l], e1[l], e2[l], e3[l]}, p[4] = {p0[l], e0[l], e1[l], e2[l]};
+                CSH_UNROLL
+                for (int q = 0; q < 4; q++) {
+                    const NzEvent v = nz_event(e[q], p[q], Ss, Se);
+                    if (v.coded) {
+                        atomicAdd(&h[((v.run & 15u) << 4) | v.size], 1u);
+                        if (v.run >> 4) atomicAdd(&h[0xF0], v.run >> 4);
+                        raw[l] += v.size;
+                    } else if (v.term) {
+                        if (v.has) atomicOr(&flag[v.blk >> 5], 1u << (v.blk & 31u));
+                        if (v.eob) atomicOr(&flag[8u + (v.blk >> 5)], 1u << (v.blk & 31u));
+                    }
+                }
+            }
+        }
+        CSP_WAVE_SYNC();
+        const uint32_t rawbits = lsum32(raw);
+        const uint32_t cs = cs0 + ci, j = r.j + ci, hist_row = r.hist_row + ci * uint32_t(r.ntables);
+        hist_flush(hist, c.slot_hist + size_t(hist_row) * 256u, freq);
         LFOR(l) {
-            uint32_t *h = hist + 256 * (l & 3);
-            const uint32_t e[4] = {e0[l], e1[l], e2[l], e3[l]}, p[4] = {p0[l], e0[l], e1[l], e2[l]};
-            CSH_UNROLL
-            for (int q = 0; q < 4; q++) {
-                const NzEvent v = nz_event(e[q], p[q], Ss, Se);
-                if (v.coded) {
-                    atomicAdd(&h[((v.run & 15u) << 4) | v.size], 1u);
-                    if (v.run >> 4) atomicAdd(&h[0xF0], v.run >> 4);
-                    raw[l] += v.size;
-                } else if (v.term) {
-                    if (v.has) atomicOr(&flag[v.blk >> 5], 1u << (v.blk & 31u));
-                    if (v.eob) atomicOr(&flag[8u + (v.blk >> 5)], 1u << (v.blk & 31u));
-                }
-            }
-        }
-    }
-    CSP_WAVE_SYNC();
-    const uint32_t rawbits = lsum32(raw);
-    LFOR(l) {
-        for (int i = l; i < 256; i += 64) {
-            const uint32_t v = hist[i] + hist[256 + i] + hist[512 + i] + hist[768 + i];
-            c.slot_hist[size_t(r.hist_row) * 256u + uint32_t(i)] = uint16_t(v);
-            if (v) atomicAdd(&c.tables[r.table_base].freq[i], v);
-        }
-        if (l == 0) c.slot_raw[cs] = rawbits;
-        if (l < 4 && r.j * 4u + uint32_t(l) < ((r.nunits_work + 63u) >> 6)) {
-            c.sym_bits[r.word_base + r.j * 4u + uint32_t(l)] = uint64_t(flag[2 * l]) | (uint64_t(flag[2 * l + 1]) << 32);
-            c.eob_bits[r.word_base + r.j * 4u + uint32_t(l)] = uint64_t(flag[8 + 2 * l]) | (uint64_t(flag[9 + 2 * l]) << 32);
-        }
-    }
+            if (l == 0) c.slot_raw[cs] = rawbits;
+            if (l < 4 && j * 4u + uint32_t(l) < ((r.nunits_work + 63u) >> 6)) {
+                c.sym_bits[r.word_base + j * 4u + uint32_t(l)] = uint64_t(flag[2 * l]) | (uint64_t(flag[2 * l + 1]) << 32);
+                c.eob_bits[r.word_base + j * 4u + uint32_t(l)] = uint64_t(flag[8 + 2 * l]) | (uint64_t(flag[9 + 2 * l]) << 32);
+            }
+        }
+        CSP_WAVE_SYNC();
+        LFOR(l) if (l < 16) flag[l] = 0u;
+        CSP_WAVE_SYNC();
+    }
+    freq_flush(c.tables[r.table_base].freq, freq);
 }
 
 __device__ __forceinline__ static void lor_bits(uint32_t *words, uint64_t pos, uint32_t v, uint32_t n) {
@@ -339,30 +379,30 @@
     if (lo) atomicOr(words + (pos >> 5) + 1, lo);
 }
 __global__ void __launch_bounds__(256) k_list_pack(EncCtx c) {
-    CSH_SHARED uint32_t s_win[4][CSH_LP_WORDS];
+    CSH_SHARED alignas(16) uint32_t s_win[4][CSH_LP_WORDS];
     CSH_SHARED uint32_t s_lut[4][256];
     CSH_SHARED uint16_t s_eob[4][256];
-    const int wv = lwave();
+    const int wv = int(uni(uint32_t(lwave())));
     const uint32_t idx = blockIdx.x * 4u + uint32_t(wv);
-    if (idx >= c.nlist_slots) return;
-    const uint32_t cs = c.list_slots[idx];
-    const SlotRec r = c.slots[cs];
+    if (idx >= c.nlist_runs) return;
+    const uint32_t cs0 = c.list_runs[idx];
+    const SlotRec r = c.slots[cs0];
     if (c.work_active && !c.work_active[r.work]) return;
     const ScanWork &w = c.work[r.work];
     if (w.no_room) { LFOR(l) if (l == 0) c.status[w.image] = 20200; return; }
-    const ListSlot ls = list_of_slot(c, r);
+    const uint32_t nrun = run_chunks(c, r);
+    const uint64_t lbase = c.nzlists[r.nzlist].base;
+    ListSlot nx = list_chunk(c, lbase, r.nzrec);
     const uint64_t scan0 = c.chunk_off[r.first_chunk];
-    const uint64_t raw_bit0 = w.raw_off * 8 + (c.chunk_off[cs] - scan0);
+    const uint64_t raw_bit0 = w.raw_off * 8 + (c.chunk_off[cs0] - scan0);
     uint32_t pad = 0;
-    if (r.j == r.nch - 1) { const uint64_t total = c.chunk_off[r.first_chunk + r.nch] - scan0; pad = uint32_t((8 - (total & 7)) & 7); }
+    if (r.j + nrun == r.nch) { const uint64_t total = c.chunk_off[r.first_chunk + r.nch] - scan0; pad = uint32_t((8 - (total & 7)) & 7); }
     uint32_t *buf = s_win[wv], *lut = s_lut[wv];
     uint16_t *eobrun = s_eob[wv];
     LFOR(l) {
-        for (int i = l; i < 256; i += 64) {
-            lut[i] = c.tables[r.table_base].lut[i];
-            eobrun[i] = uint32_t(i) < r.nun ? c.eobrun[r.unit0 + uint32_t(i)] : uint16_t(0);
-        }
-        for (int i = l; i < CSH_LP_WORDS; i += 64) buf[i] = 0u;
+        for (int i = l; i < 256; i += 64) lut[i] = c.tables[r.table_base].lut[i];
+        uint4 zero; zero.x = zero.y = zero.z = zero.w = 0u;
+        for (int i = 4 * l; i < CSH_LP_WORDS; i += 256) *reinterpret_cast<uint4 *>(buf + i) = zero;
     }
     CSP_WAVE_SYNC();
     uint32_t *out = c.raw + (raw_bit0 >> 5);
@@ -371,67 +411,94 @@
     bool first_flush = true;
     const uint32_t Ss = r.Ss, Se = r.Se;
     const uint32_t zrl = lut[0xF0], zc = zrl & 0xFFFFu, zl = zrl >> 16;
-    uint32_t carry = CSH_NZ_END;
-    const uint32_t n_ext = ls.n + (pad ? 1u : 0u);
     LV<uint32_t> x0, x1, x2, x3;
-    LFOR(l) list_load4(ls, 4u * uint32_t(l), x0[l], x1[l], x2[l], x3[l]);
-    for (uint32_t g0 = 0; g0 < n_ext; g0 += 256) {
-        const LV<uint32_t> e0 = x0, e1 = x1, e2 = x2, e3 = x3;
-        if (g0 + 256u < n_ext) LFOR(l) list_load4(ls, g0 + 256u + 4u * uint32_t(l), x0[l], x1[l], x2[l], x3[l]);
-        const LV<uint32_t> p0 = lprev(e3, carry);
-        carry = llast(e3);
-        LV<uint32_t> v0, v1, v2, v3, n0, n1, n2, n3, z, len;
-        LFOR(l) {
-            const uint32_t e[4] = {e0[l], e1[l], e2[l], e3[l]}, p[4] = {p0[l], e0[l], e1[l], e2[l]};
-            uint32_t v[4], n[4], zz = 0, ln = 0;
-            CSH_UNROLL
-            for (int q = 0; q < 4; q++) {
-                v[q] = 0; n[q] = 0;
-                const uint32_t g = g0 + 4u * uint32_t(l) + uint32_t(q);
-                const NzEvent ev = nz_event(e[q], p[q], Ss, Se);
-                if (g >= ls.n) { if (pad && g == ls.n) { v[q] = (1u << pad) - 1u; n[q] = pad; } }
-                else if (ev.coded) {
-                    const uint32_t t = lut[((ev.run & 15u) << 4) | ev.size];
-                    v[q] = ((t & 0xFFFFu) << ev.size) | ev.bits; n[q] = (t >> 16) + ev.size;
-                    zz |= (ev.run >> 4) << (2 * q);
-                    ln += (ev.run >> 4) * zl;
-                } else if (ev.term) {
-                    const uint32_t run = eobrun[ev.blk];
-                    if (run) {
-                        const uint32_t nb = lbitlen(run) - 1u, t = lut[nb << 4];
-                        v[q] = ((t & 0xFFFFu) << nb) | (run & ((1u << nb) - 1u)); n[q] = (t >> 16) + nb;
+    bool ahead = false;
+    for (uint32_t ci = 0; ci < nrun; ci++) {
+        const ListSlot ls = nx;
+        const bool more = ci + 1u < nrun;
+        if (more) nx = list_chunk(c, lbase, r.nzrec + ci + 1u);
+#ifdef CSH_EMUL
+        {
+            const uint64_t want = (raw_bit0 & 31u) + (c.chunk_off[cs0 + ci] - c.chunk_off[cs0]);
+            if (c.overflow[1] ? pos > want : pos != want) { fprintf(stderr, "k_list_pack: chunk %u of a run does not start where the one before it ended\n", ci); abort(); }
+        }
+#endif
+        CSP_WAVE_SYNC();
+        {
+            const uint32_t u0 = r.unit0 + 256u * ci, left = r.nunits_work - 256u * (r.j + ci), nun = left < 256u ? left : 256u;
+            LFOR(l) for (int i = l; i < 256; i += 64) eobrun[i] = uint32_t(i) < nun ? c.eobrun[u0 + uint32_t(i)] : uint16_t(0);
+        }
+        CSP_WAVE_SYNC();
+        if (!ahead) LFOR(l) list_load4(ls, 4u * uint32_t(l), x0[l], x1[l], x2[l], x3[l]);
+        ahead = false;
+        uint32_t carry = CSH_NZ_END;
+        const uint32_t cpad = more ? 0u : pad;
+        const uint32_t n_ext = ls.n + (cpad ? 1u : 0u);
+        for (uint32_t g0 = 0; g0 < n_ext; g0 += 256) {
+            const LV<uint32_t> e0 = x0, e1 = x1, e2 = x2, e3 = x3;
+            if (g0 + 256u < n_ext) LFOR(l) list_load4(ls, g0 + 256u + 4u * uint32_t(l), x0[l], x1[l], x2[l], x3[l]);
+            else if (more) { LFOR(l) list_load4(nx, 4u * uint32_t(l), x0[l], x1[l], x2[l], x3[l]); ahead = true; }
+            const LV<uint32_t> p0 = lprev(e3, carry);
+            carry = llast(e3);
+            LV<uint32_t> v0, v1, v2, v3, n0, n1, n2, n3, z, len;
+            LFOR(l) {
+                const uint32_t e[4] = {e0[l], e1[l], e2[l], e3[l]}, p[4] = {p0[l], e0[l], e1[l], e2[l]};
+                uint32_t v[4], n[4], zz = 0, ln = 0;
+                CSH_UNROLL
+                for (int q = 0; q < 4; q++) {
+                    v[q] = 0; n[q] = 0;
+                    const uint32_t g = g0 + 4u * uint32_t(l) + uint32_t(q);
+                    const NzEvent ev = nz_event(e[q], p[q], Ss, Se);
+                    if (g >= ls.n) { if (cpad && g == ls.n) { v[q] = (1u << cpad) - 1u; n[q] = cpad; } }
+                    else if (ev.coded) {
+                        const uint32_t t = lut[((ev.run & 15u) << 4) | ev.size];
+                        v[q] = ((t & 0xFFFFu) << ev.size) | ev.bits; n[q] = (t >> 16) + ev.size;
+                        zz |= (ev.run >> 4) << (2 * q);
+                        ln += (ev.run >> 4) * zl;
+                    } else if (ev.term) {
+                        const uint32_t run = eobrun[ev.blk];
+                        if (run) {
+                            const uint32_t nb = lbitlen(run) - 1u, t = lut[nb << 4];
+                            v[q] = ((t & 0xFFFFu) << nb) | (run & ((1u << nb) - 1u)); n[q] = (t >> 16) + nb;
+                        }
                     }
-                }
-                ln += n[q];
-            }
-            v0[l] = v[0]; v1[l] = v[1]; v2[l] = v[2]; v3[l] = v[3]; n0[l] = n[0]; n1[l] = n[1]; n2[l] = n[2]; n3[l] = n[3]; z[l] = zz; len[l] = ln;
-        }
-        uint32_t tot;
-        const LV<uint32_t> ex = lscan(len, tot);
-        LFOR(l) {
-            uint64_t at = pos + ex[l] - uint64_t(ww) * 32u;
-            const uint32_t v[4] = {v0[l], v1[l], v2[l], v3[l]}, n[4] = {n0[l], n1[l], n2[l], n3[l]};
-            CSH_UNROLL
-            for (int q = 0; q < 4; q++) {
-                for (uint32_t t = (z[l] >> (2 * q)) & 3u; t; t--) { lor_bits(buf, at, zc, zl); at += zl; }
-                if (n[q]) { lor_bits(buf, at, v[q], n[q]); at += n[q]; }
-            }
-        }
-        pos += tot;
-        const uint32_t done = uint32_t(pos >> 5) - ww;
-        if (done > CSH_LP_WORDS - 640) {
-            CSP_WAVE_SYNC();
-            LFOR(l) for (uint32_t q = uint32_t(l); q < done; q += 64) {
-                const uint32_t v = buf[q];
-                if (first_flush && q == 0) { if (v) atomicOr(out + ww, v); } else out[ww + q] = v;
-            }
-            const uint32_t partial = buf[done];
-            CSP_WAVE_SYNC();
-            LFOR(l) for (int q = l; q < CSH_LP_WORDS; q += 64) buf[q] = (q == 0) ? partial : 0u;
-            CSP_WAVE_SYNC();
-            ww += done; first_flush = false;
-        }
-    }
+                    ln += n[q];
+                }
+                v0[l] = v[0]; v1[l] = v[1]; v2[l] = v[2]; v3[l] = v[3]; n0[l] = n[0]; n1[l] = n[1]; n2[l] = n[2]; n3[l] = n[3]; z[l] = zz; len[l] = ln;
+            }
+            uint32_t tot;
+            const LV<uint32_t> ex = lscan(len, tot);
+            LFOR(l) {
+                uint64_t at = pos + ex[l] - uint64_t(ww) * 32u;
+                const uint32_t v[4] = {v0[l], v1[l], v2[l], v3[l]}, n[4] = {n0[l], n1[l], n2[l], n3[l]};
+                CSH_UNROLL
+                for (int q = 0; q < 4; q++) {
+                    for (uint32_t t = (z[l] >> (2 * q)) & 3u; t; t--) { lor_bits(buf, at, zc, zl); at += zl; }
+                    if (n[q]) { lor_bits(buf, at, v[q], n[q]); at += n[q]; }
+                }
+            }
+            pos += tot;
+            const uint32_t done = uint32_t(pos >> 5) - ww;
+            if (done > CSH_LP_WORDS - 640) {
+                CSP_WAVE_SYNC();
+                LFOR(l) for (uint32_t q = uint32_t(l); q < done; q += 64) {
+                    const uint32_t v = buf[q];
+                    if (first_flush && q == 0) { if (v) atomicOr(out + ww, v); } else out[ww + q] = v;
+                }
+                const uint32_t partial = buf[done];
+                CSP_WAVE_SYNC();
+                LFOR(l) for (int q = l; q < CSH_LP_WORDS; q += 64) buf[q] = (q == 0) ? partial : 0u;
+                CSP_WAVE_SYNC();
+                ww += done; first_flush = false;
+            }
+        }
+    }
+#ifdef CSH_EMUL
+    {
+        const uint64_t want = (raw_bit0 & 31u) + (c.chunk_off[cs0 + nrun] - c.chunk_off[cs0]) + pad;
+        if (c.overflow[1] ? pos > want : pos != want) { fprintf(stderr, "k_list_pack: a run does not end where its sizes say\n"); abort(); }
+    }
+#endif
     CSP_WAVE_SYNC();
     const uint32_t last = uint32_t((pos + 31) >> 5) - ww;
     LFOR(l) for (uint32_t q = uint32_t(l); q < last; q += 64) {
@@ -491,30 +558,42 @@
         }
     }
 }
-__global__ void __launch_bounds__(256) k_list_refine(EncCtx c) {
-    CSH_SHARED uint32_t s_hist[4][4][256];
+__global__ void __launch_bounds__(256, 5) k_list_refine(EncCtx c) {
+    CSH_SHARED alignas(16) uint32_t s_hist[4][4][256];
     CSH_SHARED uint32_t s_lastn[4][256];
     CSH_SHARED uint32_t s_nh[4][256];
     CSH_SHARED uint32_t s_corr[4][256][2];
-    const int wv = lwave();
+    const int wv = int(uni(uint32_t(lwave())));
     const uint32_t idx = blockIdx.x * 4u + uint32_t(wv);
-    if (idx >= c.nref_slots) return;
-    const uint32_t cs = c.ref_slots[idx];
-    const SlotRec r = c.slots[cs];
+    if (idx >= c.nref_runs) return;
+    const uint32_t cs0 = c.ref_runs[idx];
+    const SlotRec r = c.slots[cs0];
     if (c.work_active && !c.work_active[r.work]) return;
-    const ListSlot ls = list_of_slot(c, r);
+    const uint32_t nrun = run_chunks(c, r);
+    const uint64_t lbase = c.nzlists[r.nzlist].base;
+    ListSlot nx = list_chunk(c, lbase, r.nzrec);
+    const TokRegion rg = c.regions[r.region];
     uint32_t *hist = &s_hist[wv][0][0], *lastn = s_lastn[wv], *nh = s_nh[wv], *corr = &s_corr[wv][0][0];
     LFOR(l) {
-        for (int i = l; i < 1024; i += 64) hist[i] = 0u;
-        for (int i = l; i < 256; i += 64) { lastn[i] = 0u; nh[i] = 0u; corr[2 * i] = 0u; corr[2 * i + 1] = 0u; }
-    }
-    CSP_WAVE_SYNC();
+        uint4 zero; zero.x = zero.y = zero.z = zero.w = 0u;
+        for (int i = 4 * l; i < 1024; i += 256) *reinterpret_cast<uint4 *>(hist + i) = zero;
+    }
     const uint32_t Ss = r.Ss, Se = r.Se;
-    RefCarry C;
-    C.runH = C.runN = C.base = C.prevN = C.prevNZ = 0u;
-    LV<uint32_t> ntok;
-    LFOR(l) ntok[l] = 0u;
-    {
+    LV<uint32_t> freq[4];
+    LFOR(l) { freq[0][l] = 0u; freq[1][l] = 0u; freq[2][l] = 0u; freq[3][l] = 0u; }
+    for (uint32_t ci = 0; ci < nrun; ci++) {
+        const ListSlot ls = nx;
+        if (ci + 1u < nrun) nx = list_chunk(c, lbase, r.nzrec + ci + 1u);
+        const uint32_t cs = cs0 + ci, j = r.j + ci, unit0 = r.unit0 + 256u * ci, corr0 = r.corr0 + 256u * ci, hist_row = r.hist_row + ci * uint32_t(r.ntables);
+        const uint32_t left = r.nunits_work - 256u * j, nun = left < 256u ? left : 256u;
+        CSP_WAVE_SYNC();
+        LFOR(l) for (int i = l; i < 256; i += 64) { lastn[i] = 0u; nh[i] = 0u; corr[2 * i] = 0u; corr[2 * i + 1] = 0u; }
+        CSP_WAVE_SYNC();
+        RefCarry C;
+        C.runH = C.runN = C.base = C.prevN = C.prevNZ = 0u;
+        LV<uint32_t> ntok;
+        LFOR(l) ntok[l] = 0u;
+        {
         LV<uint32_t> x[4];
         LFOR(l) list_load4(ls, 4u * uint32_t(l), x[0][l], x[1][l], x[2][l], x[3][l]);
         for (uint32_t g0 = 0; g0 < ls.n; g0 += 256) {
@@ -540,94 +619,89 @@
                 }
             }
         }
-    }
-    CSP_WAVE_SYNC();
-    for (uint32_t w4 = 0; w4 < 4; w4++) {
+        }
+        CSP_WAVE_SYNC();
+        for (uint32_t w4 = 0; w4 < 4; w4++) {
+            LFOR(l) {
+                const uint32_t i = 64u * w4 + uint32_t(l);
+                if (i < nun) {
+                    const uint32_t ln = lastn[i];
+                    if (ls.n && (ln >> 6) != Se) ntok[l] += 1u;
+                    c.tail[unit0 + i] = uint8_t(nh[i] - (ln & 63u));
+                    c.corr[corr0 + i] = (uint64_t(corr[2u * i]) << 32) | corr[2u * i + 1u];
+                }
+            }
+            const uint64_t ms = lballot([&](int b) { const uint32_t i = 64u * w4 + uint32_t(b); return i < nun && lastn[i] != 0u; });
+            const uint64_t me = lballot([&](int b) { const uint32_t i = 64u * w4 + uint32_t(b); return i < nun && (lastn[i] >> 6) != Se; });
+            LFOR(l) if (l == 0 && j * 4u + w4 < ((r.nunits_work + 63u) >> 6)) { c.sym_bits[r.word_base + j * 4u + w4] = ms; c.eob_bits[r.word_base + j * 4u + w4] = me; }
+        }
+        const uint32_t total = lsum32(ntok);
+        hist_flush(hist, c.slot_hist + size_t(hist_row) * 256u, freq);
+        LFOR(l) if (l == 0) c.slot_raw[cs] = C.runN + C.runH;
+        if (c.stats_only) continue;
+        uint32_t rel = 0;
+        LFOR(l) if (l == 0) rel = atomicAdd(&c.tok_cursor[r.region], total);
+        rel = uni(rel);
+        const bool ok = uint64_t(rel) + total <= rg.cap;
         LFOR(l) {
-            const uint32_t i = 64u * w4 + uint32_t(l);
-            if (i < r.nun) {
-                const uint32_t ln = lastn[i];
-                if (ls.n && (ln >> 6) != Se) ntok[l] += 1u;
-                c.tail[r.unit0 + i] = uint8_t(nh[i] - (ln & 63u));
-                c.corr[r.corr0 + i] = (uint64_t(corr[2u * i]) << 32) | corr[2u * i + 1u];
-            }
-        }
-        const uint64_t ms = lballot([&](int j) { const uint32_t i = 64u * w4 + uint32_t(j); return i < r.nun && lastn[i] != 0u; });
-        const uint64_t me = lballot([&](int j) { const uint32_t i = 64u * w4 + uint32_t(j); return i < r.nun && (lastn[i] >> 6) != Se; });
-        LFOR(l) if (l == 0 && r.j * 4u + w4 < ((r.nunits_work + 63u) >> 6)) { c.sym_bits[r.word_base + r.j * 4u + w4] = ms; c.eob_bits[r.word_base + r.j * 4u + w4] = me; }
-    }
-    const uint32_t total = lsum32(ntok);
-    LFOR(l) {
-        for (int i = l; i < 256; i += 64) {
-            const uint32_t v = hist[i] + hist[256 + i] + hist[512 + i] + hist[768 + i];
-            c.slot_hist[size_t(r.hist_row) * 256u + uint32_t(i)] = uint16_t(v);
-            if (v) atomicAdd(&c.tables[r.table_base].freq[i], v);
-        }
-        if (l == 0) c.slot_raw[cs] = C.runN + C.runH;
-    }
-    if (c.stats_only) return;
-    const TokRegion rg = c.regions[r.region];
-    uint32_t rel = 0;
-    LFOR(l) if (l == 0) rel = atomicAdd(&c.tok_cursor[r.region], total);
-    rel = uni(rel);
-    const bool ok = uint64_t(rel) + total <= rg.cap;
-    LFOR(l) {
-        if (l < 4) { c.tok_off[cs * 4u + uint32_t(l)] = rg.base + rel; c.chunk_ntok[cs * 4u + uint32_t(l)] = (ok && l == 0) ? total : 0u; }
-        if (l == 0 && !ok) c.overflow[1] = 1;
-    }
-    if (!ok) return;
-    uint32_t *tk = c.tokens + rg.base + rel;
-    C.runH = C.runN = C.base = C.prevN = C.prevNZ = 0u;
-    uint32_t curc = 0, at = 0;
-    for (uint32_t g0 = 0; g0 < ls.n; g0 += 256) {
-        LV<uint32_t> e[4], hex[4], z[4], zp[4], zq[4], cur[4], nt;
-        LFOR(l) list_load4(ls, g0 + 4u * uint32_t(l), e[0][l], e[1][l], e[2][l], e[3][l]);
-        ref_step<true>(e, Ss, Se, C, hex, z, zp, zq);
-        LFOR(l) {
-            uint32_t s = 0;
-            CSH_UNROLL
-            for (int q = 0; q < 4; q++) {
-                const uint32_t v = e[q][l], blk = (v >> 23) & 255u, lastk = lastn[blk] >> 6, isN = ref_isN(v, Ss, Se);
-                uint32_t nz = 0, n = 0;
-                if ((isN | ref_isH(v, Ss, Se)) && (v & 127u) <= lastk) { nz = ((z[q][l] - zp[q][l]) >> 4) - ((zq[q][l] - zp[q][l]) >> 4); n = nz + isN; }
-                cur[q][l] = n ? ((blk + 1u) << 6) | hex[q][l] : 0u;
-                if ((v & CSH_NZ_END) && lastk != Se) n = 1u;
-                zq[q][l] = nz | (n << 8);
-                s += n;
-            }
-            nt[l] = s;
-        }
-        lscan_last4(cur, curc);
-        uint32_t tot;
-        const LV<uint32_t> ex = lscan(nt, tot);
-        LFOR(l) {
-            uint32_t o = at + ex[l];
-            CSH_UNROLL
-            for (int q = 0; q < 4; q++) {
-                const uint32_t v = e[q][l], blk = (v >> 23) & 255u, nz = zq[q][l] & 255u, n = zq[q][l] >> 8;
-                if (!n) continue;
-                const uint32_t cu = ref_same(cur[q][l], blk);
-                if (v & CSH_NZ_END) {
-                    if (o < total) tk[o] = TK_EOB | (blk << 3) | ((nh[blk] - cu) << 16) | (cu << 22);
-                    o++;
-                    continue;
-                }
-                uint32_t cnt = hex[q][l] - cu, from = cu;
-                for (uint32_t t = 0; t < nz; t++) {
-                    if (o < total) tk[o] = TK_REF | (blk << 3) | (cnt << 16) | (from << 22) | (1u << 28);
-                    o++; cnt = 0u; from = hex[q][l];
-                }
-                if (n > nz) {
-                    if (o < total) tk[o] = TK_REF | (blk << 3) | (((z[q][l] - zp[q][l]) & 15u) << 11) | ((v & 128u) ? 0u : (1u << 15)) | (cnt << 16) | (from << 22);
-                    o++;
-                }
-            }
-        }
-        at += tot;
-    }
+            if (l < 4) { c.tok_off[cs * 4u + uint32_t(l)] = rg.base + rel; c.chunk_ntok[cs * 4u + uint32_t(l)] = (ok && l == 0) ? total : 0u; }
+            if (l == 0 && !ok) c.overflow[1] = 1;
+        }
+        if (!ok) continue;
+        uint32_t *tk = c.tokens + rg.base + rel;
+        C.runH = C.runN = C.base = C.prevN = C.prevNZ = 0u;
+        uint32_t curc = 0, at = 0;
+        for (uint32_t g0 = 0; g0 < ls.n; g0 += 256) {
+            LV<uint32_t> e[4], hex[4], z[4], zp[4], zq[4], cur[4], nt;
+            LFOR(l) list_load4(ls, g0 + 4u * uint32_t(l), e[0][l], e[1][l], e[2][l], e[3][l]);
+            ref_step<true>(e, Ss, Se, C, hex, z, zp, zq);
+            LFOR(l) {
+                uint32_t s = 0;
+                CSH_UNROLL
+                for (int q = 0; q < 4; q++) {
+                    const uint32_t v = e[q][l], blk = (v >> 23) & 255u, lastk = lastn[blk] >> 6, isN = ref_isN(v, Ss, Se);
+                    uint32_t nz = 0, n = 0;
+                    if ((isN | ref_isH(v, Ss, Se)) && (v & 127u) <= lastk) { nz = ((z[q][l] - zp[q][l]) >> 4) - ((zq[q][l] - zp[q][l]) >> 4); n = nz + isN; }
+                    cur[q][l] = n ? ((blk + 1u) << 6) | hex[q][l] : 0u;
+                    if ((v & CSH_NZ_END) && lastk != Se) n = 1u;
+                    zq[q][l] = nz | (n << 8);
+                    s += n;
+                }
+                nt[l] = s;
+            }
+            lscan_last4(cur, curc);
+            uint32_t tot;
+            const LV<uint32_t> ex = lscan(nt, tot);
+            LFOR(l) {
+                uint32_t o = at + ex[l];
+                CSH_UNROLL
+                for (int q = 0; q < 4; q++) {
+                    const uint32_t v = e[q][l], blk = (v >> 23) & 255u, nz = zq[q][l] & 255u, n = zq[q][l] >> 8;
+                    if (!n) continue;
+                    const uint32_t cu = ref_same(cur[q][l], blk);
+                    if (v & CSH_NZ_END) {
+                        if (o < total) tk[o] = TK_EOB | (blk << 3) | ((nh[blk] - cu) << 16) | (cu << 22);
+                        o++;
+                        continue;
+                    }
+                    uint32_t cnt = hex[q][l] - cu, from = cu;
+                    for (uint32_t t = 0; t < nz; t++) {
+                        if (o < total) tk[o] = TK_REF | (blk << 3) | (cnt << 16) | (from << 22) | (1u << 28);
+                        o++; cnt = 0u; from = hex[q][l];
+                    }
+                    if (n > nz) {
+                        if (o < total) tk[o] = TK_REF | (blk << 3) | (((z[q][l] - zp[q][l]) & 15u) << 11) | ((v & 128u) ? 0u : (1u << 15)) | (cnt << 16) | (from << 22);
+                        o++;
+                    }
+                }
+            }
+            at += tot;
+        }
 #ifdef CSH_EMUL
-    if (at != total) { fprintf(stderr, "k_list_refine: pass 2 made %u tokens, pass 1 counted %u\n", at, total); abort(); }
+        if (at != total) { fprintf(stderr, "k_list_refine: pass 2 made %u tokens, pass 1 counted %u\n", at, total); abort(); }
 #endif
+    }
+    freq_flush(c.tables[r.table_base].freq, freq);
 }
 
 __global__ void k_reset_works(ScanWork *work, int nwork) {
@@ -641,11 +715,11 @@
     if (c.nz_build) CSH_LAUNCH_PHASED(k_nzlist, 3, dim3(c.nnzchunks), dim3(2 * CSP_WAVE_THREADS), st, c);
     if (c.nz_filter) CSH_LAUNCH(k_nzfilter, dim3(c.nnzchunks), dim3(CSP_WAVE_THREADS), st, c);
 }
-void launch_list_stats(hipStream_t st, const EncCtx &c) { if (c.nlist_slots) CSH_LAUNCH(k_list_stats, dim3((c.nlist_slots + 3) / 4), dim3(4 * CSP_WAVE_THREADS), st, c); }
-void launch_list_refine(hipStream_t st, const EncCtx &c) { if (c.nref_slots) CSH_LAUNCH(k_list_refine, dim3((c.nref_slots + 3) / 4), dim3(4 * CSP_WAVE_THREADS), st, c); }
-void launch_list_pack(hipStream_t st, const EncCtx &c) { if (c.nlist_slots) CSH_LAUNCH(k_list_pack, dim3((c.nlist_slots + 3) / 4), dim3(4 * CSP_WAVE_THREADS), st, c); }
+void launch_list_stats(hipStream_t st, const EncCtx &c) { if (c.nlist_runs) CSH_LAUNCH(k_list_stats, dim3((c.nlist_runs + 3) / 4), dim3(4 * CSP_WAVE_THREADS), st, c); }
+void launch_list_refine(hipStream_t st, const EncCtx &c) { if (c.nref_runs) CSH_LAUNCH(k_list_refine, dim3((c.nref_runs + 3) / 4), dim3(4 * CSP_WAVE_THREADS), st, c); }
+void launch_list_pack(hipStream_t st, const EncCtx &c) { if (c.nlist_runs) CSH_LAUNCH(k_list_pack, dim3((c.nlist_runs + 3) / 4), dim3(4 * CSP_WAVE_THREADS), st, c); }
 __global__ void __launch_bounds__(64) k_make_slots(const ScanWork *works, uint32_t nworks, const EncScan *script, const NzList *nzlists, SlotRec *slots, uint32_t *slot_work, uint32_t *list_slots,
-                                                   uint32_t *tok_slots, uint32_t *ref_slots) {
+                                                   uint32_t *tok_slots, uint32_t *ref_slots, uint32_t *list_runs, uint32_t *ref_runs, uint32_t list_run) {
     const uint32_t wi = blockIdx.x;
     if (wi >= nworks) return;
     const ScanWork &w = works[wi];
@@ -667,6 +741,8 @@
         slot_work[w.first_chunk + j] = wi;
         (listed ? list_slots : tok_slots)[w.ls_base + j] = w.first_chunk + j;
         if (ref_list) ref_slots[w.rs_base + j] = w.first_chunk + j;
+        if (listed && j % list_run == 0u) list_runs[w.lr_base + j / list_run] = w.first_chunk + j;
+        if (ref_list && j % list_run == 0u) ref_runs[w.rr_base + j / list_run] = w.first_chunk + j;
     }
 }
 __global__ void __launch_bounds__(64) k_rebind_slots(const ScanWork *works, uint32_t nworks, const NzList *nzlists, SlotRec *slots) {
@@ -681,9 +757,9 @@
     if (nworks) CSH_LAUNCH(k_rebind_slots, dim3(nworks), dim3(64), st, works, nworks, nzlists, slots);
 }
 void launch_make_slots(hipStream_t st, const ScanWork *works, uint32_t nworks, const EncScan *script, const NzList *nzlists, SlotRec *slots, uint32_t *slot_work, uint32_t *list_slots,
-                       uint32_t *tok_slots, uint32_t *ref_slots) {
+                       uint32_t *tok_slots, uint32_t *ref_slots, uint32_t *list_runs, uint32_t *ref_runs, uint32_t list_run) {
     if (!nworks) return;
-    CSH_LAUNCH(k_make_slots, dim3(nworks), dim3(64), st, works, nworks, script, nzlists, slots, slot_work, list_slots, tok_slots, ref_slots);
+    CSH_LAUNCH(k_make_slots, dim3(nworks), dim3(64), st, works, nworks, script, nzlists, slots, slot_work, list_slots, tok_slots, ref_slots, list_runs, ref_runs, list_run);
 }
 
 void launch_reset_works(hipStream_t st, ScanWork *work, int nwork) { if (nwork) CSH_LAUNCH(k_reset_works, dim3((nwork + 255) / 256), dim3(256), st, work, nwork); }
diff --git a/caesium-clt_amd/csrc/kernels.h b/caesium-clt_amd/csrc/kernels.h
--- a/caesium-clt_amd/csrc/kernels.h
+++ b/caesium-clt_amd/csrc/kernels.h
@@ -60,7 +60,7 @@
                           uint32_t *need_seq, uint64_t *hist, uint32_t *posv, uint32_t *prog);
 void launch_rebind_slots(hipStream_t st, const ScanWork *works, uint32_t nworks, const NzList *nzlists, SlotRec *slots);
 void launch_make_slots(hipStream_t st, const ScanWork *works, uint32_t nworks, const EncScan *script, const NzList *nzlists, SlotRec *slots, uint32_t *slot_work, uint32_t *list_slots,
-                       uint32_t *tok_slots, uint32_t *ref_slots);
+                       uint32_t *tok_slots, uint32_t *ref_slots, uint32_t *list_runs, uint32_t *ref_runs, uint32_t list_run);
 void launch_decode_prog(hipStream_t st, const uint8_t *clean, const ParScan *pss, const ParHuffSet *huffs, const DecScan *scans, const ProgChain *chains,
                         const int *chain_scans, int nchains, const ImgDesc *imgs, int16_t *coef, uint32_t *need_seq);
 void launch_dec_mark_pending(hipStream_t st, const ParScan *ps, uint32_t total_sub, const uint64_t *list_in, const uint32_t *cnt_in, uint32_t *scan_pending);
@@ -146,6 +146,11 @@
     uint32_t ntok_slots;
     const uint32_t *ref_slots;
     uint32_t nref_slots;
+    const uint32_t *list_runs;
+    uint32_t nlist_runs;
+    const uint32_t *ref_runs;
+    uint32_t nref_runs;
+    uint32_t list_run;
     uint32_t nz_build, nz_filter;
 };
 enum : uint32_t { TK_SYM = 0u, TK_RAW = 1u, TK_ACF = 2u, TK_REF = 3u, TK_EOB = 4u };
@@ -163,6 +168,9 @@
                         uint32_t set, uint32_t nchunks, int16_t *coef);
 void launch_reset_works(hipStream_t st, ScanWork *work, int nwork);
 
+#ifndef CSH_LIST_RUN
+#define CSH_LIST_RUN 8
+#endif
 #ifndef CSH_TR_WG
 #define CSH_TR_WG 256
 #endif
diff --git a/caesium-clt_amd/csrc/pipeline.cpp b/caesium-clt_amd/csrc/pipeline.cpp
--- a/caesium-clt_amd/csrc/pipeline.cpp
+++ b/caesium-clt_amd/csrc/pipeline.cpp
@@ -248,6 +248,7 @@
         t->n_fused_lists = b->enc.last_run_fused;
         t->n_list_refine = b->enc.last_run_refine;
         t->n_ac_in_lists = b->enc.last_run_ac_lists;
+        t->n_list_runs = b->enc.last_run_list_runs;
         for (const Item &it : b->items) if (it.image < 0) t->n_failed++;
         for (int i = 0; i < b->nimg; i++) { t->out_bytes += b->out.h_img_size[i]; t->pixels += uint64_t(b->imgs[i].width) * b->imgs[i].height; }
         t->in_bytes = b->dec.bits_pool.size();
diff --git a/caesium-clt_amd/csrc/types.h b/caesium-clt_amd/csrc/types.h
--- a/caesium-clt_amd/csrc/types.h
+++ b/caesium-clt_amd/csrc/types.h
@@ -165,6 +165,8 @@
     uint32_t ls_base;
     uint32_t rs_base;
     uint32_t region;
+    uint32_t lr_base;
+    uint32_t rr_base;
 };
 
 struct EChunk { uint32_t a; uint16_t comp, kind; uint32_t j; uint32_t plan; uint32_t region; };
diff --git a/include/caesium_hip.h b/include/caesium_hip.h
--- a/include/caesium_hip.h
+++ b/include/caesium_hip.h
@@ -92,6 +92,7 @@
     uint32_t n_fused_lists;
     uint32_t n_list_refine;
     uint32_t n_ac_in_lists;
+    uint32_t n_list_runs;
 } csh_timing;
 
 int csh_device_count(void);
```

Measured after the change: 44660, median of 6. +1.5%, better.
